# NickTravers/NeuralNetworkLibrary

Hardware: AMD Instinct MI355X
Metric: ResNet-34 224x224 training throughput (Learner.train1minibatch, fwd+loss+bwd+optimizer) (higher is better)
Workload: dtype f32; 1 GPU; DogsCats ResNet-34 classifier, 224x224, bs=64 per GPU, SGD momentum 0.9, fp32; global_batch=64, image_size=224, parallelism=dp1

## Files before the change

### include/nnl.h

```cpp
#ifndef NNL_H_
#define NNL_H_

#include <stddef.h>
#include <stdint.h>

#ifdef __cplusplus
extern "C" {
#endif

typedef enum {
  NNL_OK = 0,
  NNL_ERR_INVALID_ARG = -1,
  NNL_ERR_HIP = -2,
  NNL_ERR_UNSUPPORTED = -3,
  NNL_ERR_WORKSPACE = -4
} nnl_status_t;

int nnl_version(void);
const char* nnl_last_error(void);
int nnl_reload_env(void);

enum { NNL_PROF_CONV_FWD = 0, NNL_PROF_CONV_DGRAD = 1, NNL_PROF_CONV_WGRAD = 2, NNL_PROF_EMBDOT = 3,
       NNL_PROF_TABULAR = 4, NNL_PROF_RETINA_LOSS = 5, NNL_PROF_LSTM = 6, NNL_PROF_SOFTMAX_CE = 7,
       NNL_PROF_ELEMENTWISE = 8, NNL_PROF_GEMM = 9, NNL_PROF_OPTIM = 10, NNL_PROF_KINDS = 11 };
int nnl_prof_enable(int enable);
int nnl_prof_collect(int64_t* launches, double* total_ms, double* total_work);
int nnl_prof_collect2(int64_t* launches, double* total_ms, double* total_work, double* total_exec);
int nnl_dp_bump(int32_t* step, void* stream);
int nnl_dp_signal(int32_t* flag, const int32_t* step, void* stream);
int nnl_dp_wait(const int32_t* flag, int32_t value, int64_t timeout_us, int32_t* err, void* stream);
const char* nnl_source_stamp(void);

int nnl_embdotbias_fwd(const int64_t* x, const float* U, const float* M, const float* bu, const float* bi,
                       float* y, float* z, int64_t n, int64_t n_user, int64_t n_item, int64_t D,
                       int has_range, float lo, float hi, int32_t* err_flag, void* stream);
size_t nnl_embdotbias_bwd_workspace_bytes(int64_t n);
int nnl_embdotbias_bwd(const int64_t* x, const float* U, const float* M, const float* z, const float* dy,
                       float* dU, float* dM, float* dbu, float* dbi, int64_t n, int64_t n_user,
                       int64_t n_item, int64_t D, int has_range, float lo, float hi, void* workspace, size_t workspace_bytes, void* stream);

typedef struct {
  int32_t N, H, W, C;
  int32_t K, R, S;
  int32_t stride, pad;
  int32_t P, Q;
} nnl_conv_geom_t;

size_t nnl_conv2d_fwd_workspace_bytes(const nnl_conv_geom_t* g);
int64_t nnl_conv2d_tile_counters(void);
int nnl_conv2d_fwd(const float* x, const float* w, const float* bias, float* y, const nnl_conv_geom_t* g,
                   int relu, void* workspace, size_t workspace_bytes, int32_t* tile_counters, float* bn_partials,
                   const float* bn_pivot, int32_t* bn_rows, void* stream);
int nnl_conv2d_fwd_add_up2(const float* x, const float* w, const float* bias, const float* small, float* y,
                           const nnl_conv_geom_t* g, void* stream);
int nnl_upsample2_bwd(const float* dy, float* dsmall, int64_t N, int64_t h, int64_t w, int64_t C, void* stream);
int nnl_conv2d_weight_transpose(const float* w, float* wt, int K, int R, int S, int C, void* stream);
typedef struct {
  const float* w;
  float* wt;
  int32_t K, RS, C, first_tile;
} nnl_wt_desc_t;
int nnl_conv2d_weight_transpose_multi(const nnl_wt_desc_t* desc, const int32_t* tile_tensor, int64_t n_tiles,
                                      double total_elems, void* stream);
size_t nnl_conv2d_dgrad_workspace_bytes(const nnl_conv_geom_t* g);
int nnl_conv2d_dgrad(const float* dy, const float* wt, float* dx, const nnl_conv_geom_t* g, const float* addend,
                     void* workspace, size_t workspace_bytes, int32_t* tile_counters, void* stream);
typedef struct {
  const float* src;
  float* dst;
  int32_t rows, ch, flip, first_block;
  int32_t two_d, reserved;
} nnl_wino_desc_t;
int nnl_conv2d_wino_preferred(const nnl_conv_geom_t* g, int dgrad);
int nnl_wino_filter_multi(const nnl_wino_desc_t* desc, const int32_t* block_desc, int64_t n_blocks, void* stream);
int nnl_conv2d_fwd_pre(const float* x, const float* w, const float* bias, float* y, const nnl_conv_geom_t* g, int relu,
                       void* workspace, size_t workspace_bytes, int32_t* tile_counters, float* bn_partials, const float* bn_pivot,
                       int32_t* bn_rows, const float* u, void* stream);
int nnl_conv2d_dgrad_pre(const float* dy, const float* wt, float* dx, const nnl_conv_geom_t* g, const float* addend,
                         void* workspace, size_t workspace_bytes, int32_t* tile_counters, const float* u, void* stream);
size_t nnl_debug_conv_wino_workspace_bytes(int N, int H, int W, int C, int K);
int nnl_debug_conv_wino_fwd(const float* x, const float* filt, const float* bias, const float* add, float* y, void* ws,
                            size_t ws_bytes, int32_t* counters, long n_counters, float* bn_part, const float* bn_pivot, int N,
                            int H, int W, int C, int K, int relu, int flip, void* stream);
size_t nnl_debug_conv_wino2_workspace_bytes(int N, int H, int W, int C, int K);
int nnl_debug_conv_wino2_fwd(const float* x, const float* filt, const float* bias, const float* add, float* y, void* ws,
                            size_t ws_bytes, int32_t* counters, long n_counters, float* bn_part, const float* bn_pivot, int N,
                            int H, int W, int C, int K, int relu, int flip, void* stream);
int nnl_debug_conv_plan_times(int N, int H, int W, int C, int K, double* out);

int nnl_debug_route_record(int enable);
int nnl_debug_route_collect(char* out, size_t n);
size_t nnl_conv2d_wgrad_workspace_bytes(const nnl_conv_geom_t* g);
int nnl_conv2d_wgrad(const float* x, const float* dy, float* dw, const nnl_conv_geom_t* g, void* workspace,
                     size_t workspace_bytes, void* stream);
size_t nnl_colsum_workspace_bytes(int64_t rows, int64_t cols);
int nnl_sum_tensors(const float* const* src, int n, float* out, int64_t numel, void* stream);
int nnl_colsum(const float* a, float* out, int64_t rows, int64_t cols, void* workspace, size_t workspace_bytes,
               void* stream);
int nnl_relu_gate_colsum(const float* dy, const float* y, float* g, float* colsum, int64_t rows, int64_t cols, void* workspace,
                         size_t workspace_bytes, void* stream);
int nnl_act_gate_colsum(const float* dy, const float* y, float* g, float* colsum, int64_t rows, int64_t cols, int act,
                        void* workspace, size_t workspace_bytes, void* stream);

size_t nnl_bn_workspace_bytes(int64_t rows, int64_t C);
int nnl_bn_fwd(const float* x, const float* gamma, const float* beta, const float* residual, float* y,
               float* save_mean, float* save_invstd, float* running_mean, float* running_var, int64_t rows,
               int64_t C, float eps, float momentum, int training, int relu, int64_t* num_batches_tracked,
               uint32_t* relu_mask, const float* ext_partials, int64_t ext_rows, const float* ext_pivot, float* pivot_out,
               void* workspace, size_t workspace_bytes, void* stream);
int nnl_bn_bwd(const float* dy, const float* y, const uint32_t* relu_mask, const float* x, const float* gamma,
               const float* mean, const float* invstd, float* dx, float* dres, float* dgamma, float* dbeta, int64_t rows,
               int64_t C, int training, int relu, void* workspace, size_t workspace_bytes, void* stream);

int nnl_bn_relu_maxpool_supported(int64_t C);
int nnl_bn_relu_maxpool_fwd(const float* x, const float* gamma, const float* beta, float* y, uint8_t* idx, float* save_mean,
                            float* save_invstd, float* save_scale, float* save_shift, float* running_mean, float* running_var,
                            int64_t N, int64_t H, int64_t W, int64_t C, int64_t P, int64_t Q, int ks, int stride, int pad, float eps,
                            float momentum, int training, int64_t* num_batches_tracked, void* workspace, size_t workspace_bytes,
                            void* stream);
int nnl_bn_relu_maxpool_bwd(const float* dpool, const float* y, const uint8_t* idx, const float* x, const float* gamma,
                            const float* beta, const float* mean, const float* invstd, const float* scale, const float* shift,
                            float* dx, float* dgamma, float* dbeta,
                            int64_t N, int64_t H, int64_t W, int64_t C, int64_t P, int64_t Q, int ks, int stride, int pad,
                            int training, void* workspace, size_t workspace_bytes, void* stream);

int nnl_debug_bn_plan(int64_t rows, int64_t C, int64_t N, int64_t H, int64_t W, int64_t P, int64_t Q, int32_t* out10);

int nnl_bn_sync_stats(const float* x, float* stats, int64_t rows, int64_t C, void* workspace, size_t workspace_bytes,
                      void* stream);
int nnl_bn_sync_fwd(const float* x, const float* all_stats, int world, const float* gamma, const float* beta,
                    const float* residual, float* y, float* save_mean, float* save_invstd, float* running_mean,
                    float* running_var, int64_t rows, int64_t C, float eps, float momentum, int relu,
                    int64_t* num_batches_tracked, uint32_t* relu_mask, void* workspace, size_t workspace_bytes, void* stream);
int nnl_bn_sync_bwd_reduce(const float* dy, const float* y, const uint32_t* relu_mask, const float* x, const float* mean,
                           const float* invstd, float* sums, int64_t rows, int64_t C, int relu, void* workspace,
                           size_t workspace_bytes, void* stream);
int nnl_bn_sync_bwd(const float* dy, const float* y, const uint32_t* relu_mask, const float* x, const float* gamma,
                    const float* mean, const float* invstd, const float* local_sums, const float* global_sums,
                    const float* all_stats,
                    int world, float* dx, float* dres, float* dgamma, float* dbeta, int64_t rows, int64_t C, int relu,
                    void* workspace, size_t workspace_bytes, void* stream);

int nnl_maxpool2d_fwd(const float* x, float* y, uint8_t* idx, int64_t N, int64_t H, int64_t W, int64_t C, int64_t P,
                      int64_t Q, int ksize, int stride, int pad, void* stream);
int nnl_maxpool2d_bwd(const float* dy, const uint8_t* idx, float* dx, int64_t N, int64_t H, int64_t W, int64_t C,
                      int64_t P, int64_t Q, int ksize, int stride, int pad, void* stream);
int nnl_concat_pool_fwd(const float* x, float* out, int32_t* argmax, int64_t N, int64_t HW, int64_t C, void* stream);
int nnl_concat_pool_bwd(const float* dout, const int32_t* argmax, float* dx, int64_t N, int64_t HW, int64_t C, void* stream);

int nnl_bbox_decode(const float* anchors, const float* reg, const float* clas, int64_t bs, int64_t A, int64_t K,
                    const float* mean4, const float* std4, float thresh, float width, float height, float* cand_boxes,
                    int32_t* cand_classes, float* cand_scores, int32_t* cand_order, int32_t* cand_count, void* stream);
int nnl_bbox_decode_window(const float* anchors, const float* reg, const float* clas, int64_t bs, int64_t A, int64_t K,
                           const float* mean4, const float* std4, float thresh, float x_min, float y_min, float x_max, float y_max,
                           float* cand_boxes, int32_t* cand_classes, float* cand_scores, int32_t* cand_order, int32_t* cand_count,
                           void* stream);
size_t nnl_nms_workspace_bytes(int64_t bs, int64_t top_k);
int nnl_nms(const float* cand_boxes, const int32_t* cand_classes, const float* cand_scores, const int32_t* cand_order,
            const int32_t* cand_count, int64_t bs, int64_t cap, int64_t top_k, float max_overlap, float* kept_boxes,
            int32_t* kept_classes, float* kept_scores, int32_t* kept_count, void* workspace, size_t workspace_bytes,
            void* stream);

typedef struct {
  float col_jit, row_jit;
  float inv;
  float cols;
  int32_t flip;
} nnl_tta_undo_t;
int nnl_tta_bbox_merge(const float* boxes, const int32_t* classes, const float* scores, const int32_t* counts,
                       const nnl_tta_undo_t* undo, int64_t L, int64_t P, int64_t M, float* cand_boxes, int32_t* cand_classes,
                       float* cand_scores, int32_t* cand_order, int32_t* cand_count, int32_t* err_flag, void* stream);

int nnl_tab_renorm(const int64_t* xcat, float* const* tables, const int32_t* card, const int32_t* dim,
                   const int32_t* row_off, const int32_t* row_table, int32_t* flags, int64_t bs, int32_t ncat,
                   int32_t total_rows, float max_norm, int32_t* err_flag, void* stream);
int nnl_tab_gather_fwd(const int64_t* xcat, const float* const* tables, const int32_t* card, const int32_t* dim,
                       const int32_t* col_off, const int32_t* col_table, const float* row_mask, const float* cont,
                       const float* cont_mask, float* out, int64_t bs, int32_t ncat, int32_t cat_width,
                       int32_t n_cont, int32_t ld_out, void* stream);
size_t nnl_tab_scatter_bwd_workspace_bytes(int64_t bs, int32_t ncat);
int nnl_tab_scatter_bwd(const int64_t* xcat, const int32_t* card, const int32_t* dim, const int32_t* col_off,
                        const int32_t* col_table, const int64_t* grad_off, const float* row_mask,
                        const float* cont_mask, const float* dout, float* dtab_flat, int64_t dtab_elems,
                        float* dcont, int64_t bs, int32_t ncat, int32_t cat_width, int32_t n_cont, int32_t ld_out,
                        void* workspace, size_t workspace_bytes, void* stream);
int nnl_tab_scan_bwd(const int64_t* xcat, const int32_t* card, const int32_t* dim, const int32_t* col_off,
                     const int64_t* grad_off, const float* row_mask, const float* cont_mask, const float* dout,
                     float* dtab_flat, float* dcont, const int32_t* blk_col, const int32_t* blk_first, int32_t n_scan_blocks,
                     int32_t max_dim, int64_t bs, int32_t ncat, int32_t cat_width, int32_t n_cont, int32_t ld_out, void* stream);

int nnl_pad_cols(const float* src, float* dst, int64_t rows, int64_t C, int64_t Cp, void* stream);
int nnl_keep_masks(const float* u, float* a, int64_t na, float keep_a, float* b, int64_t nb, float keep_b, void* stream);

int nnl_linear_small_supported(int64_t N);
int nnl_linear_small_fwd(const float* x, const float* w, const float* bias, float* y, int64_t M, int64_t K, int64_t ldx, int64_t N,
                         void* stream);
size_t nnl_linear_small_bwd_workspace_bytes(int64_t M, int64_t K, int64_t N);
int nnl_linear_small_bwd(const float* dy, const float* x, const float* w, float* dx, float* dw, float* db, int64_t M, int64_t K,
                         int64_t ldx, int64_t N, void* workspace, size_t workspace_bytes, void* stream);

size_t nnl_retina_loss_workspace_bytes(int64_t bs, int64_t A);
int nnl_retina_loss_fwd(const float* anchors, const float* reg, const float* clas, const float* boxes,
                        const int64_t* cats, int32_t* state, float* npos, float* out, int64_t bs, int64_t A,
                        int64_t K, int64_t M, float beta, float alpha, float gamma, void* workspace,
                        size_t workspace_bytes, void* stream);
int nnl_retina_loss_bwd(const float* anchors, const float* reg, const float* clas, const float* boxes,
                        const int64_t* cats, const int32_t* state, const float* npos, const float* grad_out,
                        float* dreg, float* dclas, int64_t bs, int64_t A, int64_t K, int64_t M, float beta,
                        float alpha, float gamma, void* stream);

int64_t nnl_lstm_padded_hidden(int64_t H);
int64_t nnl_lstm_padded_gates(int64_t H);
size_t nnl_lstm_workspace_bytes(int64_t T, int64_t B, int64_t H);
int nnl_lstm_fwd(const float* gx, const float* w_hh_pad, const float* h0, const float* c0, float* y, float* cy,
                 float* gates, int64_t T, int64_t B, int64_t H, void* workspace, size_t workspace_bytes, int32_t* err_flag,
                 void* stream);
int nnl_lstm_bwd(const float* dy, const float* dhT, const float* dcT, const float* gates, const float* cy,
                 const float* c0, const float* w_hh_t_pad, float* dgates_pad, float* dh0, float* dc0, int64_t T, int64_t B,
                 int64_t H, void* workspace, size_t workspace_bytes, int32_t* err_flag, void* stream);
int nnl_debug_lstm_bptt2_plan(int64_t B, int64_t H, int32_t* out5);
int nnl_debug_lstm_plan(int64_t B, int64_t H, int32_t* out14);

size_t nnl_mse_workspace_bytes(int64_t n);
int nnl_mse_fwd(const float* pred, const float* target, float* loss, int64_t n, void* workspace, size_t workspace_bytes, void* stream);
int nnl_mse_bwd(const float* pred, const float* target, const float* grad_out, float* dpred, int64_t n, void* stream);
size_t nnl_bce_logits_workspace_bytes(int64_t n);
int nnl_bce_logits_fwd(const float* logits, const float* target, float* loss, int64_t n, void* workspace, size_t workspace_bytes, void* stream);
int nnl_bce_logits_bwd(const float* logits, const float* target, const float* grad_out, float* dlogits, int64_t n, void* stream);
size_t nnl_fbeta_workspace_bytes(int64_t N, int64_t C);
int nnl_fbeta(const float* pred, const float* target, float* out, int64_t N, int64_t C, float beta2, float threshold, int use_thresh, float eps,
              void* workspace, size_t workspace_bytes, void* stream);
int nnl_scaled_sigmoid_fwd(const float* x, float* y, float* sig, int64_t n, float lo, float hi, void* stream);
int nnl_scaled_sigmoid_bwd(const float* dy, const float* sig, float* dx, int64_t n, float lo, float hi, void* stream);

int nnl_embedding_rowmask_fwd(const int64_t* x, const float* W, const float* rowmask, float* out, int64_t n,
                              int64_t V, int64_t D, int32_t* err_flag, void* stream);
size_t nnl_embedding_rowmask_bwd_workspace_bytes(int64_t n);
int nnl_embedding_rowmask_bwd(const int64_t* x, const float* rowmask, const float* dout, float* dW, int64_t n,
                              int64_t V, int64_t D, int64_t padding_idx, void* workspace, size_t workspace_bytes, void* stream);
int nnl_softmax_ce_fwd(const float* logits, const int64_t* target, float* lse, float* loss_rows, float* loss_mean,
                       int64_t rows, int64_t V, int32_t* err_flag, void* stream);
int nnl_softmax_ce_bwd(const float* logits, const int64_t* target, const float* lse, const float* grad_out,
                       float* dlogits, int64_t rows, int64_t V, int64_t ld_dlogits, void* stream);
size_t nnl_seq_reg_workspace_bytes(int64_t T, int64_t R);
int nnl_seq_reg_fwd(const float* h, float* out3, int64_t T, int64_t R, float alpha, float beta, void* workspace,
                    size_t workspace_bytes, void* stream);
int nnl_seq_reg_bwd(const float* h, const float* grad_out, float* dh, int64_t T, int64_t R, float alpha, float beta, void* stream);
// ... 112 lines not shown
```

### neuralnetworklibrary_amd/_lib.py

```python
import ctypes as C
import os

import torch

_HERE = os.path.dirname(os.path.abspath(__file__))
LIB_PATH = os.environ.get('NNL_LIB_PATH') or os.path.join(_HERE, 'libnnl_hip.so')

if not os.path.exists(LIB_PATH):
    raise ImportError(
        f"{LIB_PATH} not found: build it with `python -c 'import __graft_entry__ as g; g.build()'` "
        "(or `make -C neuralnetworklibrary_amd/csrc`). There is no CPU fallback for the HIP hot path.")

lib = C.CDLL(LIB_PATH)

c_p = C.c_void_p
i32, i64, f32, f64 = C.c_int32, C.c_int64, C.c_float, C.c_double
sz = C.c_size_t


class ConvGeom(C.Structure):
    _fields_ = [('N', i32), ('H', i32), ('W', i32), ('C', i32), ('K', i32), ('R', i32), ('S', i32),
                ('stride', i32), ('pad', i32), ('P', i32), ('Q', i32)]


SIGNATURES = {
    'nnl_version': (C.c_int, []),
    'nnl_last_error': (C.c_char_p, []),
    'nnl_reload_env': (C.c_int, []),
    'nnl_prof_enable': (C.c_int, [C.c_int]),
    'nnl_prof_collect': (C.c_int, [C.POINTER(i64), C.POINTER(f64), C.POINTER(f64)]),
    'nnl_prof_collect2': (C.c_int, [C.POINTER(i64), C.POINTER(f64), C.POINTER(f64), C.POINTER(f64)]),
    'nnl_source_stamp': (C.c_char_p, []),
    'nnl_dp_bump': (C.c_int, [c_p, c_p]),
    'nnl_dp_signal': (C.c_int, [c_p, c_p, c_p]),
    'nnl_dp_wait': (C.c_int, [c_p, i32, i64, c_p, c_p]),
    'nnl_embdotbias_fwd': (C.c_int, [c_p, c_p, c_p, c_p, c_p, c_p, c_p, i64, i64, i64, i64, C.c_int, f32, f32,
                                     c_p, c_p]),
    'nnl_embdotbias_bwd_workspace_bytes': (sz, [i64]),
    'nnl_embdotbias_bwd': (C.c_int, [c_p, c_p, c_p, c_p, c_p, c_p, c_p, c_p, c_p, i64, i64, i64, i64, C.c_int,
                                     f32, f32, c_p, sz, c_p]),
    'nnl_conv2d_fwd_workspace_bytes': (sz, [C.POINTER(ConvGeom)]),
    'nnl_conv2d_dgrad_workspace_bytes': (sz, [C.POINTER(ConvGeom)]),
    'nnl_conv2d_tile_counters': (i64, []),
    'nnl_conv2d_wino_preferred': (C.c_int, [C.POINTER(ConvGeom), C.c_int]),
    'nnl_wino_filter_multi': (C.c_int, [c_p, c_p, i64, c_p]),
    'nnl_conv2d_fwd_pre': (C.c_int, [c_p, c_p, c_p, c_p, C.POINTER(ConvGeom), C.c_int, c_p, sz, c_p, c_p, c_p, C.POINTER(i32), c_p, c_p]),
    'nnl_conv2d_dgrad_pre': (C.c_int, [c_p, c_p, c_p, C.POINTER(ConvGeom), c_p, c_p, sz, c_p, c_p, c_p]),
    'nnl_debug_conv_wino_workspace_bytes': (sz, [C.c_int] * 5),
    'nnl_debug_conv_wino_fwd': (C.c_int, [c_p] * 6 + [sz, c_p, C.c_long, c_p, c_p] + [C.c_int] * 7 + [c_p]),
    'nnl_debug_conv_wino2_workspace_bytes': (sz, [C.c_int] * 5),
    'nnl_debug_conv_wino2_fwd': (C.c_int, [c_p] * 6 + [sz, c_p, C.c_long, c_p, c_p] + [C.c_int] * 7 + [c_p]),
    'nnl_debug_conv_plan_times': (C.c_int, [C.c_int] * 5 + [C.POINTER(C.c_double)]),
    'nnl_debug_route_record': (C.c_int, [C.c_int]),
    'nnl_debug_route_collect': (C.c_int, [C.c_char_p, sz]),
    'nnl_conv2d_fwd': (C.c_int, [c_p, c_p, c_p, c_p, C.POINTER(ConvGeom), C.c_int, c_p, sz, c_p, c_p, c_p, C.POINTER(i32), c_p]),
    'nnl_conv2d_weight_transpose': (C.c_int, [c_p, c_p, C.c_int, C.c_int, C.c_int, C.c_int, c_p]),
    'nnl_conv2d_weight_transpose_multi': (C.c_int, [c_p, c_p, i64, f64, c_p]),
    'nnl_conv2d_dgrad': (C.c_int, [c_p, c_p, c_p, C.POINTER(ConvGeom), c_p, c_p, sz, c_p, c_p]),
    'nnl_conv2d_wgrad_workspace_bytes': (sz, [C.POINTER(ConvGeom)]),
    'nnl_conv2d_wgrad': (C.c_int, [c_p, c_p, c_p, C.POINTER(ConvGeom), c_p, sz, c_p]),
    'nnl_colsum_workspace_bytes': (sz, [i64, i64]),
    'nnl_colsum': (C.c_int, [c_p, c_p, i64, i64, c_p, sz, c_p]),
    'nnl_relu_gate_colsum': (C.c_int, [c_p, c_p, c_p, c_p, i64, i64, c_p, sz, c_p]),
    'nnl_conv2d_fwd_add_up2': (C.c_int, [c_p, c_p, c_p, c_p, c_p, C.POINTER(ConvGeom), c_p]),
    'nnl_upsample2_bwd': (C.c_int, [c_p, c_p, i64, i64, i64, i64, c_p]),
    'nnl_act_gate_colsum': (C.c_int, [c_p, c_p, c_p, c_p, i64, i64, C.c_int, c_p, sz, c_p]),
    'nnl_maxpool2d_fwd': (C.c_int, [c_p, c_p, c_p, i64, i64, i64, i64, i64, i64, C.c_int, C.c_int, C.c_int, c_p]),
    'nnl_maxpool2d_bwd': (C.c_int, [c_p, c_p, c_p, i64, i64, i64, i64, i64, i64, C.c_int, C.c_int, C.c_int, c_p]),
    'nnl_sum_tensors': (C.c_int, [c_p, C.c_int, c_p, i64, c_p]),
    'nnl_bn_relu_maxpool_supported': (C.c_int, [i64]),
    'nnl_bn_relu_maxpool_fwd': (C.c_int, [c_p, c_p, c_p, c_p, c_p, c_p, c_p, c_p, c_p, c_p, c_p, i64, i64, i64, i64, i64, i64,
                                          C.c_int, C.c_int, C.c_int, f32, f32, C.c_int, c_p, c_p, sz, c_p]),
    'nnl_bn_relu_maxpool_bwd': (C.c_int, [c_p, c_p, c_p, c_p, c_p, c_p, c_p, c_p, c_p, c_p, c_p, c_p, c_p, i64, i64, i64, i64, i64, i64,
                                          C.c_int, C.c_int, C.c_int, C.c_int, c_p, sz, c_p]),
    'nnl_concat_pool_fwd': (C.c_int, [c_p, c_p, c_p, i64, i64, i64, c_p]),
    'nnl_concat_pool_bwd': (C.c_int, [c_p, c_p, c_p, i64, i64, i64, c_p]),
    'nnl_bbox_decode': (C.c_int, [c_p, c_p, c_p, i64, i64, i64, c_p, c_p, f32, f32, f32, c_p, c_p, c_p, c_p, c_p, c_p]),
    'nnl_bbox_decode_window': (C.c_int, [c_p, c_p, c_p, i64, i64, i64, c_p, c_p, f32, f32, f32, f32, f32, c_p, c_p, c_p, c_p, c_p, c_p]),
    'nnl_nms_workspace_bytes': (sz, [i64, i64]),
    'nnl_nms': (C.c_int, [c_p, c_p, c_p, c_p, c_p, i64, i64, i64, f32, c_p, c_p, c_p, c_p, c_p, sz, c_p]),
    'nnl_tta_bbox_merge': (C.c_int, [c_p, c_p, c_p, c_p, c_p, i64, i64, i64, c_p, c_p, c_p, c_p, c_p, c_p, c_p]),
    'nnl_tab_renorm': (C.c_int, [c_p, c_p, c_p, c_p, c_p, c_p, c_p, i64, i32, i32, f32, c_p, c_p]),
    'nnl_tab_gather_fwd': (C.c_int, [c_p, c_p, c_p, c_p, c_p, c_p, c_p, c_p, c_p, c_p, i64, i32, i32, i32, i32, c_p]),
    'nnl_tab_scatter_bwd_workspace_bytes': (sz, [i64, i32]),
    'nnl_tab_scatter_bwd': (C.c_int, [c_p, c_p, c_p, c_p, c_p, c_p, c_p, c_p, c_p, c_p, i64, c_p, i64, i32, i32, i32, i32, c_p, sz, c_p]),
    'nnl_tab_scan_bwd': (C.c_int, [c_p] * 12 + [i32, i32, i64, i32, i32, i32, i32, c_p]),
    'nnl_pad_cols': (C.c_int, [c_p, c_p, i64, i64, i64, c_p]),
    'nnl_keep_masks': (C.c_int, [c_p, c_p, i64, f32, c_p, i64, f32, c_p]),
    'nnl_linear_small_supported': (C.c_int, [i64]),
    'nnl_linear_small_fwd': (C.c_int, [c_p, c_p, c_p, c_p, i64, i64, i64, i64, c_p]),
    'nnl_linear_small_bwd_workspace_bytes': (sz, [i64, i64, i64]),
    'nnl_linear_small_bwd': (C.c_int, [c_p, c_p, c_p, c_p, c_p, c_p, i64, i64, i64, i64, c_p, sz, c_p]),
    'nnl_retina_loss_workspace_bytes': (sz, [i64, i64]),
    'nnl_retina_loss_fwd': (C.c_int, [c_p, c_p, c_p, c_p, c_p, c_p, c_p, c_p, i64, i64, i64, i64, f32, f32, f32, c_p, sz, c_p]),
    'nnl_retina_loss_bwd': (C.c_int, [c_p, c_p, c_p, c_p, c_p, c_p, c_p, c_p, c_p, c_p, i64, i64, i64, i64, f32, f32, f32, c_p]),
    'nnl_lstm_padded_hidden': (i64, [i64]),
    'nnl_lstm_padded_gates': (i64, [i64]),
    'nnl_lstm_workspace_bytes': (sz, [i64, i64, i64]),
    'nnl_lstm_fwd': (C.c_int, [c_p, c_p, c_p, c_p, c_p, c_p, c_p, i64, i64, i64, c_p, sz, c_p, c_p]),
    'nnl_lstm_bwd': (C.c_int, [c_p, c_p, c_p, c_p, c_p, c_p, c_p, c_p, c_p, c_p, i64, i64, i64, c_p, sz, c_p, c_p]),
    'nnl_debug_lstm_bptt2_plan': (C.c_int, [i64, i64, c_p]),
    'nnl_debug_lstm_plan': (C.c_int, [i64, i64, C.POINTER(i32)]),
    'nnl_embedding_rowmask_fwd': (C.c_int, [c_p, c_p, c_p, c_p, i64, i64, i64, c_p, c_p]),
    'nnl_embedding_rowmask_bwd_workspace_bytes': (sz, [i64]),
    'nnl_embedding_rowmask_bwd': (C.c_int, [c_p, c_p, c_p, c_p, i64, i64, i64, i64, c_p, sz, c_p]),
    'nnl_softmax_ce_fwd': (C.c_int, [c_p, c_p, c_p, c_p, c_p, i64, i64, c_p, c_p]),
    'nnl_softmax_ce_bwd': (C.c_int, [c_p, c_p, c_p, c_p, c_p, i64, i64, i64, c_p]),
    'nnl_mse_workspace_bytes': (sz, [i64]),
    'nnl_mse_fwd': (C.c_int, [c_p, c_p, c_p, i64, c_p, sz, c_p]),
    'nnl_mse_bwd': (C.c_int, [c_p, c_p, c_p, c_p, i64, c_p]),
    'nnl_bce_logits_workspace_bytes': (sz, [i64]),
    'nnl_bce_logits_fwd': (C.c_int, [c_p, c_p, c_p, i64, c_p, sz, c_p]),
    'nnl_bce_logits_bwd': (C.c_int, [c_p, c_p, c_p, c_p, i64, c_p]),
    'nnl_fbeta_workspace_bytes': (sz, [i64, i64]),
    'nnl_fbeta': (C.c_int, [c_p, c_p, c_p, i64, i64, C.c_float, C.c_float, C.c_int, C.c_float, c_p, sz, c_p]),
    'nnl_scaled_sigmoid_fwd': (C.c_int, [c_p, c_p, c_p, i64, C.c_float, C.c_float, c_p]),
    'nnl_scaled_sigmoid_bwd': (C.c_int, [c_p, c_p, c_p, i64, C.c_float, C.c_float, c_p]),
    'nnl_seq_reg_workspace_bytes': (sz, [i64, i64]),
    'nnl_seq_reg_fwd': (C.c_int, [c_p, c_p, i64, i64, C.c_float, C.c_float, c_p, sz, c_p]),
    'nnl_seq_reg_bwd': (C.c_int, [c_p, c_p, c_p, i64, i64, C.c_float, C.c_float, c_p]),
    'nnl_weight_drop': (C.c_int, [c_p, i64, c_p, c_p, i64, i64, i64, C.c_uint64, C.c_float, c_p]),
    'nnl_lstm_cell_b1': (C.c_int, [c_p, i64, c_p, i64, c_p, c_p, c_p, i64, c_p, i64, i64, c_p, c_p, c_p, c_p, i64, i64, c_p]),
    'nnl_lm_next_token_workspace_bytes': (sz, [i64, i64]),
    'nnl_lm_next_token': (C.c_int, [c_p, i64, c_p, i64, i64, i64, i64, c_p, i64, c_p, i64, c_p, c_p, c_p, c_p, sz, c_p]),
    'nnl_attn_pool_workspace_bytes': (sz, [i64, i64, i64, i64]),
    'nnl_attn_pool_fwd': (C.c_int, [c_p, c_p, c_p, c_p, c_p, i64, c_p, c_p, i64, i64, i64, i64, c_p, sz, c_p, i64, c_p]),
    'nnl_attn_pool_bwd': (C.c_int, [c_p, c_p, c_p, c_p, c_p, c_p, c_p, c_p, c_p, c_p, i64, i64, i64, i64, c_p, sz, c_p, i64, c_p]),
    'nnl_image_aug_workspace_bytes': (sz, [i64, i64, i64]),
    'nnl_image_aug': (C.c_int, [c_p, i64, c_p, i64, c_p, i64, i64, i64, C.POINTER(f32), C.c_int, c_p, c_p, sz, c_p]),
    'nnl_detect_aug': (C.c_int, [c_p, i64, c_p, i64, c_p, c_p, c_p, i64, c_p, i64, i64, i64, i64, i64, i64, f64, C.POINTER(f32),
                                 c_p, c_p, c_p, c_p]),
    'nnl_optim_chunk_elems': (i64, []),
    'nnl_optim_patch': (C.c_int, [c_p, c_p, c_p, i64, c_p]),
    'nnl_optim_step': (C.c_int, [c_p, c_p, c_p, i64, C.c_int, c_p, C.c_int, c_p, c_p]),
    'nnl_bn_workspace_bytes': (sz, [i64, i64]),
    'nnl_bn_fwd': (C.c_int, [c_p, c_p, c_p, c_p, c_p, c_p, c_p, c_p, c_p, i64, i64, f32, f32, C.c_int, C.c_int, c_p, c_p, c_p, i64,
                             c_p, c_p, c_p, sz, c_p]),
    'nnl_debug_bn_plan': (C.c_int, [i64] * 7 + [C.POINTER(i32)]),
    'nnl_bn_sync_stats': (C.c_int, [c_p, c_p, i64, i64, c_p, sz, c_p]),
    'nnl_bn_sync_fwd': (C.c_int, [c_p, c_p, C.c_int, c_p, c_p, c_p, c_p, c_p, c_p, c_p, c_p, i64, i64, f32, f32, C.c_int, c_p,
                                  c_p, c_p, sz, c_p]),
    'nnl_bn_sync_bwd_reduce': (C.c_int, [c_p, c_p, c_p, c_p, c_p, c_p, c_p, i64, i64, C.c_int, c_p, sz, c_p]),
    'nnl_bn_sync_bwd': (C.c_int, [c_p, c_p, c_p, c_p, c_p, c_p, c_p, c_p, c_p, c_p, C.c_int, c_p, c_p, c_p, c_p, i64, i64,
                                  C.c_int, c_p, sz, c_p]),
    'nnl_bn_bwd': (C.c_int, [c_p, c_p, c_p, c_p, c_p, c_p, c_p, c_p, c_p, c_p, c_p, i64, i64, C.c_int, C.c_int, c_p, sz, c_p]),
    'nnl_seg_event_gaps': (C.c_int, [c_p, c_p, c_p, i64, f64, c_p, c_p, c_p, c_p, c_p]),
    'nnl_seg_rolling': (C.c_int, [c_p, c_p, c_p, c_p, i64, i64, i64, i64, C.c_int, C.c_int, c_p, c_p]),
    'nnl_assoc_contingency': (C.c_int, [c_p, c_p, i64, i64, c_p, c_p, c_p, i64, c_p, c_p]),
    'nnl_assoc_table_stats': (C.c_int, [c_p, c_p, i64, c_p, c_p, c_p, i64, c_p, c_p]),
    'nnl_assoc_cat_cont_workspace_bytes': (sz, [c_p, i64, c_p, i64]),
    'nnl_assoc_cat_cont': (C.c_int, [c_p, c_p, i64, c_p, c_p, i64, i64, c_p, c_p, i64, c_p, sz, c_p, c_p]),
    'nnl_assoc_cont_cont_workspace_bytes': (sz, [i64, i64]),
    'nnl_assoc_cont_cont': (C.c_int, [c_p, c_p, i64, i64, c_p, c_p, i64, C.c_int, c_p, sz, c_p, c_p]),
    'nnl_det_coco_match': (C.c_int, [c_p] * 7 + [i64, i64, i64, c_p, i64, c_p, i64, c_p, sz, c_p, c_p, c_p, c_p, c_p]),
    'nnl_det_coco_accumulate': (C.c_int, [c_p] * 8 + [i64, i64, i64, i64, i64, c_p, i64, c_p, i64, c_p, c_p, c_p, c_p]),
    'nnl_det_map_match': (C.c_int, [c_p, c_p, c_p, c_p, i64, i64, i64, c_p, i64, c_p, c_p]),
    'nnl_det_map_integrate_workspace_bytes': (sz, [i64, i64]),
    'nnl_det_map_integrate': (C.c_int, [c_p, c_p, c_p, c_p, c_p, i64, i64, i64, c_p, sz, c_p, c_p]),
}

for _name, (_res, _args) in SIGNATURES.items():
    try:
        _fn = getattr(lib, _name)
    except AttributeError as e:
        raise ImportError(f"libnnl_hip.so does not export {_name}; rebuild it") from e
    _fn.restype = _res
    _fn.argtypes = _args

PROF_KINDS = ['conv_fwd', 'conv_dgrad', 'conv_wgrad', 'embdot', 'tabular', 'retina_loss', 'lstm',
              'softmax_ce', 'elementwise', 'gemm', 'optim']


class NnlError(RuntimeError):
    pass


def check(status):
    if status != 0:
        raise NnlError(f"nnl error {status}: {lib.nnl_last_error().decode()}")


def ptr(t):
    return None if t is None else C.c_void_p(t.data_ptr())


def stream():
    return C.c_void_p(torch.cuda.current_stream().cuda_stream)


def require_cuda(*tensors):
    for t in tensors:
        if t is not None and not t.is_cuda:
            raise NnlError("nnl HIP op called with a non-CUDA tensor: the MI355X path has no CPU fallback")


def prof_enable(flag=True):
    check(lib.nnl_prof_enable(1 if flag else 0))


def prof_collect():
    n = len(PROF_KINDS)
    a, b, c, d = (i64 * n)(), (f64 * n)(), (f64 * n)(), (f64 * n)()
    check(lib.nnl_prof_collect2(a, b, c, d))
    return {k: {'launches': int(a[i]), 'ms': float(b[i]), 'work': float(c[i]), 'exec': float(d[i])} for i, k in enumerate(PROF_KINDS)}


def source_stamp_of_tree():
    import glob
    import hashlib
    csrc = os.path.join(os.path.dirname(os.path.abspath(__file__)), 'csrc')
    names = sorted(os.path.basename(p) for p in glob.glob(os.path.join(csrc, '*.hip')) + glob.glob(os.path.join(csrc, '*.h')))
    hsh = hashlib.sha256()
    for p in [os.path.join(csrc, n) for n in names] + [os.path.join(csrc, 'Makefile'), os.path.join(csrc, '..', '..', 'include', 'nnl.h')]:
# ... 8 lines not shown
```

### neuralnetworklibrary_amd/csrc/conv2d.hip

```cpp
#include "igemm_kernels.h"
#include "igemm_taps.h"
#include "wino.h"
#include "igemm_wgrad.h"
#include "igemm_wgrad2d.h"

#ifdef NNL_TAPS_TIMING
static void* g_wgrad_dbg = nullptr;
extern "C" void* nnl_debug_wgrad_stamps(void) { return g_wgrad_dbg; }
#endif

namespace {

int check_geom(const nnl_conv_geom_t* g, const char* who) {
  if (!g) return nnl_set_error(NNL_ERR_INVALID_ARG, "%s: null geometry", who);
  if (g->N <= 0 || g->H <= 0 || g->W <= 0 || g->C <= 0 || g->K <= 0 || g->R <= 0 || g->S <= 0 || g->stride <= 0 ||
      g->pad < 0)
    return nnl_set_error(NNL_ERR_INVALID_ARG, "%s: non-positive dimension", who);
  if (g->H + 2L * g->pad < g->R || g->W + 2L * g->pad < g->S)
    return nnl_set_error(NNL_ERR_INVALID_ARG, "%s: the %d x %d filter is larger than the padded input (%d x %d, pad %d)", who, g->R, g->S,
                         g->H, g->W, g->pad);
  const int P = (g->H + 2 * g->pad - g->R) / g->stride + 1, Q = (g->W + 2 * g->pad - g->S) / g->stride + 1;
  if (P != g->P || Q != g->Q || P <= 0 || Q <= 0)
    return nnl_set_error(NNL_ERR_INVALID_ARG, "%s: P,Q=(%d,%d) do not match the geometry (%d,%d)", who, g->P, g->Q, P, Q);
  if (g->C % 4 != 0)
    return nnl_set_error(NNL_ERR_UNSUPPORTED, "%s: C=%d must be a multiple of 4 (pad the channels; ops.py does)", who, g->C);
  if ((long)g->N * g->H * g->W * g->C >= (1L << 31) || (long)g->N * g->P * g->Q * g->K >= (1L << 31) ||
      (long)g->N * g->P * g->Q >= (1L << 30))
    return nnl_set_error(NNL_ERR_UNSUPPORTED, "%s: tensor too large for 32-bit row indexing", who);
  return NNL_OK;
}

template <int BM, int BN, int WGM, int WGN, int MODE>
int launch_rowk(IgemmRowkParams p, hipStream_t s) {
  p.grid_m = (int)nnl_cdiv(p.M, BM);
  p.grid_n = (int)nnl_cdiv(p.Nc, BN);
  NNL_ROUTE("rowk<%d,%d>:%s", BM, BN, MODE == IGEMM_MODE_FWD ? "fwd" : "dgrad");
  hipLaunchKernelGGL((igemm_rowk_kernel<BM, BN, 16, WGM, WGN, MODE>), dim3(p.grid_m * p.grid_n), dim3(256), 0, s, p);
  NNL_CHECK_LAUNCH();
  return NNL_OK;
}

template <int MODE>
int dispatch_rowk(const IgemmRowkParams& p, hipStream_t s) {
  const long b128 = nnl_cdiv(p.M, 128);
  if (p.Nc > 64) {
    if (b128 * nnl_cdiv(p.Nc, 128) >= 400) return launch_rowk<128, 128, 2, 2, MODE>(p, s);
    if (nnl_cdiv(p.M, 64) * nnl_cdiv(p.Nc, 128) >= 400) return launch_rowk<64, 128, 2, 2, MODE>(p, s);
    return launch_rowk<64, 64, 2, 2, MODE>(p, s);
  }
  if (b128 >= 400) return launch_rowk<128, 64, 2, 2, MODE>(p, s);
  return launch_rowk<64, 64, 2, 2, MODE>(p, s);
}


static bool taps_dma(int bk) {
  const int m = NNL_ENV_INT("NNL_IGEMM_DMA", 0);
  return bk == 16 ? (m & 1) != 0 : (m & 2) != 0;
}

template <int BM, int BN, int BK = 16>
int launch_taps(IgemmTapsParams p, hipStream_t s) {
  p.grid_m = (int)nnl_cdiv(p.M, BM);
  p.grid_n = (int)nnl_cdiv(p.Nc, BN);
  p.cls_tiles = p.grid_m * p.grid_n;
  const dim3 grid((unsigned)(p.grid_m * p.grid_n * (p.ncls > 1 ? p.ncls : 1)), p.ksplit > 1 ? p.ksplit : 1);
  NNL_ROUTE("taps<%d,%d,%d>%s%s%s", BM, BN, BK, (BM == 64 && BN == 64 && taps_dma(BK)) ? ":dma" : "", p.ncls > 1 ? ":ncls" : "",
            p.ksplit > 1 ? ":ksplit" : "");
  if constexpr (BM == 64 && BN == 64) {
    if (taps_dma(BK))
      hipLaunchKernelGGL((igemm_taps_kernel<64, 64, BK, 2, 2, false, 0, true>), grid, dim3(256), 0, s, p);
    else if constexpr (BK == 16)
      hipLaunchKernelGGL((igemm_taps_kernel<64, 64, 16, 2, 2, true, 0, false, 2>), grid, dim3(256), 0, s, p);
    else
      hipLaunchKernelGGL((igemm_taps_kernel<64, 64, BK, 2, 2, true>), grid, dim3(256), 0, s, p);
  } else {
    hipLaunchKernelGGL((igemm_taps_kernel<BM, BN, BK, 2, 2>), grid, dim3(256), 0, s, p);
  }
  NNL_CHECK_LAUNCH();
  return NNL_OK;
}

template <int BK>
int launch_taps_ktail(IgemmTapsParams p, hipStream_t s) {
  p.grid_m = (int)nnl_cdiv(p.M, 64);
  p.grid_n = (int)nnl_cdiv(p.Nc, 64);
  p.cls_tiles = p.grid_m * p.grid_n;
  NNL_ROUTE("taps_ktail<%d>", BK);
  hipLaunchKernelGGL((igemm_taps_kernel<64, 64, BK, 2, 2, true, 0, false, 1, true>), dim3((unsigned)(p.grid_m * p.grid_n), 1), dim3(256), 0, s, p);
  NNL_CHECK_LAUNCH();
  return NNL_OK;
}

struct BalPlan {
  int on, bk, main_ks, n_main_tiles, tail_slices, tail_row0;
  size_t main_floats, tail_floats;
  double t_us;
};

constexpr int kCUs = 256;
constexpr long kTileCounters = 65536;

BalPlan plan_balance(long M, int Nc, int C, int ntaps) {
  BalPlan best{};
  const int e_bal = NNL_ENV_INT("NNL_IGEMM_BALANCE", 1);
  if (e_bal == 0 || Nc % 4 != 0) return best;
  const long gm = nnl_cdiv(M, 64), gn = nnl_cdiv(Nc, 64), T = gm * gn;
  const int bk = ((T < 1200 || C >= 256 || C == 64) && C % 32 == 0) ? 32 : 16;
  const long I = (long)ntaps * (C / bk);
  const double c_it = bk == 32 ? 0.60 : 0.30;
  const double occ = bk == 32 ? 4 : 6;
  auto wave_iters = [&](long blocks, long iters) {
    if (blocks <= 0) return 0.0;
    const long cap = (long)occ * kCUs;
    const long full = blocks / cap, rem = blocks - full * cap;
    return (double)(full * (long)occ + nnl_cdiv(rem, kCUs)) * iters;
  };
  const double plain = wave_iters(T, I) * c_it;
  best.t_us = plain;
  double best_t = plain * (e_bal == 2 ? 1.25 : 0.99);
  const int plan_extra = 2;
  const double plan_bw = 16000 * 1.0e3;
  for (int ks = 1; ks <= 4; ks *= 2) {
    if (I / ks < 8) break;
    const long units = T * ks;
    long n_main = ((units / kCUs) * kCUs / ks / gn) * gn;
    if (n_main > T) n_main = T;
    const long tail = T - n_main;
    const long it_main = nnl_cdiv(I, ks);
    static const int kSlices[] = {1, 2, 3, 4, 6, 8, 9, 12, 16, 18, 24, 32, 36, 48};
    for (int S : kSlices) {
      if (tail == 0 && S > 1) break;
      if (S > 1 && I / S < 4) break;
      const long it_tail = nnl_cdiv(I, S);
      const long tail_blocks = tail * S;
      double t = (wave_iters(n_main * ks, it_main) + wave_iters(tail_blocks, it_tail + (S > 1 ? plan_extra : 0))) * c_it;
      const long row0 = (n_main / gn) * 64 < M ? (n_main / gn) * 64 : M;
      const double main_b = ks > 1 ? (2.0 * ks + 1) * row0 * Nc * 4 : 0;
      const double tail_b = S > 1 ? (2.0 * S + 1) * (M - row0) * Nc * 4 : 0;
      t += (main_b + tail_b) / plan_bw + (ks > 1 ? 1 : 0) + (S > 1 && tail ? 1 : 0);
      if (t < best_t) {
        best_t = t;
        best.t_us = t;
        best.on = 1; best.bk = bk; best.main_ks = ks; best.n_main_tiles = (int)n_main; best.tail_slices = tail ? S : 1;
        best.tail_row0 = (int)row0;
        best.main_floats = ks > 1 ? (size_t)ks * row0 * Nc : 0;
        best.tail_floats = (S > 1 && tail) ? (size_t)S * (M - row0) * Nc : 0;
      }
    }
  }
  if (best.on && best.main_ks == 1 && best.tail_slices == 1) best.on = 0;
  return best;
}
// ... 2 lines not shown
  const BalPlan pl = plan_balance(M, Nc, C, ntaps);
  return pl.on ? (pl.main_floats + pl.tail_floats) * sizeof(float) : 0;
}

__global__ __launch_bounds__(256) void slab_reduce_kernel(const float* __restrict__ part, long slab_stride4, int nslabs,
                                                           float* __restrict__ out, long n4, const float* __restrict__ bias,
                                                           const float* __restrict__ add, int Nc4, int relu) {
  const long i = (long)blockIdx.x * 256 + threadIdx.x;
  if (i >= n4) return;
  f32x4 acc = reinterpret_cast<const f32x4*>(part)[i];
  for (int sl = 1; sl < nslabs; ++sl) acc += reinterpret_cast<const f32x4*>(part)[(long)sl * slab_stride4 + i];
  if (bias) acc += reinterpret_cast<const f32x4*>(bias)[i % Nc4];
  if (add) acc += reinterpret_cast<const f32x4*>(add)[i];
  if (relu == 1) { acc[0] = fmaxf(acc[0], 0.f); acc[1] = fmaxf(acc[1], 0.f); acc[2] = fmaxf(acc[2], 0.f); acc[3] = fmaxf(acc[3], 0.f); }
  else if (relu == 2) { acc[0] = nnl_sigmoid(acc[0]); acc[1] = nnl_sigmoid(acc[1]); acc[2] = nnl_sigmoid(acc[2]); acc[3] = nnl_sigmoid(acc[3]); }
  reinterpret_cast<f32x4*>(out)[i] = acc;
}

int launch_balanced(IgemmTapsParams p, const BalPlan& pl, float* ws, int* counters, hipStream_t s) {
  p.grid_m = (int)nnl_cdiv(p.M, 64);
  p.grid_n = (int)nnl_cdiv(p.Nc, 64);
  const int T = p.grid_m * p.grid_n;
  p.bal = 1; p.main_ks = pl.main_ks; p.n_main_tiles = pl.n_main_tiles; p.tail_slices = pl.tail_slices; p.tail_row0 = pl.tail_row0;
  p.main_out = ws; p.main_slab_stride = (long)pl.tail_row0 * p.Nc;
  p.tail_out = ws + pl.main_floats; p.tail_slab_stride = (long)(p.M - pl.tail_row0) * p.Nc;
  p.tile_counters = counters;
  const unsigned grid = (unsigned)(pl.n_main_tiles * pl.main_ks + (T - pl.n_main_tiles) * pl.tail_slices);
  NNL_ROUTE("balanced<%d>%s%s%s%s:%s@main_ks=%d,tail_slices=%d", pl.bk == 32 ? 32 : 16, p.ktail ? ":ktail" : "",
            (!p.ktail && taps_dma(pl.bk == 32 ? 32 : 16)) ? ":dma" : "", pl.main_ks > 1 ? ":main_ks" : "", pl.tail_slices > 1 ? ":tail_slices" : "",
            p.tile_counters != nullptr ? "counters" : "reduce", pl.main_ks, pl.tail_slices);
  if (p.ktail && pl.bk == 32)
    hipLaunchKernelGGL((igemm_taps_kernel<64, 64, 32, 2, 2, true, 0, false, 1, true>), dim3(grid), dim3(256), 0, s, p);
  else if (p.ktail)
    hipLaunchKernelGGL((igemm_taps_kernel<64, 64, 16, 2, 2, true, 0, false, 1, true>), dim3(grid), dim3(256), 0, s, p);
  else if (pl.bk == 32 && taps_dma(32))
    hipLaunchKernelGGL((igemm_taps_kernel<64, 64, 32, 2, 2, false, 0, true>), dim3(grid), dim3(256), 0, s, p);
  else if (pl.bk != 32 && taps_dma(16))
    hipLaunchKernelGGL((igemm_taps_kernel<64, 64, 16, 2, 2, false, 0, true>), dim3(grid), dim3(256), 0, s, p);
  else if (pl.bk == 32)
    hipLaunchKernelGGL((igemm_taps_kernel<64, 64, 32, 2, 2, true>), dim3(grid), dim3(256), 0, s, p);
  else
    hipLaunchKernelGGL((igemm_taps_kernel<64, 64, 16, 2, 2, true, 0, false, 2>), dim3(grid), dim3(256), 0, s, p);
  NNL_CHECK_LAUNCH();
  if (p.tile_counters != nullptr) return NNL_OK;
  const int Nc4 = p.Nc / 4;
  if (pl.main_ks > 1 && pl.tail_row0 > 0) {
    const long n4 = (long)pl.tail_row0 * Nc4;
    NNL_ROUTE("slab_reduce:main");
    hipLaunchKernelGGL(slab_reduce_kernel, dim3((unsigned)nnl_cdiv(n4, 256)), dim3(256), 0, s, (const float*)p.main_out, n4, pl.main_ks,
                       p.y, n4, p.bias, p.add, Nc4, p.relu);
    NNL_CHECK_LAUNCH();
  }
  if (pl.tail_slices > 1 && p.M > pl.tail_row0) {
    const long n4 = (long)(p.M - pl.tail_row0) * Nc4;
    const long off = (long)pl.tail_row0 * p.Nc;
    NNL_ROUTE("slab_reduce:tail");
    hipLaunchKernelGGL(slab_reduce_kernel, dim3((unsigned)nnl_cdiv(n4, 256)), dim3(256), 0, s, (const float*)p.tail_out, n4,
                       pl.tail_slices, p.y + off, n4, p.bias, p.add ? p.add + off : nullptr, Nc4, p.relu);
    NNL_CHECK_LAUNCH();
  }
  return NNL_OK;
}

int dispatch_taps(const IgemmTapsParams& p_in, hipStream_t s, void* ws = nullptr, size_t ws_bytes = 0, int* counters = nullptr,
                  int* bn_rows = nullptr) {
  IgemmTapsParams p = p_in;
#ifdef NNL_TAPS_TIMING
  p.tile_counters = counters;
#endif
  if (bn_rows) *bn_rows = 0;
  float* const bn_part = p.bn_part;
  p.bn_part = nullptr;
  if (!p.ktail && p.ntaps == 1 && p.C <= 512 && p.Nc >= 8192 && p.M >= 1024 && p.ncls <= 1) {
    return launch_taps<128, 128>(p, s);
  }
  const bool dense = p.out_stride == 1 && p.OH == p.P && p.OW == p.Q && p.oh0 == 0 && p.ow0 == 0 && p.ksplit <= 1;
  const int rows64 = (int)nnl_cdiv(p.M, 64);
  if (ws != nullptr && dense) {
    const BalPlan pl = plan_balance(p.M, p.Nc, p.ktail ? (int)nnl_cdiv(p.C, 32) * 32 : p.C, p.ntaps);
    if (pl.on && ws_bytes >= (pl.main_floats + pl.tail_floats) * sizeof(float)) {
      int* const cnt = rows64 * nnl_cdiv(p.Nc, 64) <= kTileCounters ? counters : nullptr;
      if (bn_part && cnt != nullptr) {
        p.bn_part = bn_part;
        if (bn_rows) *bn_rows = rows64;
      }
      return launch_balanced(p, pl, (float*)ws, cnt, s);
    }
  }
  if (bn_part && dense) {
    p.bn_part = bn_part;
    if (bn_rows) *bn_rows = rows64;
  }
  if (p.ktail) return p.C >= 64 ? launch_taps_ktail<32>(p, s) : launch_taps_ktail<16>(p, s);
  const long blocks64 = rows64 * nnl_cdiv(p.Nc, 64) * (p.ncls > 1 ? p.ncls : 1);
  const bool bk32 = blocks64 < 1200 || p.C >= 256 || p.C == 64;
  if (bk32 && p.C % 32 == 0) return launch_taps<64, 64, 32>(p, s);
  return launch_taps<64, 64>(p, s);
}

bool affine_taps_ok(int S) { return S <= 32; }

bool dgrad_tap_table_ok(const nnl_conv_geom_t* g) {
  if (g->stride == 1 && affine_taps_ok(g->S)) return true;
  return (g->pad + g->stride - 1) / g->stride <= 127;
}

bool taps_ok(long a_elems, long b_elems, int C, int ntaps) {
  return C % 16 == 0 && ntaps <= IGEMM_MAX_TAPS && a_elems * 4 < (1L << 31) && b_elems * 4 < (1L << 32) - 64;
}

int taps_kind(long a_elems, long b_elems, int C, int ntaps) {
  if (taps_ok(a_elems, b_elems, C, ntaps)) return 1;
  if (ntaps == 1 && C % 4 == 0 && C >= 32 && a_elems * 4 < (1L << 31) && b_elems * 4 < (1L << 32) - 64 && NNL_ENV_INT("NNL_IGEMM_KTAIL", 1) != 0)
    return 2;
  return 0;
}

__global__ void weight_transpose_kernel(const float* __restrict__ w, float* __restrict__ wt, int K, int RS, int C) {
  __shared__ float tile[32][33];
  const int tap = blockIdx.z;
  const int k0 = blockIdx.y * 32, c0 = blockIdx.x * 32;
  const int tx = threadIdx.x & 31, ty = threadIdx.x >> 5;
  for (int i = ty; i < 32; i += 8) {
    const int k = k0 + i, c = c0 + tx;
    tile[i][tx] = (k < K && c < C) ? w[((long)k * RS + tap) * C + c] : 0.f;
  }
  __syncthreads();
  for (int i = ty; i < 32; i += 8) {
    const int c = c0 + i, k = k0 + tx;
    if (k < K && c < C) wt[((long)c * RS + tap) * K + k] = tile[tx][i];
  }
}

__global__ void weight_transpose_multi_kernel(const nnl_wt_desc_t* __restrict__ desc, const int* __restrict__ tile_tensor) {
  __shared__ float tile[32][33];
  const nnl_wt_desc_t d = desc[tile_tensor[blockIdx.x]];
  int t = (int)blockIdx.x - d.first_tile;
  const int ct = (d.C + 31) / 32, kt = (d.K + 31) / 32;
  const int c0 = (t % ct) * 32; t /= ct;
  const int k0 = (t % kt) * 32;
  const int tap = t / kt;
  const int tx = threadIdx.x & 31, ty = threadIdx.x >> 5;
  for (int i = ty; i < 32; i += 8) {
    const int k = k0 + i, c = c0 + tx;
    tile[i][tx] = (k < d.K && c < d.C) ? d.w[((long)k * d.RS + tap) * d.C + c] : 0.f;
  }
  __syncthreads();
  for (int i = ty; i < 32; i += 8) {
    const int c = c0 + i, k = k0 + tx;
    if (k < d.K && c < d.C) d.wt[((long)c * d.RS + tap) * d.K + k] = tile[tx][i];
  }
}

__global__ __launch_bounds__(256) void splitk_reduce_kernel(const float* __restrict__ part, float* __restrict__ out, long n4,
                                                             int splits) {
  __shared__ f32x4 red[8][32];
  const int col = threadIdx.x & 31, sl = threadIdx.x >> 5;
  const long i = (long)blockIdx.x * 32 + col;
  f32x4 acc = {0.f, 0.f, 0.f, 0.f};
  if (i < n4) {
    int s = sl;
    for (; s + 24 < splits; s += 32) {
      const f32x4 v0 = reinterpret_cast<const f32x4*>(part)[(long)s * n4 + i], v1 = reinterpret_cast<const f32x4*>(part)[(long)(s + 8) * n4 + i];
      const f32x4 v2 = reinterpret_cast<const f32x4*>(part)[(long)(s + 16) * n4 + i], v3 = reinterpret_cast<const f32x4*>(part)[(long)(s + 24) * n4 + i];
      acc += v0; acc += v1; acc += v2; acc += v3;
    }
    for (; s < splits; s += 8) acc += reinterpret_cast<const f32x4*>(part)[(long)s * n4 + i];
  }
  red[sl][col] = acc;
  __syncthreads();
  if (sl == 0 && i < n4) {
    f32x4 t = red[0][col];
#pragma unroll
    for (int l = 1; l < 8; ++l) t += red[l][col];
    reinterpret_cast<f32x4*>(out)[i] = t;
  }
}

__global__ __launch_bounds__(256) void colsum_partial_kernel(const float* __restrict__ a, float* __restrict__ part, long rows,
                                                              int cols, long rows_per_chunk) {
  __shared__ float red[4][64];
  const int c = blockIdx.x * 64 + (threadIdx.x & 63);
  const int rl = threadIdx.x >> 6;
  const long r0 = (long)blockIdx.y * rows_per_chunk;
  const long r1 = r0 + rows_per_chunk < rows ? r0 + rows_per_chunk : rows;
  float acc = 0.f;
  if (c < cols) {
    long r = r0 + rl;
    for (; r + 12 < r1; r += 16) {
      const float v0 = a[r * cols + c], v1 = a[(r + 4) * cols + c], v2 = a[(r + 8) * cols + c], v3 = a[(r + 12) * cols + c];
      acc += (v0 + v1) + (v2 + v3);
    }
    for (; r < r1; r += 4) acc += a[r * cols + c];
  }
  red[rl][threadIdx.x & 63] = acc;
  __syncthreads();
  if (rl == 0 && c < cols)
    part[(long)blockIdx.y * cols + c] = (red[0][threadIdx.x] + red[1][threadIdx.x]) + (red[2][threadIdx.x] + red[3][threadIdx.x]);
}

template <int ACT>
__device__ __forceinline__ float act_gate(float dy, float y) {
  if (ACT == 1) return y > 0.f ? dy : 0.f;
  return dy * ((1.f - y) * y);
}

template <int ACT>
__global__ __launch_bounds__(256) void act_gate_colsum_kernel(const float* __restrict__ dy, const float* __restrict__ y,
                                                               float* __restrict__ g, float* __restrict__ part, long rows, int cols,
                                                               long rows_per_chunk) {
  __shared__ float red[4][64];
  const int c = blockIdx.x * 64 + (threadIdx.x & 63);
  const int rl = threadIdx.x >> 6;
  const long r0 = (long)blockIdx.y * rows_per_chunk;
  const long r1 = r0 + rows_per_chunk < rows ? r0 + rows_per_chunk : rows;
  float acc = 0.f;
  if (c < cols) {
    long r = r0 + rl;
    for (; r + 12 < r1; r += 16) {
      float v[4];
#pragma unroll
      for (int u = 0; u < 4; ++u) {
        const long o = (r + 4 * u) * cols + c;
        v[u] = act_gate<ACT>(dy[o], y[o]);
      }
#pragma unroll
      for (int u = 0; u < 4; ++u) g[(r + 4 * u) * cols + c] = v[u];
      acc += (v[0] + v[1]) + (v[2] + v[3]);
    }
    for (; r < r1; r += 4) {
      const long o = r * cols + c;
      const float v = act_gate<ACT>(dy[o], y[o]);
      g[o] = v;
      acc += v;
    }
  }
  red[rl][threadIdx.x & 63] = acc;
  __syncthreads();
  if (rl == 0 && c < cols && part != nullptr)
    part[(long)blockIdx.y * cols + c] = (red[0][threadIdx.x] + red[1][threadIdx.x]) + (red[2][threadIdx.x] + red[3][threadIdx.x]);
}

__global__ __launch_bounds__(256) void colsum_final_kernel(const float* __restrict__ part, float* __restrict__ out, int cols,
                                                            int nchunk) {
  __shared__ float red[16][17];
  const int cl = threadIdx.x & 15, kl = threadIdx.x >> 4;
  const int c = blockIdx.x * 16 + cl;
  float acc = 0.f;
  if (c < cols)
    for (int k = kl; k < nchunk; k += 16) acc += part[(long)k * cols + c];
  red[kl][cl] = acc;
  __syncthreads();
  if (kl == 0 && c < cols) {
    float t = red[0][cl];
#pragma unroll
    for (int l = 1; l < 16; ++l) t += red[l][cl];
    out[c] = t;
  }
}

int colsum_chunks(long rows) {
  long n = nnl_cdiv(rows, 64);
  if (n > 256) n = 256;
  if (n < 1) n = 1;
  return (int)n;
}

struct WgradPlan { int bm, bn, grid_m, grid_n, splits, k_per_split, kg; };

WgradPlan plan_wgrad(int Mc, int Nc, long Kp, int square_bn_divides = 0) {
  struct Cand { int bm, bn; double cost; };
  static const Cand cands[4] = {{128, 128, 1.00}, {128, 64, 1.08}, {64, 128, 1.08}, {64, 64, 1.10}};
  const long max_splits = Kp / 256 > 0 ? Kp / 256 : 1;
  WgradPlan pl{};
  double best_t = 1e300;
  for (int ci = 0; ci < 4; ++ci) {
    const Cand& c = cands[ci];
    if (square_bn_divides != 0) {
      if (c.bm != c.bn || square_bn_divides % c.bn != 0 || (c.bm == 128 && Mc < 128)) continue;
    } else if ((c.bm == 128 && Mc < 128) || (c.bn == 128 && Nc < 128)) continue;
    const long tiles = nnl_cdiv(Mc, c.bm) * nnl_cdiv(Nc, c.bn);
    const double us_per_px = (double)c.bm * c.bn * 2.0 / 441e3 * c.cost;
    for (long sp = 1; sp <= max_splits && (sp == 1 || tiles * sp <= 256 * 5); ++sp) {
      const long k1 = nnl_cdiv(nnl_cdiv(Kp, sp), 32) * 32;
      const long rs = nnl_cdiv(Kp, k1);
      if (rs != sp) continue;
      const long per_cu = nnl_cdiv(tiles * rs, 256);
      const double starve = per_cu < 4 ? pow(4.0 / per_cu, 0.3) : 1.0;
      const double t = (double)per_cu * k1 * us_per_px * starve + (rs > 1 ? (rs + 1.0) * Mc * Nc * 4 / 4.5e6 + 3 : 0);
      if (t < best_t) {
        best_t = t;
        pl.bm = c.bm; pl.bn = c.bn; pl.grid_m = (int)nnl_cdiv(Mc, c.bm); pl.grid_n = (int)nnl_cdiv(Nc, c.bn);
        pl.splits = (int)rs; pl.k_per_split = (int)k1;
      }
    }
  }
  if (pl.bm == 0) {
    pl.bm = Mc >= 128 ? 128 : 64; pl.bn = (Nc >= 128 && pl.bm == 128) ? 128 : 64;
    if (square_bn_divides != 0 && square_bn_divides % pl.bn != 0) { pl.bm = 64; pl.bn = 64; }
    pl.grid_m = (int)nnl_cdiv(Mc, pl.bm); pl.grid_n = (int)nnl_cdiv(Nc, pl.bn);
    pl.splits = 1; pl.k_per_split = (int)(nnl_cdiv(Kp, 32) * 32);
  }
  pl.kg = 1;
  const bool kg_tile = (pl.bm == 128 && pl.bn == 128) || (pl.bm == 64 && pl.bn == 64);
  if (kg_tile && pl.splits >= 2) {
    int kg = (pl.bm == 128 && pl.splits >= 16) ? 4 : 1;
    if (square_bn_divides != 0 && pl.bm == 128) kg = 1;
    if (kg > 1) {
      const long sp = nnl_cdiv(pl.splits, kg);
      const long k1 = nnl_cdiv(nnl_cdiv(Kp, sp), 32L * kg) * 32L * kg;
      pl.kg = kg; pl.k_per_split = (int)k1; pl.splits = (int)nnl_cdiv(Kp, k1);
    }
  }
  return pl;
}

bool wgrad_v2_ok(long a_elems, long b_elems, long Kp) {
  return a_elems * 4 < (1L << 32) - 64 && b_elems * 4 < (1L << 32) - 64 && Kp < (1L << 23);
}

constexpr size_t wgrad_lds_bytes(int bm_plus_bn, int bk, int kg) { return (size_t)kg * 2 * bk * bm_plus_bn * sizeof(float); }

template <auto Kernel, class Params, class Note>
int launch_wave_groups(const Params& q, int kg, size_t lds, hipStream_t s, Note note) {
  if (lds > 64 * 1024) {
    static bool attr_set = false;
    if (!attr_set) {
      NNL_CHECK_HIP(hipFuncSetAttribute(reinterpret_cast<const void*>(Kernel), hipFuncAttributeMaxDynamicSharedMemorySize, (int)lds));
      attr_set = true;
    }
  }
  note();
  hipLaunchKernelGGL(Kernel, dim3(q.grid_m * q.grid_n * q.splits), dim3(256 * kg), lds, s, q);
  NNL_CHECK_LAUNCH();
  return NNL_OK;
}

template <int BM, int BN, int BK, bool PIPE, int KG, bool PAIR>
int launch_wgrad_tile(const IgemmWgradParams& q, hipStream_t s) {
  return launch_wave_groups<igemm_wgrad_kernel<BM, BN, BK, 2, 2, PIPE, KG, false, PAIR>>(q, KG, wgrad_lds_bytes(BM + BN, BK, KG), s, [&] {
    NNL_ROUTE("wgrad<%d,%d,%d,kg%d>%s%s@splits=%d", BM, BN, BK, KG, PAIR ? ":pair" : "", q.splits > 1 ? ":splitk" : "", q.splits);
  });
}

int launch_wgrad_v2(const IgemmKmajorParams& p, long a_elems, long b_elems, const WgradPlan& pl, hipStream_t s) {
  IgemmWgradParams q{};
  q.a = p.a; q.b = p.b; q.y = p.y;
  q.a_bytes = (unsigned)(a_elems * 4); q.b_bytes = (unsigned)(b_elems * 4);
  q.H = p.H; q.W = p.W; q.C = p.C; q.P = p.P; q.Q = p.Q; q.R = p.R; q.S = p.S; q.stride = p.stride; q.pad = p.pad;
  q.Mc = p.Mc; q.Nc = p.Nc; q.Kp = (int)p.Kp;
  q.splits = pl.splits; q.k_per_split = pl.k_per_split; q.grid_m = pl.grid_m; q.grid_n = pl.grid_n;
#ifdef NNL_TAPS_TIMING
  { static void* dbg = nullptr; if (!dbg) (void)hipMalloc(&dbg, 3276 * 5 * 8); q.dbg_t = (unsigned long long*)dbg; g_wgrad_dbg = dbg; }
#endif
  {
    const long T = 128, gm = pl.grid_m, gn = pl.grid_n;
    const long fp_m = (T < gm ? T : gm) * pl.bm + nnl_cdiv(T, gm) * pl.bn;
    const long fp_n = nnl_cdiv(T, gn) * pl.bm + (T < gn ? T : gn) * pl.bn;
    q.n_fast = fp_n < fp_m ? 1 : 0;
  }
  const bool t128 = pl.bm == 128 && pl.bn == 128, t64 = pl.bm == 64 && pl.bn == 64;
  if (!(pl.kg == 1 || (pl.kg == 4 && t128)) || (t64 && pl.k_per_split % 32 != 0))
    return nnl_set_error(NNL_ERR_UNSUPPORTED, "wgrad: no kernel for the plan <%d,%d> kg=%d k_per_split=%d", pl.bm, pl.bn, pl.kg, pl.k_per_split);
  const bool pair = p.R * p.S == 1 || p.C % pl.bn == 0;
  if (t128) {
    if (pl.kg == 4) return pair ? launch_wgrad_tile<128, 128, 16, true, 4, true>(q, s) : launch_wgrad_tile<128, 128, 16, true, 4, false>(q, s);
    return pair ? launch_wgrad_tile<128, 128, 16, true, 1, true>(q, s) : launch_wgrad_tile<128, 128, 16, true, 1, false>(q, s);
  }
  if (pl.bm == 128) return launch_wgrad_tile<128, 64, 16, false, 1, false>(q, s);
  if (pl.bn == 128) return launch_wgrad_tile<64, 128, 16, true, 1, false>(q, s);
  return pair ? launch_wgrad_tile<64, 64, 32, true, 1, true>(q, s) : launch_wgrad_tile<64, 64, 32, true, 1, false>(q, s);
}

__global__ __launch_bounds__(256) void wino_wgrad_finish_kernel(const float* __restrict__ part, float* __restrict__ dw, long n4,
                                                                 int C4, int splits, long slab4) {
  __shared__ f32x4 red[8][32][4];
  const int it = threadIdx.x & 31, sl = threadIdx.x >> 5;
  const long i = (long)blockIdx.x * 32 + it;
  f32x4 u0 = {0.f, 0.f, 0.f, 0.f}, u1 = u0, u2 = u0, u3 = u0;
  long c4 = 0, r = 0, k = 0;
  if (i < n4) {
    c4 = i % C4; const long kr = i / C4; r = kr % 3; k = kr / 3;
    const f32x4* src = reinterpret_cast<const f32x4*>(part) + (k * 12 + r) * C4 + c4;
    for (int s = sl; s < splits; s += 8) {
      const f32x4* q = src + s * slab4;
      u0 += q[0]; u1 += q[3L * C4]; u2 += q[6L * C4]; u3 += q[9L * C4];
    }
  }
  red[sl][it][0] = u0; red[sl][it][1] = u1; red[sl][it][2] = u2; red[sl][it][3] = u3;
  __syncthreads();
  if (sl == 0 && i < n4) {
#pragma unroll
    for (int l = 1; l < 8; ++l) { u0 += red[l][it][0]; u1 += red[l][it][1]; u2 += red[l][it][2]; u3 += red[l][it][3]; }
    f32x4* dst = reinterpret_cast<f32x4*>(dw) + (k * 9 + r * 3) * C4 + c4;
    const f32x4 h = 0.5f * (u1 + u2);
    dst[0] = u0 + h;
    dst[C4] = 0.5f * (u1 - u2);
    dst[2L * C4] = h + u3;
  }
}

bool wgrad_wino_ok(const nnl_conv_geom_t* g) {
  const int mode = NNL_ENV_INT("NNL_WGRAD_WINO", 1);
  if (mode == 0) return false;
  if (g->R != 3 || g->S != 3 || g->stride != 1 || g->pad != 1 || g->Q % 2 != 0 || g->C % 64 != 0 || g->K % 4 != 0) return false;
  const long pairs = (long)g->N * g->P * (g->Q / 2);
  if (pairs < 1024 || !wgrad_v2_ok(2 * pairs * g->K, (long)g->N * g->H * g->W * g->C, pairs)) return false;
  if (mode == 2) return true;
  if (g->C == 64) return pairs >= 65536;
  return pairs >= 2048;
}

WgradPlan plan_wgrad_wino(const nnl_conv_geom_t* g) {
  return plan_wgrad(g->K, 12 * g->C, (long)g->N * g->P * (g->Q / 2), 3 * g->C);
}

int launch_wgrad_wino(const float* dy, const float* x, float* slabs, const nnl_conv_geom_t* g, const WgradPlan& pl, hipStream_t s) {
  IgemmWgradParams q{};
  const long pairs = (long)g->N * g->P * (g->Q / 2);
  q.a = dy; q.b = x; q.y = slabs;
  q.a_bytes = (unsigned)(2 * pairs * g->K * 4); q.b_bytes = (unsigned)((long)g->N * g->H * g->W * g->C * 4);
  q.H = g->H; q.W = g->W; q.C = g->C; q.P = g->P; q.Q = g->Q / 2; q.R = 3; q.S = 3; q.stride = 1; q.pad = 1;
  q.Mc = g->K; q.Nc = 12 * g->C; q.Kp = (int)pairs;
  q.splits = pl.splits; q.k_per_split = pl.k_per_split; q.grid_m = pl.grid_m; q.grid_n = pl.grid_n;
  q.n_fast = 1;
  if (pl.kg != 1 || (pl.bm == 64 && pl.k_per_split % 32 != 0))
    return nnl_set_error(NNL_ERR_UNSUPPORTED, "wgrad_wino1d: no kernel for the plan <%d> kg=%d k_per_split=%d", pl.bm, pl.kg, pl.k_per_split);
  const auto note = [&] { NNL_ROUTE("wgrad_wino1d<%d,%d,kg1>@splits=%d", pl.bm, pl.bm == 128 ? 16 : 32, pl.splits); };
  if (pl.bm == 128) return launch_wave_groups<igemm_wgrad_kernel<128, 128, 16, 2, 2, true, 1, true>>(q, 1, wgrad_lds_bytes(256, 16, 1), s, note);
  return launch_wave_groups<igemm_wgrad_kernel<64, 64, 32, 2, 2, true, 1, true>>(q, 1, wgrad_lds_bytes(128, 32, 1), s, note);
}

__global__ __launch_bounds__(256) void wino2d_wgrad_finish_kernel(const float* __restrict__ part, float* __restrict__ dw, long n_items, int C4,
                                                                   int splits, long slab4) {
  __shared__ f32x4 du[16][16];
  const int it = threadIdx.x >> 4, pos = threadIdx.x & 15;
  const long i = (long)blockIdx.x * 16 + it;
  const long c4 = i % C4, k = i / C4;
  f32x4 u = {0.f, 0.f, 0.f, 0.f};
  if (i < n_items) {
    const f32x4* src = reinterpret_cast<const f32x4*>(part) + (k * 16 + pos) * C4 + c4;
    for (int s0 = 0; s0 < splits; s0 += 8) {
      f32x4 v[8];
#pragma unroll
      for (int e = 0; e < 8; ++e) if (s0 + e < splits) v[e] = src[(long)(s0 + e) * slab4];
#pragma unroll
      for (int e = 0; e < 8; ++e) if (s0 + e < splits) u += v[e];
    }
  }
  du[it][pos] = u;
  __syncthreads();
  if (pos < 9 && i < n_items) {
    const int r = pos / 3, sx = pos - r * 3;
    const float gr[4] = {r == 0 ? 1.f : 0.f, 0.5f, r == 1 ? -0.5f : 0.5f, r == 2 ? 1.f : 0.f};
    const float gs[4] = {sx == 0 ? 1.f : 0.f, 0.5f, sx == 1 ? -0.5f : 0.5f, sx == 2 ? 1.f : 0.f};
    f32x4 acc = {0.f, 0.f, 0.f, 0.f};
#pragma unroll
    for (int a = 0; a < 4; ++a) {
      f32x4 row = {0.f, 0.f, 0.f, 0.f};
#pragma unroll
      for (int b = 0; b < 4; ++b) row += gs[b] * du[it][a * 4 + b];
      acc += gr[a] * row;
    }
    reinterpret_cast<f32x4*>(dw)[(k * 9 + pos) * C4 + c4] = acc;
  }
}

bool wgrad_wino2d_ok(const nnl_conv_geom_t* g) {
  const int mode = NNL_ENV_INT("NNL_WGRAD_WINO2D", 1);
  if (mode == 0 || NNL_ENV_INT("NNL_WGRAD_WINO", 1) == 0) return false;
  if (g->R != 3 || g->S != 3 || g->stride != 1 || g->pad != 1 || g->C % 64 != 0 || g->K % 4 != 0 || g->H < 2 || g->W < 2) return false;
  const long quads = (long)g->N * ((g->H + 1) / 2) * ((g->W + 1) / 2);
  if (quads < 512 || !wgrad_v2_ok((long)g->N * g->H * g->W * g->K, (long)g->N * g->H * g->W * g->C, quads)) return false;
  if (mode == 2) return true;
  return quads >= 1024;
}

WgradPlan plan_wgrad_wino2d(const nnl_conv_geom_t* g) {
  const long quads = (long)g->N * ((g->H + 1) / 2) * ((g->W + 1) / 2);
  WgradPlan pl = plan_wgrad(g->K, 16 * g->C, quads, g->C);
  auto with_tile = [&](int bt, int splits_target) {
    WgradPlan q{};
    q.bm = q.bn = bt; q.grid_m = (int)nnl_cdiv(g->K, bt); q.grid_n = (int)nnl_cdiv(16L * g->C, bt); q.kg = 1;
    const long tiles = (long)q.grid_m * q.grid_n;
    long sp = splits_target > 0 ? splits_target : (256L * 4 + tiles - 1) / tiles;
    const long max_sp = quads / 256 > 0 ? quads / 256 : 1;
    if (sp > max_sp) sp = max_sp;
    if (sp < 1) sp = 1;
    const long k1 = nnl_cdiv(nnl_cdiv(quads, sp), 32) * 32;
    q.k_per_split = (int)k1; q.splits = (int)nnl_cdiv(quads, k1);
    return q;
  };
  const bool big = g->K >= 128 && g->C % 128 == 0;
  if (big && (double)quads * g->K * g->C >= 500e6) return pl.bm == 128 ? pl : with_tile(128, 0);
  WgradPlan p64 = pl.bm == 64 ? pl : with_tile(64, 0);
  if (p64.splits >= 4) {
    const long sp = nnl_cdiv(p64.splits, 4);
    const long k1 = nnl_cdiv(nnl_cdiv(quads, sp), 128L) * 128L;
    if (k1 / 4 >= 700) {
      p64.kg = 4; p64.k_per_split = (int)k1; p64.splits = (int)nnl_cdiv(quads, k1);
      return p64;
    }
    return pl;
  }
  if (big) return pl.bm == 128 ? pl : with_tile(128, 0);
  return p64;
}

int launch_wgrad_wino2d(const float* dy, const float* x, float* slabs, const nnl_conv_geom_t* g, const WgradPlan& pl, hipStream_t s) {
  IgemmWgrad2dParams q{};
  q.a = dy; q.b = x; q.y = slabs;
  q.a_bytes = (unsigned)((long)g->N * g->H * g->W * g->K * 4); q.b_bytes = (unsigned)((long)g->N * g->H * g->W * g->C * 4);
  q.H = g->H; q.W = g->W; q.C = g->C; q.H2 = (g->H + 1) / 2; q.W2 = (g->W + 1) / 2;
  q.Mc = g->K; q.Nc = 16 * g->C; q.Kp = (int)((long)g->N * q.H2 * q.W2);
  q.splits = pl.splits; q.k_per_split = pl.k_per_split; q.grid_m = pl.grid_m; q.grid_n = pl.grid_n;
  q.n_fast = 1;
  if (!(pl.kg == 1 || (pl.kg == 4 && pl.bm == 64)) || (pl.bm == 64 && pl.k_per_split % 32 != 0))
    return nnl_set_error(NNL_ERR_UNSUPPORTED, "wgrad_wino2d: no kernel for the plan <%d> kg=%d k_per_split=%d", pl.bm, pl.kg, pl.k_per_split);
  const auto note = [&] { NNL_ROUTE("wgrad_wino2d<%d,%d,kg%d>@splits=%d", pl.bm, pl.bm == 128 ? 16 : 32, pl.kg, pl.splits); };
  if (pl.bm == 128) return launch_wave_groups<igemm_wgrad2d_kernel<128, 16, 1>>(q, 1, wgrad_lds_bytes(256, 16, 1), s, note);
  if (pl.kg == 4) return launch_wave_groups<igemm_wgrad2d_kernel<64, 32, 4>>(q, 4, wgrad_lds_bytes(128, 32, 4), s, note);
  return launch_wave_groups<igemm_wgrad2d_kernel<64, 32, 1>>(q, 1, wgrad_lds_bytes(128, 32, 1), s, note);
}

int launch_wgrad_direct(IgemmKmajorParams p, const WgradPlan& pl, float* ws, float* dw, hipStream_t s) {
  p.grid_m = pl.grid_m; p.grid_n = pl.grid_n; p.splits = pl.splits; p.k_per_split = pl.k_per_split;
  p.y = pl.splits > 1 ? ws : dw;
  const long a_elems = p.Kp * p.Mc, b_elems = (long)p.N * p.H * p.W * p.C;
  if (wgrad_v2_ok(a_elems, b_elems, p.Kp)) {
    const int st = launch_wgrad_v2(p, a_elems, b_elems, pl, s);
    if (st) return st;
  } else {
    const dim3 grid(pl.grid_m * pl.grid_n * pl.splits), block(256);
    NNL_ROUTE("wgrad_kmajor<%d,%d>%s@splits=%d", pl.bm, pl.bn, pl.splits > 1 ? ":splitk" : "", pl.splits);
    if (pl.bm == 128 && pl.bn == 128)
      hipLaunchKernelGGL((igemm_kmajor_kernel<128, 128, 16, 2, 2>), grid, block, 0, s, p);
    else if (pl.bm == 128)
      hipLaunchKernelGGL((igemm_kmajor_kernel<128, 64, 16, 2, 2>), grid, block, 0, s, p);
    else if (pl.bn == 128)
      hipLaunchKernelGGL((igemm_kmajor_kernel<64, 128, 16, 2, 2>), grid, block, 0, s, p);
    else
      hipLaunchKernelGGL((igemm_kmajor_kernel<64, 64, 16, 2, 2>), grid, block, 0, s, p);
    NNL_CHECK_LAUNCH();
  }
  if (pl.splits > 1) {
    const long n4 = (long)p.Mc * p.Nc / 4;
    NNL_ROUTE("splitk_reduce");
    hipLaunchKernelGGL(splitk_reduce_kernel, dim3((unsigned)nnl_cdiv(n4, 32)), dim3(256), 0, s, (const float*)ws, dw, n4, pl.splits);
    NNL_CHECK_LAUNCH();
  }
  return NNL_OK;
}

IgemmTapsParams fwd_taps_params(const nnl_conv_geom_t* g, const float* x, const float* w, float* y, const float* bias, int relu) {
  IgemmTapsParams q{};
  q.a = x; q.b = w; q.y = y; q.bias = bias; q.add = nullptr;
  q.a_bytes = (unsigned)((long)g->N * g->H * g->W * g->C * 4); q.b_bytes = (unsigned)((long)g->K * g->R * g->S * g->C * 4);
  q.H = g->H; q.W = g->W; q.C = g->C; q.P = g->P; q.Q = g->Q;
  q.in_stride = g->stride; q.ih0 = -g->pad; q.iw0 = -g->pad;
  q.OH = g->P; q.OW = g->Q; q.out_stride = 1; q.oh0 = 0; q.ow0 = 0;
  q.M = g->N * g->P * g->Q; q.Nc = g->K; q.b_row_stride = g->R * g->S * g->C; q.relu = relu;
  q.ntaps = g->R * g->S;
  for (int r = 0; r < g->R; ++r)
    for (int ss = 0; ss < g->S; ++ss) {
      const int t = r * g->S + ss;
      q.tap_dh[t] = (signed char)r; q.tap_dw[t] = (signed char)ss;
      q.tap_aoff[t] = (r * g->W + ss) * g->C; q.tap_woff[t] = t * g->C;
    }
  q.tap_affine = affine_taps_ok(g->S); q.tap_R = g->R; q.tap_S = g->S; q.tap_dh0 = 0; q.tap_dw0 = 0; q.tap_dstep = 1;
  return q;
}

IgemmTapsParams gemm_taps_params(const float* a, const float* b, float* y, int M, int N, int K) {
  IgemmTapsParams q{};
  q.a = a; q.b = b; q.y = y;
  q.a_bytes = (unsigned)((long)M * K * 4); q.b_bytes = (unsigned)((long)N * K * 4);
  q.H = 1; q.W = 1; q.C = K; q.P = 1; q.Q = 1; q.in_stride = 1; q.ih0 = 0; q.iw0 = 0;
  q.OH = 1; q.OW = 1; q.out_stride = 1; q.oh0 = 0; q.ow0 = 0;
  q.M = M; q.Nc = N; q.b_row_stride = K; q.ntaps = 1;
  q.tap_dh[0] = 0; q.tap_dw[0] = 0; q.tap_aoff[0] = 0; q.tap_woff[0] = 0;
  q.tap_affine = 1; q.tap_R = 1; q.tap_S = 1; q.tap_dstep = 1;
  return q;
}

}

int nnl_internal_gemm_nt(const float* a, const float* b, float* y, const float* bias, const float* add, int M, int N,
                         int K, int relu, hipStream_t s) {
  if (M <= 0 || N <= 0 || K <= 0 || K % 4 != 0) return nnl_set_error(NNL_ERR_INVALID_ARG, "gemm_nt: bad sizes");
  IgemmRowkParams p{};
  p.a = a; p.b = b; p.y = y; p.bias = bias; p.add = add;
  p.N = M; p.H = 1; p.W = 1; p.C = K; p.P = 1; p.Q = 1; p.R = 1; p.S = 1; p.stride = 1; p.pad = 0;
  p.M = M; p.Nc = N; p.Kg = K; p.relu = relu;
  if (taps_ok((long)M * K, (long)N * K, K, 1)) {
    IgemmTapsParams q = gemm_taps_params(a, b, y, M, N, K);
    q.bias = bias; q.add = add; q.relu = relu;
    return dispatch_taps(q, s);
  }
  return dispatch_rowk<IGEMM_MODE_FWD>(p, s);
}

int nnl_internal_gemm_nt_splitk(const float* a, const float* b, float* y_slabs, int M, int N, int K, int splits, hipStream_t s) {
  if (M <= 0 || N <= 0 || K <= 0 || K % 32 != 0 || splits < 1 || !taps_ok((long)M * K, (long)N * K, K, 1))
    return nnl_set_error(NNL_ERR_INVALID_ARG, "gemm_nt_splitk: bad sizes M=%d N=%d K=%d", M, N, K);
  IgemmTapsParams q = gemm_taps_params(a, b, y_slabs, M, N, K);
  q.ksplit = splits; q.slab_stride = (long)M * N;
  return launch_taps<64, 64, 32>(q, s);
}

int nnl_internal_lstm_step(IgemmTapsParams q, int epi, hipStream_t s) {
  if ((epi != 1 && epi != 2) || q.M <= 0 || q.C % 32 != 0 || q.lstm.H <= 0 || q.lstm.counters == nullptr)
    return nnl_set_error(NNL_ERR_INVALID_ARG, "lstm_step: bad arguments");
  q.grid_m = (int)nnl_cdiv(q.M, 64);
  q.grid_n = epi == 1 ? (int)nnl_cdiv(q.lstm.H, 16) : (int)nnl_cdiv(q.lstm.H, 64);
  q.bal = 0;
  const dim3 grid(q.grid_m * q.grid_n, q.ksplit > 1 ? q.ksplit : 1), block(256);
  if (epi == 1)
    hipLaunchKernelGGL((igemm_taps_kernel<64, 64, 32, 2, 2, true, 1>), grid, block, 0, s, q);
  else
    hipLaunchKernelGGL((igemm_taps_kernel<64, 64, 32, 2, 2, true, 2>), grid, block, 0, s, q);
  NNL_CHECK_LAUNCH();
  return NNL_OK;
}

size_t nnl_internal_gemm_tn_workspace_bytes(int Mc, int Nc, long Kp) {
  const WgradPlan pl = plan_wgrad(Mc, Nc, Kp);
  return pl.splits > 1 ? (size_t)pl.splits * Mc * Nc * sizeof(float) : 0;
}

int nnl_internal_gemm_tn(const float* a, const float* b, float* y, int Mc, int Nc, long Kp, void* ws, size_t ws_bytes,
                         hipStream_t s) {
  if (Mc <= 0 || Nc <= 0 || Kp <= 0 || Mc % 4 != 0 || Nc % 4 != 0) return nnl_set_error(NNL_ERR_INVALID_ARG, "gemm_tn: bad sizes");
  IgemmKmajorParams p{};
  p.a = a; p.b = b;
  p.N = (int)Kp; p.H = 1; p.W = 1; p.C = Nc; p.P = 1; p.Q = 1; p.R = 1; p.S = 1; p.stride = 1; p.pad = 0;
  p.Mc = Mc; p.Nc = Nc; p.Kp = Kp;
  const size_t need = nnl_internal_gemm_tn_workspace_bytes(Mc, Nc, Kp);
  if (need > 0 && (ws == nullptr || ws_bytes < need)) return nnl_set_error(NNL_ERR_WORKSPACE, "gemm_tn: workspace too small");
  return launch_wgrad_direct(p, plan_wgrad(Mc, Nc, Kp), (float*)ws, y, s);
}

static int wino_mode(int N, int H, int W, int Cin, int Nc, int R, int S, int stride, int pad) {
  if (!nnl_wino_ok(N, H, W, Cin, Nc, R, S, stride, pad)) return 0;
  const int e = NNL_ENV_INT("NNL_CONV_WINO", 1);
  const bool two_ok = nnl_wino2_ok(N, H, W, Cin, Nc, R, S, stride, pad);
  if (e >= 3) return two_ok ? 2 : 1;
  if (e == 2) return 1;
  const double t_d = plan_balance((long)N * H * W, Nc, Cin, 9).t_us + 6.0;
  const double t_w = nnl_wino_plan_time_us(N, H, W, Cin, Nc) + 6.0 + 3.0 + 21.0 * Cin * Nc * 4.0 / 4.0e6;
  const bool two_on = two_ok && NNL_ENV_INT("NNL_CONV_WINO2", 1) != 0;
  if (!(t_w < 0.97 * t_d)) {
    if (two_on && nnl_wino2_plan_is_pos(N, H, W, Cin, Nc) && nnl_wino2_plan_time_us(N, H, W, Cin, Nc) < 0.9 * t_d) return 2;
    return 0;
  }
  if (two_on && nnl_wino2_plan_time_us(N, H, W, Cin, Nc) < 0.9 * t_w) return 2;
  return 1;
}
static size_t wino_mode_workspace(int mode, int N, int H, int W, int Cin, int Nc) {
  return mode == 2 ? nnl_wino2_workspace_bytes(N, H, W, Cin, Nc) : nnl_wino_workspace_bytes(N, H, W, Cin, Nc);
}
static int wino_mode_launch(int mode, const WinoProblem& q, void* ws, size_t ws_bytes, int* counters, long n_counters, hipStream_t s) {
  nnl_prof_exec_frac(mode >= 2 ? 1.0 / 2.25 : 1.0 / 1.5);
  return mode == 2 ? nnl_wino2_launch(q, ws, ws_bytes, counters, n_counters, s) : nnl_wino_launch(q, ws, ws_bytes, counters, n_counters, s);
}

extern "C" int nnl_debug_conv_plan_times(int N, int H, int W, int Cin, int Nc, double* out) {
  out[0] = plan_balance((long)N * H * W, Nc, Cin, 9).t_us;
  out[1] = nnl_wino_plan_time_us(N, H, W, Cin, Nc);
  out[2] = nnl_wino2_plan_time_us(N, H, W, Cin, Nc);
  out[3] = -1.0;
  return wino_mode(N, H, W, Cin, Nc, 3, 3, 1, 1);
// ... 130 lines not shown
  {
    const bool taps = taps_ok((long)g->N * g->P * g->Q * g->K, (long)g->C * g->R * g->S * g->K, g->K, g->R * g->S) && dgrad_tap_table_ok(g);
    const bool s2_full = g->stride == 2 && g->R == 3 && g->S == 3 && g->pad == 1;
    if (addend != nullptr && !(taps && (g->stride == 1 || s2_full)))
      return nnl_set_error(NNL_ERR_UNSUPPORTED, "conv2d_dgrad: the fused addend needs K %% 16 == 0 and stride 1 (or a 3x3 / pad 1 filter at stride 2)");
  }
  hipStream_t s = (hipStream_t)stream;
  IgemmRowkParams p{};
  p.a = dy; p.b = wt; p.y = dx; p.bias = nullptr;
  p.N = g->N; p.H = g->P; p.W = g->Q; p.C = g->K;
  p.P = g->H; p.Q = g->W;
  p.R = g->R; p.S = g->S; p.stride = g->stride; p.pad = g->pad;
  p.M = g->N * g->H * g->W; p.Nc = g->C; p.Kg = g->R * g->S * g->K; p.relu = 0;
  NnlProfScope prof(NNL_PROF_CONV_DGRAD, s, 2.0 * g->N * (double)g->P * g->Q * g->K * g->R * g->S * g->C);
  const long a_elems = (long)g->N * g->P * g->Q * g->K, b_elems = (long)g->C * g->R * g->S * g->K;
  const int wmode = workspace != nullptr ? wino_mode(g->N, g->P, g->Q, g->K, g->C, g->R, g->S, g->stride, g->pad) : 0;
  if (wmode && workspace_bytes >= wino_mode_workspace(wmode, g->N, g->P, g->Q, g->K, g->C)) {
    WinoProblem wq{};
    wq.in = dy; wq.filt = wt; wq.out = dx; wq.bias = nullptr; wq.add = addend;
    wq.N = g->N; wq.H = g->P; wq.W = g->Q; wq.Cin = g->K; wq.Nc = g->C; wq.relu = 0; wq.flip = 1;
    wq.u_pre = u;
    return wino_mode_launch(wmode, wq, workspace, workspace_bytes, tile_counters, kTileCounters, s);
  }
  const int tk = dgrad_tap_table_ok(g) ? taps_kind(a_elems, b_elems, g->K, g->R * g->S) : 0;
  if (tk && (g->stride == 1 || g->stride == 2)) {
    IgemmTapsParams q{};
    q.ktail = tk == 2;
    q.a = dy; q.b = wt; q.y = dx; q.bias = nullptr; q.add = addend;
    q.a_bytes = (unsigned)(a_elems * 4); q.b_bytes = (unsigned)(b_elems * 4);
    q.H = g->P; q.W = g->Q; q.C = g->K;
    q.in_stride = 1; q.ih0 = 0; q.iw0 = 0;
    q.OH = g->H; q.OW = g->W; q.Nc = g->C; q.b_row_stride = g->R * g->S * g->K; q.relu = 0;
    const int st2 = g->stride;
    struct Cls { int ph, pw, P, Q, nt; signed char dh[IGEMM_MAX_TAPS], dw[IGEMM_MAX_TAPS]; int aoff[IGEMM_MAX_TAPS], woff[IGEMM_MAX_TAPS]; };
    Cls cls[4];
    int ncls = 0;
    bool need_zero = false;
    for (int ph = 0; ph < st2; ++ph)
      for (int pw = 0; pw < st2; ++pw) {
        Cls c{};
        c.ph = ph; c.pw = pw;
        c.P = (g->H - ph + st2 - 1) / st2; c.Q = (g->W - pw + st2 - 1) / st2;
        for (int r = 0; r < g->R; ++r) {
          if ((ph + g->pad - r) % st2 != 0) continue;
          for (int ss = 0; ss < g->S; ++ss) {
            if ((pw + g->pad - ss) % st2 != 0) continue;
            const int dh = (ph + g->pad - r) / st2, dw = (pw + g->pad - ss) / st2;
            c.dh[c.nt] = (signed char)dh; c.dw[c.nt] = (signed char)dw;
            c.aoff[c.nt] = (dh * g->Q + dw) * g->K; c.woff[c.nt] = (r * g->S + ss) * g->K;
            ++c.nt;
          }
        }
        if (c.P <= 0 || c.Q <= 0) continue;
        if (c.nt == 0) { need_zero = true; continue; }
        cls[ncls++] = c;
      }
    if (need_zero) NNL_ROUTE("dgrad:need_zero");
    if (need_zero) NNL_CHECK_HIP(hipMemsetAsync(dx, 0, sizeof(float) * g->N * g->H * g->W * g->C, s));
    auto fill = [&](IgemmTapsParams& c, const Cls& k, int at) {
      for (int t = 0; t < k.nt; ++t) {
        c.tap_dh[at + t] = k.dh[t]; c.tap_dw[at + t] = k.dw[t]; c.tap_aoff[at + t] = k.aoff[t]; c.tap_woff[at + t] = k.woff[t];
      }
    };
    bool merged = ncls > 1;
    for (int i = 1; i < ncls && merged; ++i) merged = cls[i].P == cls[0].P && cls[i].Q == cls[0].Q;
    if (merged) {
      NNL_ROUTE("dgrad:merged@ncls=%d", ncls);
      for (int i = 1; i < ncls; ++i)
        for (int j = i; j > 0 && cls[j].nt > cls[j - 1].nt; --j) { const Cls t = cls[j]; cls[j] = cls[j - 1]; cls[j - 1] = t; }
      IgemmTapsParams c = q;
      c.P = cls[0].P; c.Q = cls[0].Q; c.M = g->N * c.P * c.Q;
      c.out_stride = st2; c.oh0 = cls[0].ph; c.ow0 = cls[0].pw;
      c.ncls = ncls;
      int at = 0;
      for (int i = 0; i < ncls; ++i) {
        c.cls_tap0[i] = at; c.cls_ntaps[i] = cls[i].nt; c.cls_oh0[i] = cls[i].ph; c.cls_ow0[i] = cls[i].pw;
        fill(c, cls[i], at);
        at += cls[i].nt;
      }
      c.ntaps = cls[0].nt;
      return dispatch_taps(c, s, nullptr, 0, tile_counters);
    }
    if (st2 > 1) NNL_ROUTE("dgrad:per_class@ncls=%d", ncls);
    for (int i = 0; i < ncls; ++i) {
      IgemmTapsParams c = q;
      c.P = cls[i].P; c.Q = cls[i].Q; c.M = g->N * c.P * c.Q;
      c.out_stride = st2; c.oh0 = cls[i].ph; c.ow0 = cls[i].pw;
      fill(c, cls[i], 0);
      c.ntaps = cls[i].nt;
      if (st2 == 1 && cls[i].nt == g->R * g->S && affine_taps_ok(g->S)) {
        c.tap_affine = 1; c.tap_R = g->R; c.tap_S = g->S; c.tap_dh0 = g->pad; c.tap_dw0 = g->pad; c.tap_dstep = -1;
      }
      int st = dispatch_taps(c, s, st2 == 1 ? workspace : nullptr, workspace_bytes, tile_counters);
      if (st) return st;
    }
    return NNL_OK;
  }
  return dispatch_rowk<IGEMM_MODE_DGRAD>(p, s);
}

extern "C" size_t nnl_conv2d_wgrad_workspace_bytes(const nnl_conv_geom_t* g) {
  if (!g || check_geom(g, "conv2d_wgrad_workspace_bytes")) return 0;
  if (wgrad_wino2d_ok(g))
    return (size_t)plan_wgrad_wino2d(g).splits * g->K * 16 * g->C * sizeof(float);
  if (wgrad_wino_ok(g))
    return (size_t)plan_wgrad_wino(g).splits * g->K * 12 * g->C * sizeof(float);
  const WgradPlan pl = plan_wgrad(g->K, g->R * g->S * g->C, (long)g->N * g->P * g->Q);
  return pl.splits > 1 ? (size_t)pl.splits * g->K * g->R * g->S * g->C * sizeof(float) : 0;
}

extern "C" int nnl_conv2d_wgrad(const float* x, const float* dy, float* dw, const nnl_conv_geom_t* g, void* workspace,
                                size_t workspace_bytes, void* stream) {
  int st = check_geom(g, "conv2d_wgrad");
  if (st) return st;
  NNL_CHECK_ARG(x && dy && dw, "conv2d_wgrad: null pointer");
  NNL_CHECK_ARG(g->K % 4 == 0, "conv2d_wgrad: K=%d must be a multiple of 4", g->K);
  hipStream_t s = (hipStream_t)stream;
  IgemmKmajorParams p{};
  p.a = dy; p.b = x;
  p.N = g->N; p.H = g->H; p.W = g->W; p.C = g->C; p.P = g->P; p.Q = g->Q;
  p.R = g->R; p.S = g->S; p.stride = g->stride; p.pad = g->pad;
  p.Mc = g->K; p.Nc = g->R * g->S * g->C; p.Kp = (long)g->N * g->P * g->Q;
  const size_t need = nnl_conv2d_wgrad_workspace_bytes(g);
  if (need > 0 && (workspace == nullptr || workspace_bytes < need))
    return nnl_set_error(NNL_ERR_WORKSPACE, "conv2d_wgrad: workspace %zu B < required %zu B", workspace_bytes, need);
  NnlProfScope prof(NNL_PROF_CONV_WGRAD, s, 2.0 * p.Kp * (double)p.Mc * p.Nc);
  if (wgrad_wino2d_ok(g)) {
    const WgradPlan wp = plan_wgrad_wino2d(g);
    nnl_prof_exec_frac(1.0 / 2.25);
    int st2 = launch_wgrad_wino2d(dy, x, (float*)workspace, g, wp, s);
    if (st2) return st2;
    const long n_items = (long)g->K * (g->C / 4);
    NNL_ROUTE("wgrad_wino2d_finish");
    hipLaunchKernelGGL(wino2d_wgrad_finish_kernel, dim3((unsigned)nnl_cdiv(n_items, 16L)), dim3(256), 0, s, (const float*)workspace, dw, n_items,
                       g->C / 4, wp.splits, (long)g->K * 16 * (g->C / 4));
    NNL_CHECK_LAUNCH();
    return NNL_OK;
  }
  if (wgrad_wino_ok(g)) {
    const WgradPlan wp = plan_wgrad_wino(g);
    nnl_prof_exec_frac(1.0 / 1.5);
    int st2 = launch_wgrad_wino(dy, x, (float*)workspace, g, wp, s);
    if (st2) return st2;
    const long n4 = (long)g->K * 3 * (g->C / 4);
    NNL_ROUTE("wgrad_wino1d_finish");
    hipLaunchKernelGGL(wino_wgrad_finish_kernel, dim3((unsigned)nnl_cdiv(n4, 32L)), dim3(256), 0, s, (const float*)workspace, dw, n4,
                       g->C / 4, wp.splits, (long)g->K * 12 * (g->C / 4));
    NNL_CHECK_LAUNCH();
    return NNL_OK;
  }
  return launch_wgrad_direct(p, plan_wgrad(p.Mc, p.Nc, p.Kp), (float*)workspace, dw, s);
}

extern "C" size_t nnl_colsum_workspace_bytes(int64_t rows, int64_t cols) {
  if (rows <= 0 || cols <= 0) return 0;
  return (size_t)colsum_chunks(rows) * cols * sizeof(float);
}

extern "C" int nnl_act_gate_colsum(const float* dy, const float* y, float* g, float* colsum, int64_t rows, int64_t cols, int act,
                                   void* workspace, size_t workspace_bytes, void* stream) {
  NNL_CHECK_ARG(dy && y && g && rows > 0 && cols > 0 && cols < (1L << 30), "act_gate_colsum: bad argument");
  NNL_CHECK_ARG(act == 1 || act == 2, "act_gate_colsum: act must be 1 (ReLU) or 2 (sigmoid)");
  if (colsum != nullptr && (workspace == nullptr || workspace_bytes < nnl_colsum_workspace_bytes(rows, cols)))
    return nnl_set_error(NNL_ERR_WORKSPACE, "act_gate_colsum: workspace too small");
  hipStream_t s = (hipStream_t)stream;
  NnlProfScope prof(NNL_PROF_ELEMENTWISE, s, 12.0 * rows * cols);
  const int nchunk = colsum_chunks(rows);
  const long rpc = nnl_cdiv(nnl_cdiv(rows, nchunk), 4) * 4;
  const dim3 grid((unsigned)nnl_cdiv(cols, 64), nchunk);
  float* part = colsum ? (float*)workspace : nullptr;
  if (act == 1)
    hipLaunchKernelGGL(act_gate_colsum_kernel<1>, grid, dim3(256), 0, s, dy, y, g, part, (long)rows, (int)cols, rpc);
  else
    hipLaunchKernelGGL(act_gate_colsum_kernel<2>, grid, dim3(256), 0, s, dy, y, g, part, (long)rows, (int)cols, rpc);
  NNL_CHECK_LAUNCH();
  if (colsum != nullptr) {
    hipLaunchKernelGGL(colsum_final_kernel, dim3((unsigned)nnl_cdiv(cols, 16)), dim3(256), 0, s, (const float*)workspace, colsum,
                       (int)cols, nchunk);
    NNL_CHECK_LAUNCH();
  }
  return NNL_OK;
}

extern "C" int nnl_relu_gate_colsum(const float* dy, const float* y, float* g, float* colsum, int64_t rows, int64_t cols,
                                    void* workspace, size_t workspace_bytes, void* stream) {
  return nnl_act_gate_colsum(dy, y, g, colsum, rows, cols, 1, workspace, workspace_bytes, stream);
}

namespace {
struct SumN { const float* src[8]; };
__global__ __launch_bounds__(256) void sum_tensors_kernel(SumN p, int n, float* __restrict__ out, long numel) {
  const long i = ((long)blockIdx.x * 256 + threadIdx.x) * 4;
  if (i + 3 < numel) {
    f32x4 v[8];
#pragma unroll
    for (int k = 0; k < 8; ++k) if (k < n) v[k] = *reinterpret_cast<const f32x4*>(p.src[k] + i);
    f32x4 acc = v[0];
#pragma unroll
    for (int k = 1; k < 8; ++k) if (k < n) acc += v[k];
    *reinterpret_cast<f32x4*>(out + i) = acc;
  } else {
    for (long j = i; j < numel; ++j) {
      float acc = p.src[0][j];
      for (int k = 1; k < n; ++k) acc += p.src[k][j];
      out[j] = acc;
    }
  }
}
}

extern "C" int nnl_sum_tensors(const float* const* src, int n, float* out, int64_t numel, void* stream) {
  NNL_CHECK_ARG(src && out && n >= 1 && n <= 8 && numel > 0, "sum_tensors: 1 to 8 tensors of numel > 0 elements");
  SumN p{};
  for (int k = 0; k < n; ++k) {
    NNL_CHECK_ARG(src[k] != nullptr && ((uintptr_t)src[k] & 15) == 0, "sum_tensors: null or unaligned source");
    p.src[k] = src[k];
  }
  NNL_CHECK_ARG(((uintptr_t)out & 15) == 0, "sum_tensors: unaligned destination");
  hipStream_t s = (hipStream_t)stream;
  NnlProfScope prof(NNL_PROF_ELEMENTWISE, s, 4.0 * (n + 1) * numel);
  hipLaunchKernelGGL(sum_tensors_kernel, dim3((unsigned)nnl_cdiv(nnl_cdiv(numel, 4L), 256L)), dim3(256), 0, s, p, n, out, (long)numel);
  NNL_CHECK_LAUNCH();
  return NNL_OK;
}

extern "C" int nnl_colsum(const float* a, float* out, int64_t rows, int64_t cols, void* workspace, size_t workspace_bytes,
                          void* stream) {
  NNL_CHECK_ARG(a && out && rows > 0 && cols > 0 && cols < (1L << 30), "colsum: bad argument");
  if (workspace == nullptr || workspace_bytes < nnl_colsum_workspace_bytes(rows, cols))
    return nnl_set_error(NNL_ERR_WORKSPACE, "colsum: workspace too small");
  hipStream_t s = (hipStream_t)stream;
  NnlProfScope prof(NNL_PROF_ELEMENTWISE, s, 4.0 * rows * cols);
  const int nchunk = colsum_chunks(rows);
  const long rpc = nnl_cdiv(nnl_cdiv(rows, nchunk), 4) * 4;
  hipLaunchKernelGGL(colsum_partial_kernel, dim3((unsigned)nnl_cdiv(cols, 64), nchunk), dim3(256), 0, s, a, (float*)workspace,
                     (long)rows, (int)cols, rpc);
  NNL_CHECK_LAUNCH();
  hipLaunchKernelGGL(colsum_final_kernel, dim3((unsigned)nnl_cdiv(cols, 16)), dim3(256), 0, s, (const float*)workspace, out, (int)cols,
                     nchunk);
  NNL_CHECK_LAUNCH();
  return NNL_OK;
}
```

### neuralnetworklibrary_amd/csrc/igemm_wgrad.h

```cpp
#pragma once
#include "igemm_taps.h"

struct IgemmWgradParams {
  unsigned long long* dbg_t;
  const float* a;
  const float* b;
  float* y;
  unsigned a_bytes, b_bytes;
  int H, W, C, P, Q;
  int R, S, stride, pad;
  int Mc, Nc, Kp;
  int splits, k_per_split, grid_m, grid_n;
  int n_fast;
};

template <int BM, int BN, int BK, int WGM, int WGN, bool PIPE = false, int KG = 1, bool WINO = false, bool PAIR = false>
__global__ __launch_bounds__(256 * KG, KG > 1 ? 1 : ((BM * BN >= 128 * 128) ? 3 : 4)) void igemm_wgrad_kernel(const IgemmWgradParams p) {
  static_assert(WGM * WGN == 4, "4 waves per group");
  static_assert(KG == 1 || (size_t)KG * 2 * BK * (BM + BN) >= (size_t)BM * BN, "the staging LDS must hold one accumulator tile for the group reduction");
  static_assert(!PAIR || (!WINO && BK * BM / 8 >= 256 && BK * BN / 8 >= 256), "PAIR: two chunks per thread on both operands");
  constexpr int NCH = PAIR ? 2 : 1;
  constexpr int CA = BM / (4 * NCH), CB = BN / (4 * NCH);
  constexpr int RA = 256 / CA, RB = 256 / CB;
  constexpr int PA = BK / RA, PB = BK / RB;
  static_assert(PA >= 1 && PB >= 1 && BK % RA == 0 && BK % RB == 0, "tile/thread mapping");
  constexpr int WTM = BM / WGM, WTN = BN / WGN;
  constexpr int TM = WTM / 32, TN = WTN / 32;

  extern __shared__ __attribute__((aligned(16))) float lds_dyn[];
  typedef float StageBuf[BK * (BM + BN)];
  const int kg = KG > 1 ? __builtin_amdgcn_readfirstlane((int)threadIdx.x >> 8) : 0;
  StageBuf* lds = reinterpret_cast<StageBuf*>(lds_dyn) + kg * 2;
  const int tid = threadIdx.x & 255, lane = tid & 63, wave = tid >> 6;
  const int wm = wave / WGN, wn = wave % WGN;
#ifdef NNL_TAPS_TIMING
  unsigned long long* const dbg_t = (p.dbg_t != nullptr && blockIdx.x < 3276 && threadIdx.x < 256) ? p.dbg_t + (long)blockIdx.x * 5 : nullptr;
  if (dbg_t && threadIdx.x == 0) {
    dbg_t[0] = wall_clock64();
    dbg_t[4] = ((unsigned long long)__builtin_amdgcn_s_getreg((31 << 11) | 20) << 32) | (unsigned)__builtin_amdgcn_s_getreg((31 << 11) | 4);
  }
#endif
  const int tiles = p.grid_m * p.grid_n;
  const int lb = nnl_xcd_remap((int)blockIdx.x, (int)gridDim.x);
  const int split = lb / tiles;
  const int t_id = lb - split * tiles;
  const int tile_n = p.n_fast ? t_id % p.grid_n : t_id / p.grid_m;
  const int tile_m = p.n_fast ? t_id / p.grid_n : t_id - tile_n * p.grid_m;
  const int m0 = tile_m * BM, n0 = tile_n * BN;
  int k_begin = split * p.k_per_split;
  int k_end = min(k_begin + p.k_per_split, p.Kp);
  int nk = (k_end - k_begin + BK - 1) / BK;
  if constexpr (KG > 1) {
    const int sub = ((p.k_per_split / KG + BK - 1) / BK) * BK;
    nk = sub / BK;
    k_begin = min(k_begin + kg * sub, k_end);
    k_end = min(k_begin + sub, k_end);
  }

  const __amdgpu_buffer_rsrc_t ra_src = __builtin_amdgcn_make_buffer_rsrc(const_cast<float*>(p.a), 0, (int)p.a_bytes, 0x00020000);
  const __amdgpu_buffer_rsrc_t rb_src = __builtin_amdgcn_make_buffer_rsrc(const_cast<float*>(p.b), 0, (int)p.b_bytes, 0x00020000);

  const int ca = tid % CA, ra_row = tid / CA;
  const int a_col = m0 + ca * 4;
  const bool a_cok = a_col < p.Mc;
  const int cb = tid % CB, rb_row = tid / CB;
  const int b_col = n0 + cb * 4;
  const bool b_cok = b_col < p.Nc;
  const int btap = (b_cok ? b_col : 0) / p.C;
  const int bc = (b_cok ? b_col : 0) - btap * p.C;
  const int br = WINO ? btap % 3 : btap / p.S, bs = WINO ? 0 : btap - br * p.S;
  const int PQ = p.P * p.Q;
  const int xi = WINO ? n0 / (3 * p.C) : 0;
  const int wca = xi, wcb = xi < 2 ? 2 : 1;
  const float bsgn = xi == 1 ? 1.f : -1.f;
  const float ac0 = xi == 3 ? 0.f : 1.f, ac1 = xi == 0 ? 0.f : (xi == 2 ? -1.f : 1.f);
  const int dh = br - p.pad, dw = WINO ? wca - 1 : bs - p.pad;
  const int qstep = WINO ? 2 : p.stride;

  f32x4 ra[PA], rb[PB];
  f32x4 ra2[WINO ? PA : 1], rb2[WINO ? PB : 1];
  f32x4 rah[PAIR ? PA : 1], rbh[PAIR ? PB : 1];
  const int adv_n = BK / PQ, adv_r = BK - adv_n * PQ, adv_p = adv_r / p.Q, adv_q = adv_r - adv_p * p.Q;
  const int step_px = qstep * p.C * 4;
  const int step_row = p.stride * p.W * p.C * 4;
  const int off_adv = adv_n * p.H * p.W * p.C * 4 + adv_p * step_row + adv_q * step_px;
  const int off_qwrap = step_row - p.Q * step_px;
  const int off_pwrap = p.H * p.W * p.C * 4 - p.P * step_row;
  const int pp_lo = dh < 0 ? (-dh + p.stride - 1) / p.stride : 0, qq_lo = dw < 0 ? (-dw + qstep - 1) / qstep : 0;
  const int pp_hi = min(p.P, (p.H - dh + p.stride - 1) / p.stride), qq_hi = min(p.Q, (p.W - dw + qstep - 1) / qstep);
  const unsigned pp_span = pp_hi > pp_lo ? (unsigned)(pp_hi - pp_lo) : 0u, qq_span = qq_hi > qq_lo ? (unsigned)(qq_hi - qq_lo) : 0u;
  const int dw2 = wcb - 1;
  const int q2_lo = dw2 < 0 ? 1 : 0, q2_hi = min(p.Q, (p.W - dw2 + 1) / 2);
  const unsigned q2_span = q2_hi > q2_lo ? (unsigned)(q2_hi - q2_lo) : 0u;
  const int delta_b = (wcb - wca) * p.C * 4;
  int a_k[PA]; unsigned a_off[PA];
  int b_k[PB], b_pp[PB], b_qq[PB], b_off[PB];
#pragma unroll
  for (int i = 0; i < PA; ++i) {
    a_k[i] = k_begin + ra_row + i * RA;
    a_off[i] = WINO ? (unsigned)(2 * a_k[i] * p.Mc + a_col) * 4u : (unsigned)(a_k[i] * p.Mc + a_col) * 4u;
  }
#pragma unroll
  for (int i = 0; i < PB; ++i) {
    const int k = k_begin + rb_row + i * RB;
    const int n = k / PQ, rem = k - n * PQ;
    b_k[i] = k; b_pp[i] = rem / p.Q; b_qq[i] = rem - b_pp[i] * p.Q;
    b_off[i] = (((n * p.H + b_pp[i] * p.stride + dh) * p.W + b_qq[i] * qstep + dw) * p.C + bc) * 4;
  }
  auto advance = [&]() {
#pragma unroll
    for (int i = 0; i < PA; ++i) { a_k[i] += BK; a_off[i] += (unsigned)((WINO ? 2 : 1) * BK * p.Mc) * 4u; }
#pragma unroll
    for (int i = 0; i < PB; ++i) {
      b_k[i] += BK;
      int qq = b_qq[i] + adv_q, pp = b_pp[i] + adv_p, off = b_off[i] + off_adv;
      const bool qw = qq >= p.Q;
      qq -= qw ? p.Q : 0; pp += qw ? 1 : 0; off += qw ? off_qwrap : 0;
      const bool pw = pp >= p.P;
      pp -= pw ? p.P : 0; off += pw ? off_pwrap : 0;
      b_qq[i] = qq; b_pp[i] = pp; b_off[i] = off;
    }
  };
  auto load_tile = [&]() {
    if constexpr (WINO) {
#pragma unroll
      for (int i = 0; i < PA; ++i) {
        const unsigned o = (a_cok && a_k[i] < k_end) ? a_off[i] : 0xFFFFFFFFu;
        ra[i] = buf_load4(ra_src, ac0 != 0.f ? o : 0xFFFFFFFFu, 0);
        ra2[i] = buf_load4(ra_src, ac1 != 0.f ? o : 0xFFFFFFFFu, (unsigned)p.Mc * 4u);
      }
#pragma unroll
      for (int i = 0; i < PB; ++i) {
        const bool okp = b_cok && b_k[i] < k_end && (unsigned)(b_pp[i] - pp_lo) < pp_span;
        rb[i] = buf_load4(rb_src, (okp && (unsigned)(b_qq[i] - qq_lo) < qq_span) ? (unsigned)b_off[i] : 0xFFFFFFFFu, 0);
        rb2[i] = buf_load4(rb_src, (okp && (unsigned)(b_qq[i] - q2_lo) < q2_span) ? (unsigned)(b_off[i] + delta_b) : 0xFFFFFFFFu, 0);
      }
      return;
    }
#pragma unroll
    for (int i = 0; i < PA; ++i) {
      const unsigned o = (a_cok && a_k[i] < k_end) ? a_off[i] : 0xFFFFFFFFu;
      ra[i] = buf_load4(ra_src, o, 0);
      if constexpr (PAIR) rah[i] = buf_load4(ra_src, o, (unsigned)(BM / 2 * 4));
    }
#pragma unroll
    for (int i = 0; i < PB; ++i) {
      const bool ok = b_cok && b_k[i] < k_end && (unsigned)(b_pp[i] - pp_lo) < pp_span && (unsigned)(b_qq[i] - qq_lo) < qq_span;
      const unsigned o = ok ? (unsigned)b_off[i] : 0xFFFFFFFFu;
      rb[i] = buf_load4(rb_src, o, 0);
      if constexpr (PAIR) rbh[i] = buf_load4(rb_src, o, (unsigned)(BN / 2 * 4));
    }
  };
  auto store_tile = [&](int buf) {
    float* As = lds[buf];
    float* Bs = As + BK * BM;
    if constexpr (WINO) {
#pragma unroll
      for (int i = 0; i < PA; ++i) {
        f32x4 v;
#pragma unroll
        for (int e = 0; e < 4; ++e) v[e] = ac0 * ra[i][e] + ac1 * ra2[i][e];
        *reinterpret_cast<f32x4*>(As + (ra_row + i * RA) * BM + ca * 4) = v;
      }
#pragma unroll
      for (int i = 0; i < PB; ++i) {
        f32x4 v;
#pragma unroll
        for (int e = 0; e < 4; ++e) v[e] = rb[i][e] + bsgn * rb2[i][e];
        *reinterpret_cast<f32x4*>(Bs + (rb_row + i * RB) * BN + cb * 4) = v;
      }
      return;
    }
#pragma unroll
    for (int i = 0; i < PA; ++i) {
      *reinterpret_cast<f32x4*>(As + (ra_row + i * RA) * BM + ca * 4) = ra[i];
      if constexpr (PAIR) *reinterpret_cast<f32x4*>(As + (ra_row + i * RA) * BM + BM / 2 + ca * 4) = rah[i];
    }
#pragma unroll
    for (int i = 0; i < PB; ++i) {
      *reinterpret_cast<f32x4*>(Bs + (rb_row + i * RB) * BN + cb * 4) = rb[i];
      if constexpr (PAIR) *reinterpret_cast<f32x4*>(Bs + (rb_row + i * RB) * BN + BN / 2 + cb * 4) = rbh[i];
    }
  };

  f32x16 acc[TM][TN];
#pragma unroll
  for (int i = 0; i < TM; ++i)
#pragma unroll
    for (int j = 0; j < TN; ++j)
#pragma unroll
      for (int e = 0; e < 16; ++e) acc[i][j][e] = 0.f;

  const int l31 = lane & 31, lh = lane >> 5;
  auto compute = [&](int buf) {
    const float* As = lds[buf] + lh * BM + wm * WTM + l31;
    const float* Bs = lds[buf] + BK * BM + lh * BN + wn * WTN + l31;
    if constexpr (PIPE) {
      float af[2][TM], bf[2][TN];
#pragma unroll
      for (int i = 0; i < TM; ++i) af[0][i] = As[i * 32];
#pragma unroll
      for (int j = 0; j < TN; ++j) bf[0][j] = Bs[j * 32];
#pragma unroll
      for (int kk = 0; kk < BK / 2; ++kk) {
        const int c = kk & 1, n = c ^ 1;
        if (kk + 1 < BK / 2) {
#pragma unroll
          for (int i = 0; i < TM; ++i) af[n][i] = As[(kk + 1) * 2 * BM + i * 32];
#pragma unroll
          for (int j = 0; j < TN; ++j) bf[n][j] = Bs[(kk + 1) * 2 * BN + j * 32];
          __builtin_amdgcn_sched_barrier(0);
        }
#pragma unroll
        for (int i = 0; i < TM; ++i)
#pragma unroll
          for (int j = 0; j < TN; ++j)
            acc[i][j] = __builtin_amdgcn_mfma_f32_32x32x2f32(af[c][i], bf[c][j], acc[i][j], 0, 0, 0);
      }
      return;
    }
#pragma unroll
    for (int kk = 0; kk < BK / 2; ++kk) {
      float af[TM], bf[TN];
#pragma unroll
      for (int i = 0; i < TM; ++i) af[i] = As[kk * 2 * BM + i * 32];
#pragma unroll
      for (int j = 0; j < TN; ++j) bf[j] = Bs[kk * 2 * BN + j * 32];
#pragma unroll
      for (int i = 0; i < TM; ++i)
#pragma unroll
        for (int j = 0; j < TN; ++j)
          acc[i][j] = __builtin_amdgcn_mfma_f32_32x32x2f32(af[i], bf[j], acc[i][j], 0, 0, 0);
    }
  };

  if (nk > 0) {
    load_tile();
    store_tile(0);
    __syncthreads();
    NNL_TSTAMP(1);
    int cur = 0;
    for (int kt = 0; kt < nk; ++kt) {
      if (kt + 1 < nk) advance();
      load_tile();
      __builtin_amdgcn_sched_barrier(0);
      compute(cur);
      __builtin_amdgcn_sched_barrier(0);
      store_tile(cur ^ 1);
      __syncthreads();
      cur ^= 1;
    }
  }

  NNL_TSTAMP(2);
  if constexpr (KG > 1) {
    float* scratch = lds_dyn;
    for (int g = 1; g < KG; ++g) {
      if (kg == g) {
#pragma unroll
        for (int i = 0; i < TM; ++i)
#pragma unroll
          for (int j = 0; j < TN; ++j)
#pragma unroll
            for (int e = 0; e < 16; ++e) scratch[((i * TN + j) * 16 + e) * 256 + tid] = acc[i][j][e];
      }
      __syncthreads();
      if (kg == 0) {
#pragma unroll
        for (int i = 0; i < TM; ++i)
#pragma unroll
          for (int j = 0; j < TN; ++j)
#pragma unroll
            for (int e = 0; e < 16; ++e) acc[i][j][e] += scratch[((i * TN + j) * 16 + e) * 256 + tid];
      }
      __syncthreads();
    }
    if (kg != 0) return;
  }
  float* out = p.y + (long)split * p.Mc * p.Nc;
  const int row_h = lh * 4;
#pragma unroll
  for (int j = 0; j < TN; ++j) {
    const int col = n0 + wn * WTN + j * 32 + l31;
#pragma unroll
    for (int i = 0; i < TM; ++i) {
#pragma unroll
      for (int e = 0; e < 16; ++e) {
        const int row = m0 + wm * WTM + i * 32 + (e & 3) + 8 * (e >> 2) + row_h;
        if (col < p.Nc && row < p.Mc) out[(long)row * p.Nc + col] = acc[i][j][e];
      }
    }
  }
#ifdef NNL_TAPS_TIMING
  asm volatile("s_waitcnt vmcnt(0)" ::: "memory");
  NNL_TSTAMP(3);
#endif
}
```

### neuralnetworklibrary_amd/csrc/igemm_wgrad2d.h

```cpp
#pragma once
#include "igemm_taps.h"

struct IgemmWgrad2dParams {
  const float* a;
  const float* b;
  float* y;
  unsigned a_bytes, b_bytes;
  int H, W, C, H2, W2;
  int Mc, Nc, Kp;
  int splits, k_per_split, grid_m, grid_n;
  int n_fast;
};

template <int BT, int BK, int KG>
__global__ __launch_bounds__(256 * KG, KG > 1 ? 1 : (BT >= 128 ? 2 : 3)) void igemm_wgrad2d_kernel(const IgemmWgrad2dParams p) {
  static_assert(KG == 1 || (size_t)KG * 2 * BK * (2 * BT) >= (size_t)BT * BT, "the staging LDS must hold one accumulator tile for the group reduction");
  constexpr int NCH = (BK * BT / 8 >= 256) ? 2 : 1;
  constexpr int CA = BT / (4 * NCH), RA = 256 / CA, PA = BK / RA, C2 = BT / 2;
  static_assert(PA >= 1 && BK % RA == 0, "tile/thread mapping");
  constexpr int WT = BT / 2, TM = WT / 32, TN = WT / 32;
  extern __shared__ __attribute__((aligned(16))) float lds_dyn[];
  typedef float StageBuf[BK * 2 * BT];
  const int kg = KG > 1 ? __builtin_amdgcn_readfirstlane((int)threadIdx.x >> 8) : 0;
  StageBuf* lds = reinterpret_cast<StageBuf*>(lds_dyn) + kg * 2;
  const int tid = threadIdx.x & 255, lane = tid & 63, wave = tid >> 6;
  const int wm = wave >> 1, wn = wave & 1;
  const int tiles = p.grid_m * p.grid_n;
  const int lb = nnl_xcd_remap((int)blockIdx.x, (int)gridDim.x);
  const int split = lb / tiles;
  const int t_id = lb - split * tiles;
  const int tile_n = p.n_fast ? t_id % p.grid_n : t_id / p.grid_m;
  const int tile_m = p.n_fast ? t_id / p.grid_n : t_id - tile_n * p.grid_m;
  const int m0 = tile_m * BT, n0 = tile_n * BT;
  int k_begin = split * p.k_per_split;
  int k_end = min(k_begin + p.k_per_split, p.Kp);
  int nk = (k_end - k_begin + BK - 1) / BK;
  if constexpr (KG > 1) {
    const int sub = ((p.k_per_split / KG + BK - 1) / BK) * BK;
    nk = sub / BK;
    k_begin = min(k_begin + kg * sub, k_end);
    k_end = min(k_begin + sub, k_end);
  }
  const __amdgpu_buffer_rsrc_t ra_src = __builtin_amdgcn_make_buffer_rsrc(const_cast<float*>(p.a), 0, (int)p.a_bytes, 0x00020000);
  const __amdgpu_buffer_rsrc_t rb_src = __builtin_amdgcn_make_buffer_rsrc(const_cast<float*>(p.b), 0, (int)p.b_bytes, 0x00020000);

  const int pos = n0 / p.C, xi = pos >> 2, nu = pos & 3;
  const float cp0 = xi < 3 ? 1.f : 0.f, cp1 = xi == 0 ? 0.f : (xi == 2 ? -1.f : 1.f);
  const float cq0 = nu < 3 ? 1.f : 0.f, cq1 = nu == 0 ? 0.f : (nu == 2 ? -1.f : 1.f);
  const float a00 = cp0 * cq0, a01 = cp0 * cq1, a10 = cp1 * cq0, a11 = cp1 * cq1;
  const int rb_ = xi < 2 ? 2 : 1, cb_ = nu < 2 ? 2 : 1;
  const float sr = xi == 1 ? 1.f : -1.f, sc = nu == 1 ? 1.f : -1.f;

  const int ca = tid % CA, row0 = tid / CA;
  const int a_col = m0 + ca * 4, b_col = n0 - pos * p.C + ca * 4;
  const bool a_cok = a_col < p.Mc;
  const int a_px = p.Mc * 4, a_row = p.W * p.Mc * 4, b_px = p.C * 4, b_row = p.W * p.C * 4;
  const int bd00 = xi * b_row + nu * b_px, bd01 = xi * b_row + cb_ * b_px, bd10 = rb_ * b_row + nu * b_px, bd11 = rb_ * b_row + cb_ * b_px;

  const int HW2 = p.H2 * p.W2;
  const int adv_n = BK / HW2, adv_r = BK - adv_n * HW2, adv_i = adv_r / p.W2, adv_j = adv_r - adv_i * p.W2;
  const int a_adv = adv_n * p.H * a_row + adv_i * 2 * a_row + adv_j * 2 * a_px, b_adv = adv_n * p.H * b_row + adv_i * 2 * b_row + adv_j * 2 * b_px;
  const int a_jwrap = 2 * a_row - p.W2 * 2 * a_px, b_jwrap = 2 * b_row - p.W2 * 2 * b_px;
  const int a_iwrap = p.H * a_row - p.H2 * 2 * a_row, b_iwrap = p.H * b_row - p.H2 * 2 * b_row;
  int r_k[PA], r_i[PA], r_j[PA], a_off[PA], b_off[PA];
#pragma unroll
  for (int s = 0; s < PA; ++s) {
    const int k = k_begin + row0 + s * RA;
    const int n = k / HW2, rem = k - n * HW2;
    const int qi = rem / p.W2, qj = rem - qi * p.W2;
    r_k[s] = k; r_i[s] = 2 * qi; r_j[s] = 2 * qj;
    a_off[s] = ((n * p.H + 2 * qi) * p.W + 2 * qj) * a_px + a_col * 4;
    b_off[s] = ((n * p.H + 2 * qi - 1) * p.W + 2 * qj - 1) * b_px + b_col * 4;
  }
  const int adv_i2 = 2 * adv_i, adv_j2 = 2 * adv_j, W22 = 2 * p.W2, H22 = 2 * p.H2;
  auto advance = [&]() {
#pragma unroll
    for (int s = 0; s < PA; ++s) {
      r_k[s] += BK;
      int j = r_j[s] + adv_j2, i = r_i[s] + adv_i2, ao = a_off[s] + a_adv, bo = b_off[s] + b_adv;
      const bool jw = j >= W22;
      j -= jw ? W22 : 0; i += jw ? 2 : 0; ao += jw ? a_jwrap : 0; bo += jw ? b_jwrap : 0;
      const bool iw = i >= H22;
      i -= iw ? H22 : 0; ao += iw ? a_iwrap : 0; bo += iw ? b_iwrap : 0;
      r_j[s] = j; r_i[s] = i; a_off[s] = ao; b_off[s] = bo;
    }
  };
  f32x4 ra[PA][NCH][4], rb[PA][NCH][4];
  auto load_tile = [&]() {
#pragma unroll
    for (int s = 0; s < PA; ++s) {
      const bool ok = r_k[s] < k_end;
      const int i2 = r_i[s], j2 = r_j[s];
      const bool okA = ok && a_cok, h1 = i2 < p.H - 1, w1 = j2 < p.W - 1;
      const unsigned ao = (unsigned)a_off[s];
      const unsigned a0 = (a00 != 0.f && okA) ? ao : 0xFFFFFFFFu, a1 = (a01 != 0.f && okA && w1) ? ao : 0xFFFFFFFFu;
      const unsigned a2 = (a10 != 0.f && okA && h1) ? ao : 0xFFFFFFFFu;
      const unsigned a3 = (a11 != 0.f && okA && h1 && w1) ? ao : 0xFFFFFFFFu;
      const bool ra_ok = (unsigned)(i2 - 1 + xi) < (unsigned)p.H, rb_ok = (unsigned)(i2 - 1 + rb_) < (unsigned)p.H;
      const bool ca_ok = (unsigned)(j2 - 1 + nu) < (unsigned)p.W, cb_ok = (unsigned)(j2 - 1 + cb_) < (unsigned)p.W;
      const unsigned b0 = (ok && ra_ok && ca_ok) ? (unsigned)(b_off[s] + bd00) : 0xFFFFFFFFu;
      const unsigned b1 = (ok && ra_ok && cb_ok) ? (unsigned)(b_off[s] + bd01) : 0xFFFFFFFFu;
      const unsigned b2 = (ok && rb_ok && ca_ok) ? (unsigned)(b_off[s] + bd10) : 0xFFFFFFFFu;
      const unsigned b3 = (ok && rb_ok && cb_ok) ? (unsigned)(b_off[s] + bd11) : 0xFFFFFFFFu;
#pragma unroll
      for (int h = 0; h < NCH; ++h) {
        const unsigned so = (unsigned)(h * C2 * 4);
        ra[s][h][0] = buf_load4(ra_src, a0, so); ra[s][h][1] = buf_load4(ra_src, a1, so + (unsigned)a_px);
        ra[s][h][2] = buf_load4(ra_src, a2, so + (unsigned)a_row); ra[s][h][3] = buf_load4(ra_src, a3, so + (unsigned)(a_row + a_px));
        rb[s][h][0] = buf_load4(rb_src, b0, so); rb[s][h][1] = buf_load4(rb_src, b1, so);
        rb[s][h][2] = buf_load4(rb_src, b2, so); rb[s][h][3] = buf_load4(rb_src, b3, so);
      }
    }
  };
  auto store_tile = [&](int buf) {
    float* As = lds[buf];
    float* Bs = As + BK * BT;
#pragma unroll
    for (int s = 0; s < PA; ++s) {
      f32x4 va[NCH], vb[NCH];
#pragma unroll
      for (int h = 0; h < NCH; ++h) va[h] = ra[s][h][0];
      if (a01 != 0.f) {
        asm volatile("" ::: "memory");
#pragma unroll
        for (int h = 0; h < NCH; ++h)
#pragma unroll
          for (int e = 0; e < 4; ++e) va[h][e] = __builtin_fmaf(a01, ra[s][h][1][e], va[h][e]);
      }
      if (a10 != 0.f) {
        asm volatile("" ::: "memory");
#pragma unroll
        for (int h = 0; h < NCH; ++h)
#pragma unroll
          for (int e = 0; e < 4; ++e) va[h][e] = __builtin_fmaf(a10, ra[s][h][2][e], va[h][e]);
      }
      if (a11 != 0.f) {
        asm volatile("" ::: "memory");
#pragma unroll
        for (int h = 0; h < NCH; ++h)
#pragma unroll
          for (int e = 0; e < 4; ++e) va[h][e] = __builtin_fmaf(a11, ra[s][h][3][e], va[h][e]);
      }
#pragma unroll
      for (int h = 0; h < NCH; ++h) {
#pragma unroll
        for (int e = 0; e < 4; ++e)
          vb[h][e] = __builtin_fmaf(sr, __builtin_fmaf(sc, rb[s][h][3][e], rb[s][h][2][e]), __builtin_fmaf(sc, rb[s][h][1][e], rb[s][h][0][e]));
        *reinterpret_cast<f32x4*>(As + (row0 + s * RA) * BT + h * C2 + ca * 4) = va[h];
        *reinterpret_cast<f32x4*>(Bs + (row0 + s * RA) * BT + h * C2 + ca * 4) = vb[h];
      }
    }
  };

  f32x16 acc[TM][TN];
#pragma unroll
  for (int i = 0; i < TM; ++i)
#pragma unroll
    for (int j = 0; j < TN; ++j)
#pragma unroll
      for (int e = 0; e < 16; ++e) acc[i][j][e] = 0.f;
  const int l31 = lane & 31, lh = lane >> 5;
  auto compute = [&](int buf) {
    const float* As = lds[buf] + lh * BT + wm * WT + l31;
    const float* Bs = lds[buf] + BK * BT + lh * BT + wn * WT + l31;
    float af[2][TM], bf[2][TN];
#pragma unroll
    for (int i = 0; i < TM; ++i) af[0][i] = As[i * 32];
#pragma unroll
    for (int j = 0; j < TN; ++j) bf[0][j] = Bs[j * 32];
#pragma unroll
    for (int kk = 0; kk < BK / 2; ++kk) {
      const int c = kk & 1, n = c ^ 1;
      if (kk + 1 < BK / 2) {
#pragma unroll
        for (int i = 0; i < TM; ++i) af[n][i] = As[(kk + 1) * 2 * BT + i * 32];
#pragma unroll
        for (int j = 0; j < TN; ++j) bf[n][j] = Bs[(kk + 1) * 2 * BT + j * 32];
        __builtin_amdgcn_sched_barrier(0);
      }
#pragma unroll
      for (int i = 0; i < TM; ++i)
#pragma unroll
        for (int j = 0; j < TN; ++j)
          acc[i][j] = __builtin_amdgcn_mfma_f32_32x32x2f32(af[c][i], bf[c][j], acc[i][j], 0, 0, 0);
    }
  };

  if (nk > 0) {
    load_tile();
    store_tile(0);
    __syncthreads();
    int cur = 0;
    for (int kt = 0; kt < nk; ++kt) {
      if (kt + 1 < nk) advance();
      load_tile();
      __builtin_amdgcn_sched_barrier(0);
      compute(cur);
      __builtin_amdgcn_sched_barrier(0);
      store_tile(cur ^ 1);
      __syncthreads();
      cur ^= 1;
    }
  }
  if constexpr (KG > 1) {
    float* scratch = lds_dyn;
    for (int g = 1; g < KG; ++g) {
      if (kg == g) {
#pragma unroll
        for (int i = 0; i < TM; ++i)
#pragma unroll
          for (int j = 0; j < TN; ++j)
#pragma unroll
            for (int e = 0; e < 16; ++e) scratch[((i * TN + j) * 16 + e) * 256 + tid] = acc[i][j][e];
      }
      __syncthreads();
      if (kg == 0) {
#pragma unroll
        for (int i = 0; i < TM; ++i)
#pragma unroll
          for (int j = 0; j < TN; ++j)
#pragma unroll
            for (int e = 0; e < 16; ++e) acc[i][j][e] += scratch[((i * TN + j) * 16 + e) * 256 + tid];
      }
      __syncthreads();
    }
    if (kg != 0) return;
  }
  float* out = p.y + (long)split * p.Mc * p.Nc;
  const int row_h = lh * 4;
#pragma unroll
  for (int j = 0; j < TN; ++j) {
    const int col = n0 + wn * WT + j * 32 + l31;
#pragma unroll
    for (int i = 0; i < TM; ++i) {
#pragma unroll
      for (int e = 0; e < 16; ++e) {
        const int row = m0 + wm * WT + i * 32 + (e & 3) + 8 * (e >> 2) + row_h;
        if (col < p.Nc && row < p.Mc) out[(long)row * p.Nc + col] = acc[i][j][e];
      }
    }
  }
}
```

### neuralnetworklibrary_amd/ops.py

```python
import collections
import contextlib
import ctypes
import os
import weakref

import numpy as np
import torch

from . import _lib
from ._lib import check, lib, ptr, require_cuda, stream

__all__ = ['mse_loss', 'bce_with_logits', 'fbeta', 'scaled_sigmoid', 'embdotbias', 'index_error_flag', 'raise_if_index_error', 'conv2d', 'to_nhwc', 'from_nhwc', 'linear', 'bn_act', 'concat_pool2d', 'TabularPlan', 'tab_embed_concat', 'embedding_renorm_drop', 'retina_loss', 'image_aug']

_ERR_FLAGS = {}


def _flags(device):
    key = (device.type, device.index)
    if key not in _ERR_FLAGS:
        _ERR_FLAGS[key] = torch.zeros(2, dtype=torch.int32, device=device)
    return _ERR_FLAGS[key]


def index_error_flag(device):
# ... 98 lines not shown
class _BCEWithLogits(torch.autograd.Function):

    @staticmethod
    def forward(ctx, input, target):
        require_cuda(input, target)
        x, t = _f32c(input).reshape(-1), _f32c(target).reshape(-1)
        n = x.numel()
        loss = torch.empty((), dtype=torch.float32, device=x.device)
        wsb = int(lib.nnl_bce_logits_workspace_bytes(n))
        ws = _workspace(wsb, x.device)
        check(lib.nnl_bce_logits_fwd(ptr(x), ptr(t), ptr(loss), n, ptr(ws), wsb, stream()))
        ctx.save_for_backward(x, t)
        ctx.shape = input.shape
        return loss

    @staticmethod
    def backward(ctx, dloss):
        x, t = ctx.saved_tensors
        g = _f32c(dloss).reshape(1)
        dx = torch.empty_like(x)
        check(lib.nnl_bce_logits_bwd(ptr(x), ptr(t), ptr(g), ptr(dx), x.numel(), stream()))
        return dx.view(ctx.shape), None


def bce_with_logits(input, target):
    return _BCEWithLogits.apply(input, target)


def fbeta(pred, target, beta, threshold=0.5, use_thresh=True, eps=1e-9):
    require_cuda(pred, target)
    p, t = _f32c(pred.detach()), _f32c(target.detach())
    if p.dim() != 2 or p.shape != t.shape or p.numel() == 0:
        raise ValueError('fbeta: pred and target must be non-empty [N, C] tensors of one shape (got %s, %s)' % (tuple(pred.shape), tuple(target.shape)))
    N, C = p.shape
    out = torch.empty((), dtype=torch.float32, device=p.device)
    wsb = int(lib.nnl_fbeta_workspace_bytes(N, C))
    ws = _workspace(wsb, p.device)
    check(lib.nnl_fbeta(ptr(p), ptr(t), ptr(out), N, C, float(beta) ** 2, float(threshold), int(bool(use_thresh)), float(eps), ptr(ws), wsb, stream()))
    return out


class _ScaledSigmoid(torch.autograd.Function):

    @staticmethod
    def forward(ctx, x, lo, hi):
        require_cuda(x)
        xc = _f32c(x)
        y, sg = torch.empty_like(xc), torch.empty_like(xc)
        check(lib.nnl_scaled_sigmoid_fwd(ptr(xc), ptr(y), ptr(sg), xc.numel(), float(lo), float(hi), stream()))
        ctx.save_for_backward(sg)
        ctx.rng = (float(lo), float(hi))
        return y

    @staticmethod
    def backward(ctx, dy):
        sg, = ctx.saved_tensors
        dyc = _f32c(dy)
        dx = torch.empty_like(sg)
        check(lib.nnl_scaled_sigmoid_bwd(ptr(dyc), ptr(sg), ptr(dx), sg.numel(), ctx.rng[0], ctx.rng[1], stream()))
        return dx, None, None


def scaled_sigmoid(x, lo, hi):
    return _ScaledSigmoid.apply(x, float(lo), float(hi))


def embdotbias(x, U, M, bu, bi, output_range=None):
    lo, hi = (None, None) if output_range is None else (float(output_range[0]), float(output_range[1]))
    return _EmbDotBias.apply(x, U, M, bu, bi, lo, hi)


def to_nhwc(x):
    return x.permute(0, 2, 3, 1).contiguous()


def from_nhwc(x):
    return x.permute(0, 3, 1, 2)


def _geom(N, H, W, C, K, R, S, stride, pad):
    P = (H + 2 * pad - R) // stride + 1
    Q = (W + 2 * pad - S) // stride + 1
    return _lib.ConvGeom(N, H, W, C, K, R, S, stride, pad, P, Q)


def _pad_c4(t_nhwc):
    C = t_nhwc.shape[-1]
    if C % 4 == 0:
        return t_nhwc
    if t_nhwc.is_cuda and t_nhwc.dtype == torch.float32 and t_nhwc.is_contiguous() and not (torch.is_grad_enabled() and t_nhwc.requires_grad):
        Cp = C + 4 - C % 4
        out = torch.empty(t_nhwc.shape[:-1] + (Cp,), dtype=torch.float32, device=t_nhwc.device)
        check(lib.nnl_pad_cols(ptr(t_nhwc), ptr(out), t_nhwc.numel() // C, C, Cp, stream()))
        return out
    return torch.nn.functional.pad(t_nhwc, (0, 4 - C % 4))


_OPEN = None


def _wino_u_numel(rows, ch, mode):
    return rows * 16 * ch if mode == 2 else rows * 12 * ch


class _FilterBatch:

    def __init__(self, key, dev, entry, desc_dtype, items, extra=()):
        self.key, self.entry, self.extra = key, entry, extra
        sizes = [int(np.prod(shape)) for _, shape, _, _ in items]
        self.flat = torch.empty(sum(sizes), dtype=torch.float32, device=dev)
        desc = np.zeros(len(items), dtype=desc_dtype)
        block_desc, self.views, off = [], {}, 0
        for i, ((k, shape, nb, row), n) in enumerate(zip(items, sizes)):
            v = self.views[k] = self.flat[off:off + n].view(shape)
            off += n
            desc[i] = row(v.data_ptr(), len(block_desc))
            block_desc += [i] * nb
        self.n_blocks = len(block_desc)
        self.desc = torch.from_numpy(desc.view(np.uint8).copy()).to(dev)
        self.block_desc = torch.tensor(block_desc, dtype=torch.int32, device=dev)

    def run(self):
        check(getattr(lib, self.entry)(ptr(self.desc), ptr(self.block_desc), self.n_blocks, *self.extra, stream()))


def _wino_batch(key, srcs):
    def item(k, t, flip, mode):
        rows, ch = t.shape[0], t.shape[3]
        nb = (rows * ch + 255) // 256 if mode == 2 else (rows * 3 * ch + 255) // 256
        return (k, mode), (_wino_u_numel(rows, ch, mode),), nb, lambda dst, first: (t.data_ptr(), dst, rows, ch, flip, first, 1 if mode == 2 else 0, 0)
    dtype = np.dtype([('src', '<u8'), ('dst', '<u8'), ('rows', '<i4'), ('ch', '<i4'), ('flip', '<i4'), ('first', '<i4'), ('two_d', '<i4'), ('reserved', '<i4')])
    return _FilterBatch(key, srcs[0][1].device, 'nnl_wino_filter_multi', dtype, [item(*s) for s in srcs])


def _wt_batch(key, weights):
    def item(w):
        K, C, R, S = w.shape
        return w.data_ptr(), (C, R, S, K), R * S * ((K + 31) // 32) * ((C + 31) // 32), lambda dst, first: (w.data_ptr(), dst, K, R * S, C, first)
    dtype = np.dtype([('w', '<u8'), ('wt', '<u8'), ('K', '<i4'), ('RS', '<i4'), ('C', '<i4'), ('first', '<i4')])
    return _FilterBatch(key, weights[0].device, 'nnl_conv2d_weight_transpose_multi', dtype, [item(w) for w in weights],
                        (float(sum(w.numel() for w in weights)),))


class _Filters:

    def __init__(self, model):
        self.mods = [m for m in model.modules() if getattr(m, 'nnl_hip_conv', False)]
        self.step = 0
        self.modes = {}
        self.batches = {}
        self.u = ({}, {})
        self.wt = {}
        self.wt_padded = {}

    def open(self):
        global _OPEN
        finish_backward()
        self.step += 1
        _OPEN = self

    def recorded(self, key_ptr, which):
        return self.modes[key_ptr][which][1] if key_ptr in self.modes else ()

    def _run(self, slot, key, build, *args):
        batch = self.batches.get(slot)
        if batch is None or batch.key != key:
            if torch.cuda.is_current_stream_capturing():
                return None
            batch = self.batches[slot] = build(key, *args)
        batch.run()
        return batch

    def _run_wino(self, which, srcs):
        if srcs and os.environ.get('NNL_WINO_PREPARE', '1') != '0':
            batch = self._run(('fwd', 'bwd')[which], tuple((k, t.data_ptr(), tuple(t.shape), mode) for k, t, _, mode in srcs), _wino_batch, srcs)
            if batch is not None:
                self.u[which].update(batch.views)

    def prepare_forward(self):
        self.open()
        srcs = []
        for m in self.mods:
            w = m.weight
            modes = self.recorded(w.data_ptr(), 0)
            if (modes and w.is_cuda and w.dim() == 4 and w.shape[2] == 3 and w.shape[3] == 3 and w.dtype == torch.float32
                    and w.is_contiguous(memory_format=torch.channels_last)):
                srcs += [(w.data_ptr(), w.permute(0, 2, 3, 1), 0, mode) for mode in sorted(modes)]
        self._run_wino(0, srcs)

    def prepare_backward(self):
        if _OPEN is not self:
            self.open()
        ws = [m.weight for m in self.mods
              if m.weight.is_cuda and m.weight.dim() == 4 and m.weight.shape[1] % 4 == 0
              and m.weight.shape[0] % 4 == 0 and m.weight.dtype == torch.float32
              and m.weight.is_contiguous(memory_format=torch.channels_last)]
        if len(ws) < 2 or sum(w.requires_grad for w in ws) * 2 < len(ws):
            return
        batch = self._run('wt', tuple((w.data_ptr(), tuple(w.shape)) for w in ws), _wt_batch, ws)
        if batch is not None:
            self.wt.update(batch.views)
            self._run_wino(1, [(w.data_ptr(), batch.views[w.data_ptr()], 1, mode) for w in ws if w.shape[2] == 3 and w.shape[3] == 3
                               for mode in sorted(self.recorded(w.data_ptr(), 1))])

    def wino(self, key_ptr, which, g):
        if _OPEN is not self or not key_ptr:
            return None
        mode = int(lib.nnl_conv2d_wino_preferred(g, which)) if (g.R == 3 and g.S == 3 and g.stride == 1) else 0
        if mode or key_ptr in self.modes:
            e = self.modes.setdefault(key_ptr, [[-1, set()], [-1, set()]])[which]
            if e[0] != self.step:
                e[0], e[1] = self.step, set()
            if mode:
                e[1].add(mode)
        u = self.u[which].get((key_ptr, mode)) if mode else None
        rows, ch = (g.C, g.K) if which else (g.K, g.C)
        return u if u is not None and u.numel() == _wino_u_numel(rows, ch, mode) else None


_CLOSED = _Filters(torch.nn.Module())


def _filters(model):
    if getattr(model, '_nnl_filters', None) is None:
        object.__setattr__(model, '_nnl_filters', _Filters(model))
    return model._nnl_filters


def prepare_forward(model):
    _filters(model).prepare_forward()


def prepare_backward(model):
    _filters(model).prepare_backward()


def finish_backward():
    global _OPEN
    if _OPEN is not None:
        for views in (*_OPEN.u, _OPEN.wt, _OPEN.wt_padded):
            views.clear()
        _OPEN = None


def prepared_batches(model):
    return tuple(_filters(model).batches.values())


def prepared_filter_counts():
    f = _OPEN or _CLOSED
    return len(f.u[0]), len(f.u[1]), len(f.wt)


@contextlib.contextmanager
def filter_window(model):
    def backward(loss):
        prepare_backward(model)
        loss.backward()
    prepare_forward(model)
    try:
        yield backward
    finally:
        finish_backward()


_PADDED_GRADS = {}


def register_padded_grad(base, ld):
    if len(_PADDED_GRADS) > 64:
        for k in [k for k, (r, _) in _PADDED_GRADS.items() if r() is None]:
            del _PADDED_GRADS[k]
    _PADDED_GRADS[id(base)] = (weakref.ref(base), int(ld))


def _padded_rows(dy, K):
    base = dy._base if dy._is_view() else None
    ent = _PADDED_GRADS.get(id(base)) if base is not None else None
    if ent is None or ent[0]() is not base or dy.dim() != 4 or dy.shape[2] != 1 or dy.shape[3] != 1:
        return None
    ld = ent[1]
    if dy.dtype != torch.float32 or dy.stride(1) != 1 or dy.stride(0) != ld or ld < K or ld % 16 != 0 or dy.storage_offset() % ld != 0:
        return None
    if dy.storage_offset() + dy.shape[0] * ld > base.numel():
        return None
    return torch.as_strided(base, (dy.shape[0], 1, 1, ld), (ld, ld, ld, 1), dy.storage_offset())


_TILE_COUNTERS = {}


def _tile_counters(device):
    t = _TILE_COUNTERS.get(device.index)
    if t is None:
        if torch.cuda.is_current_stream_capturing():
            return None
        t = _TILE_COUNTERS[device.index] = torch.zeros(int(lib.nnl_conv2d_tile_counters()), dtype=torch.int32, device=device)
    return t


class GradSlot:
    __slots__ = ('tensor', 'closed')

    def __init__(self):
        self.tensor = None
        self.closed = False



_FAN = {}


class _FanOut(torch.autograd.Function):
    @staticmethod
    def forward(ctx, p, n):
        ctx.n = n
        return tuple(p.detach().view(p.shape) for _ in range(n))

    @staticmethod
    def backward(ctx, *grads):
        have = [g for g in grads if g is not None]
        if not have:
            return None, None
        if len(have) == 1:
            return have[0], None
        g0 = have[0]
        dense = all(g.is_cuda and g.dtype == torch.float32 and g.shape == g0.shape and g.stride() == g0.stride() and g.data_ptr() % 16 == 0
                    and (g.is_contiguous() or (g.dim() == 4 and g.is_contiguous(memory_format=torch.channels_last))) for g in have)
        if not dense or len(have) > 8:
            out = have[0]
            for g in have[1:]:
                out = out + g
            return out, None
        out = torch.empty_like(g0)
        arr = (ctypes.c_void_p * len(have))(*[g.data_ptr() for g in have])
        check(lib.nnl_sum_tensors(arr, len(have), ptr(out), g0.numel(), stream()))
        return out, None


class shared_params:

    def __init__(self, modules, n):
        self.modules, self.n, self.keys = modules, int(n), []

    def __enter__(self):
        if self.n > 1 and torch.is_grad_enabled():
            for m in self.modules:
                for p in m.parameters():
                    if p.requires_grad and p.is_cuda and id(p) not in _FAN:
                        _FAN[id(p)] = list(_FanOut.apply(p, self.n))
                        self.keys.append(id(p))
        return self

    def __exit__(self, *exc):
        for k in self.keys:
            _FAN.pop(k, None)
        return False


def fan_param(p):
    if p is None or not _FAN:
        return p
    lst = _FAN.get(id(p))
    return lst.pop(0) if lst else p


_ConvState = collections.namedtuple('_ConvState', 'g relu has_bias c_in w_layout slot give_slot grad_dst uses')


def _conv_operands(x, weight, bias, stride, pad):
    xn = _pad_c4(to_nhwc(_f32c(x) if x.dim() != 4 else x.float()))
    wn = _pad_c4(to_nhwc(weight.float()))
    N, H, W, C = xn.shape
    K, R, S, _ = wn.shape
    g = _geom(N, H, W, C, K, R, S, stride, pad)
    y = torch.empty((N, g.P, g.Q, K), dtype=torch.float32, device=x.device)
    return xn, wn, (None if bias is None else _f32c(bias)), g, y


def _conv_state(x, weight, bias, g, relu, slot=None, give_slot=None):
    uses = getattr(weight, '_nnl_uses', None)
    if uses is not None:
        uses[0] += 1
    return _ConvState(g, relu, bias is not None, x.shape[1], (tuple(weight.shape), tuple(weight.stride())), slot, give_slot,
                      getattr(weight, '_nnl_grad_dst', None), uses)


def _with_k(g, K):
    return _geom(g.N, g.H, g.W, g.C, K, g.R, g.S, g.stride, g.pad)


def _conv_backward(st, xn, wn, y, dy, needs):
    if dy is None:
        return None, None, None
    g, K = st.g, st.g.K
    want_db = st.has_bias and needs[2]
    db = None
    pre = _padded_rows(dy, K) if (not st.relu and g.R == 1 and g.S == 1 and g.H == 1 and g.W == 1) else None
    if pre is not None and pre.shape[-1] != K:
        dy4 = pre
    else:
        dy4 = to_nhwc(dy.float())
        if st.relu:
            dy4, db = _conv_act_gate(y, dy4, g, st.relu, want_db)
        if K % 4 != 0:
            dy4 = _pad_c4(dy4)
    w4, g4 = wn, g
    if dy4.shape[-1] != K:
        w4, g4 = torch.nn.functional.pad(wn, (0, 0, 0, 0, 0, 0, 0, dy4.shape[-1] - K)), _with_k(g, dy4.shape[-1])
    dx = dw = None
    if needs[0]:
        dx = _conv_dgrad(st, dy4, w4, g4, K)
    elif st.slot is not None:
        st.slot.tensor, st.slot.closed = None, True
    if needs[1]:
        dw = _conv_wgrad(st, xn, dy4, g4, K)
    if db is None and want_db:
        db = _conv_bias_grad(dy4, g4, K)
    return dx, dw, db


def _conv_act_gate(y, dyn, g, relu, want_db):
    rows = g.N * g.P * g.Q
    gated = torch.empty_like(dyn)
    cb = int(lib.nnl_colsum_workspace_bytes(rows, g.K)) if want_db else 0
    cws = _workspace(cb, dyn.device, floor=True) if want_db else None
    db = torch.empty(g.K, dtype=torch.float32, device=dyn.device) if want_db else None
    check(lib.nnl_act_gate_colsum(ptr(dyn), ptr(y), ptr(gated), ptr(db), rows, g.K, int(relu), ptr(cws), cb, stream()))
    return gated, db


def _conv_dgrad_operands(dy4, w4, g4, K):
    ktail = g4.R == 1 and g4.S == 1 and g4.K % 4 == 0 and os.environ.get('NNL_IGEMM_KTAIL', '1') != '0'
    dyd, gd, padk, wkey = dy4, g4, 0, None
    f = _OPEN or _CLOSED
    if g4.K % 16 != 0 and g4.K >= 32 and not ktail:
        padk = 16 - g4.K % 16
        dyd, gd = torch.nn.functional.pad(dy4, (0, padk)), _with_k(g4, g4.K + padk)
        wkey = (w4.data_ptr(), tuple(w4.shape), padk)
        wt = f.wt_padded.get(wkey) if f.wt else None
    else:
        wt = f.wt.get(w4.data_ptr()) if g4.K == K else None
        if wt is not None and tuple(wt.shape) != (g4.C, g4.R, g4.S, g4.K):
            wt = None
    if wt is None:
        wd = torch.nn.functional.pad(w4, (0, 0, 0, 0, 0, 0, 0, padk)) if padk else w4
        wt = torch.empty((gd.C, gd.R, gd.S, gd.K), dtype=torch.float32, device=dy4.device)
        check(lib.nnl_conv2d_weight_transpose(ptr(wd), ptr(wt), gd.K, gd.R, gd.S, gd.C, stream()))
        if wkey is not None and f.wt:
            f.wt_padded[wkey] = wt
    return dyd, wt, gd


def _conv_dgrad(st, dy4, w4, g4, K):
    dyd, wt, g = _conv_dgrad_operands(dy4, w4, g4, K)
    dxn = torch.empty((g.N, g.H, g.W, g.C), dtype=torch.float32, device=dyd.device)
    wsb = int(lib.nnl_conv2d_dgrad_workspace_bytes(g))
    dws = _workspace(wsb, dyd.device)
    shortcut = None
    if st.slot is not None:
        shortcut, st.slot.tensor, st.slot.closed = st.slot.tensor, None, True
    fuse = shortcut is not None and g.K % 16 == 0 and g.R * g.S <= 49 and shortcut.numel() == dxn.numel() \
        and ((g.stride == 1 and (g.S <= 32 or g.pad <= 127)) or (g.stride == 2 and g.R == 3 and g.S == 3 and g.pad == 1))
    u = (_OPEN or _CLOSED).wino(w4.data_ptr() if g.K == K else 0, 1, g)
    check(lib.nnl_conv2d_dgrad_pre(ptr(dyd), ptr(wt), ptr(dxn), g, ptr(shortcut) if fuse else None, ptr(dws), wsb,
                                   ptr(_tile_counters(dyd.device) if wsb else None), ptr(u), stream()))
    if shortcut is not None and not fuse:
        dxn += shortcut.view_as(dxn)
    give = st.give_slot
    if give is not None and not give.closed and st.c_in == g.C:
        give.tensor = dxn
        return None
    return from_nhwc(dxn[..., :st.c_in] if st.c_in != g.C else dxn)


def _conv_wgrad(st, xn, dy4, g4, K):
    dst = st.grad_dst
    if dst is not None and st.uses is not None and st.uses[0] == 1 and dst.dim() == 4 and g4.K == K and st.c_in == g4.C \
            and dst.permute(0, 2, 3, 1).is_contiguous() and tuple(dst.shape) == (g4.K, g4.C, g4.R, g4.S):
        dwn = dst.permute(0, 2, 3, 1)
    else:
        dwn = torch.empty((g4.K, g4.R, g4.S, g4.C), dtype=torch.float32, device=dy4.device)
    wsb = int(lib.nnl_conv2d_wgrad_workspace_bytes(g4))
    ws = _workspace(wsb, dy4.device, floor=True)
    check(lib.nnl_conv2d_wgrad(ptr(xn), ptr(dy4), ptr(dwn), g4, ptr(ws), wsb, stream()))
    dw = from_nhwc(dwn[:K, :, :, :st.c_in])
    wshape, wstride = st.w_layout
    if (g4.R == 1 and g4.S == 1 and wshape == tuple(dw.shape) and wstride != tuple(dw.stride()) and dw.is_contiguous(memory_format=torch.channels_last)
            and wstride[1] == 1 and wstride[0] == dw.shape[1]):
        dw = dw.as_strided(wshape, wstride)
    return dw


def _conv_bias_grad(dy4, g4, K):
    rows = g4.N * g4.P * g4.Q
    db_full = torch.empty(g4.K, dtype=torch.float32, device=dy4.device)
    cb = int(lib.nnl_colsum_workspace_bytes(rows, g4.K))
    cws = _workspace(cb, dy4.device, floor=True)
    check(lib.nnl_colsum(ptr(dy4), ptr(db_full), rows, g4.K, ptr(cws), cb, stream()))
    return db_full[:K]


class _Conv2d(torch.autograd.Function):

    @staticmethod
    def forward(ctx, x, weight, bias, stride, pad, relu, slot=None, bn_pivot=None, give_slot=None):
        require_cuda(x, weight, bias)
        xn, wn, b, g, y = _conv_operands(x, weight, bias, stride, pad)
        N, K = g.N, g.K
        ctx.st = _conv_state(x, weight, bias, g, relu, slot, give_slot)
        wsb = int(lib.nnl_conv2d_fwd_workspace_bytes(g))
        ws = _workspace(wsb, x.device)
        part, rows = None, _lib.i32(0)
        if bn_pivot is not None:
            part = torch.empty(((N * g.P * g.Q + 63) // 64) * K * 2, dtype=torch.float32, device=x.device)
        u = (_OPEN or _CLOSED).wino(wn.data_ptr(), 0, g)
        check(lib.nnl_conv2d_fwd_pre(ptr(xn), ptr(wn), ptr(b), ptr(y), g, int(relu), ptr(ws), wsb, ptr(_tile_counters(x.device) if wsb else None),
                                     ptr(part), ptr(bn_pivot), ctypes.byref(rows) if part is not None else None, ptr(u), stream()))
        if part is None or rows.value == 0:
            part = torch.empty(0, dtype=torch.float32, device=x.device)
        else:
            part = part[:rows.value * K * 2]
        ctx.mark_non_differentiable(part)
        ctx.set_materialize_grads(False)
        ctx.save_for_backward(xn, wn, y if relu else None)
        return from_nhwc(y), part

    @staticmethod
    def backward(ctx, dy, _dpart=None):
        xn, wn, y = ctx.saved_tensors
        return _conv_backward(ctx.st, xn, wn, y, dy, ctx.needs_input_grad[:3]) + (None,) * 6


def _conv(x, weight, bias, *, stride=1, pad=0, relu=0, slot=None, bn_pivot=None, give_slot=None):
    return _Conv2d.apply(x, weight, bias, int(stride), int(pad), int(relu), slot, bn_pivot, give_slot)


def conv2d(x, weight, bias=None, stride=1, pad=0, relu=False, grad_slot=None, give_slot=None):
    return _conv(x, weight, bias, stride=stride, pad=pad, relu=relu, slot=grad_slot, give_slot=give_slot)[0]


class _ConvAddUp2(torch.autograd.Function):

    @staticmethod
    def forward(ctx, x, weight, bias, small, stride, pad):
        require_cuda(x, weight, bias, small)
        xn, wn, b, g, y = _conv_operands(x, weight, bias, stride, pad)
        sn = to_nhwc(small.float())
        ctx.small_shape = (g.N, g.P // 2, g.Q // 2, g.K)
        if tuple(sn.shape) != ctx.small_shape or g.P % 2 or g.Q % 2:
            raise _lib.NnlError('conv_add_upsampled: `small` %s is not [N, K, P/2, Q/2] of the %dx%d output' % (tuple(small.shape), g.P, g.Q))
        ctx.st = _conv_state(x, weight, bias, g, 0)
        check(lib.nnl_conv2d_fwd_add_up2(ptr(xn), ptr(wn), ptr(b), ptr(sn), ptr(y), g, stream()))
        ctx.save_for_backward(xn, wn)
        return from_nhwc(y)

    @staticmethod
    def backward(ctx, dy):
        dsmall = None
        if ctx.needs_input_grad[3]:
            dyn = to_nhwc(dy.float())
            N, h, w, K = ctx.small_shape
            ds = torch.empty(ctx.small_shape, dtype=torch.float32, device=dy.device)
            check(lib.nnl_upsample2_bwd(ptr(dyn), ptr(ds), N, h, w, K, stream()))
            dsmall = from_nhwc(ds)
        xn, wn = ctx.saved_tensors
        return _conv_backward(ctx.st, xn, wn, None, dy, ctx.needs_input_grad[:3]) + (dsmall, None, None)


def conv_add_upsampled(x, weight, bias, small, stride=1, pad=0):
    return _ConvAddUp2.apply(x, weight, bias, small, int(stride), int(pad))


def conv2d_with_bn_stats(x, weight, bias, stride, pad, bn_pivot, grad_slot=None, give_slot=None):
    return _conv(x, weight, bias, stride=stride, pad=pad, slot=grad_slot, bn_pivot=bn_pivot, give_slot=give_slot)


def _rows_in_place(x):
    return x.dtype == torch.float32 and x.dim() == 2 and x.stride(1) == 1 and x.stride(0) >= x.shape[1]


class _LinearSmall(torch.autograd.Function):

    @staticmethod
    def forward(ctx, x, weight, bias):
        require_cuda(x, weight, bias)
        x = x if _rows_in_place(x) else _f32c(x)
        w = _f32c(weight)
        b = None if bias is None else _f32c(bias)
        M, K = x.shape
        N = w.shape[0]
        y = torch.empty(M, N, dtype=torch.float32, device=x.device)
        check(lib.nnl_linear_small_fwd(ptr(x), ptr(w), ptr(b), ptr(y), M, K, x.stride(0) if M > 1 else K, N, stream()))
        ctx.save_for_backward(x, w)
        ctx.has_bias = bias is not None
        return y

    @staticmethod
    def backward(ctx, dy):
        x, w = ctx.saved_tensors
        M, K = x.shape
        N = w.shape[0]
        dy = _f32c(dy)
        dev = dy.device
        dx = torch.empty(M, K, dtype=torch.float32, device=dev) if ctx.needs_input_grad[0] else None
        dw = torch.empty(N, K, dtype=torch.float32, device=dev) if ctx.needs_input_grad[1] else None
        db = torch.empty(N, dtype=torch.float32, device=dev) if (ctx.has_bias and ctx.needs_input_grad[2]) else None
        wsb = int(lib.nnl_linear_small_bwd_workspace_bytes(M, K, N)) if (dw is not None or db is not None) else 0
        ws = _workspace(wsb, dev)
        check(lib.nnl_linear_small_bwd(ptr(dy), ptr(x), ptr(w), ptr(dx), ptr(dw), ptr(db), M, K, x.stride(0) if M > 1 else K, N, ptr(ws), wsb,
                                       stream()))
        return dx, dw, db


def linear(x, weight, bias=None, relu=False):
    lead = x.shape[:-1]
    x2 = x.reshape(-1, x.shape[-1])
    if not relu and weight.shape[0] <= 4 and x2.is_cuda and x2.shape[0] > 0:
        return _LinearSmall.apply(x2, weight, bias).reshape(*lead, weight.shape[0])
    y = _conv(x2[:, :, None, None], weight[:, :, None, None], bias, relu=relu)[0]
    return y.reshape(*lead, weight.shape[0])


def _rows_view(x):
    if x.dim() == 4:
        xn = to_nhwc(x.float())
        N, H, W, C = xn.shape
        return xn.view(-1, C), (lambda m: from_nhwc(m.view(N, H, W, C)))
    if x.dim() == 2:
        return _f32c(x), (lambda m: m)
    if x.dim() == 3:
        xn = x.float().permute(0, 2, 1).contiguous()
        N, L, C = xn.shape
        return xn.view(-1, C), (lambda m: m.view(N, L, C).permute(0, 2, 1))
    raise ValueError('bn_act: unsupported input rank %d' % x.dim())


def _relu_mask(rows, C, device):
    return torch.empty((rows * C + 31) // 32 + 2, dtype=torch.int32, device=device)


def _bn_grad_buffers(ctx, xm, gamma, has_res):
    dx = torch.empty_like(xm)
    dres = torch.empty_like(xm) if (has_res and ctx.needs_input_grad[1]) else None
# ... 1020 lines not shown
```

Baseline: 5567 images/s.

## Defer conv weight-gradient kernels and launch them as grouped multi-problem kernels

During backward, conv weight-gradient computations are queued instead of launched immediately. At the end of backward, or when a per-kernel-variant queue fills or a memory cap is hit, they are flushed as single grouped launches, one per kernel variant, with the split-K reduce and finish steps also batched into multi-item kernels. The aim is to cut per-layer launch overhead and small-grid underutilization for ResNet-34's many wgrad calls. In exchange, dy and x buffers stay alive until the flush, which raises peak memory. It also adds bookkeeping for weight use counts and copying gradients when the handed-out tensor differs.

```diff
diff --git a/include/nnl.h b/include/nnl.h
--- a/include/nnl.h
+++ b/include/nnl.h
@@ -93,6 +93,16 @@
 size_t nnl_conv2d_wgrad_workspace_bytes(const nnl_conv_geom_t* g);
 int nnl_conv2d_wgrad(const float* x, const float* dy, float* dw, const nnl_conv_geom_t* g, void* workspace,
                      size_t workspace_bytes, void* stream);
+typedef struct {
+  const float* x;
+  const float* dy;
+  float* dw;
+  nnl_conv_geom_t g;
+  void* workspace;
+  size_t workspace_bytes;
+} nnl_wgrad_item_t;
+int nnl_conv2d_wgrad_group_key(const nnl_conv_geom_t* g);
+int nnl_conv2d_wgrad_group(const nnl_wgrad_item_t* items, int n, void* stream);
 size_t nnl_colsum_workspace_bytes(int64_t rows, int64_t cols);
 int nnl_sum_tensors(const float* const* src, int n, float* out, int64_t numel, void* stream);
 int nnl_colsum(const float* a, float* out, int64_t rows, int64_t cols, void* workspace, size_t workspace_bytes,
diff --git a/neuralnetworklibrary_amd/_lib.py b/neuralnetworklibrary_amd/_lib.py
--- a/neuralnetworklibrary_amd/_lib.py
+++ b/neuralnetworklibrary_amd/_lib.py
@@ -21,6 +21,10 @@
 class ConvGeom(C.Structure):
     _fields_ = [('N', i32), ('H', i32), ('W', i32), ('C', i32), ('K', i32), ('R', i32), ('S', i32),
                 ('stride', i32), ('pad', i32), ('P', i32), ('Q', i32)]
+
+
+class WgradItem(C.Structure):
+    _fields_ = [('x', c_p), ('dy', c_p), ('dw', c_p), ('g', ConvGeom), ('workspace', c_p), ('workspace_bytes', sz)]
 
 
 SIGNATURES = {
@@ -59,6 +63,8 @@
     'nnl_conv2d_dgrad': (C.c_int, [c_p, c_p, c_p, C.POINTER(ConvGeom), c_p, c_p, sz, c_p, c_p]),
     'nnl_conv2d_wgrad_workspace_bytes': (sz, [C.POINTER(ConvGeom)]),
     'nnl_conv2d_wgrad': (C.c_int, [c_p, c_p, c_p, C.POINTER(ConvGeom), c_p, sz, c_p]),
+    'nnl_conv2d_wgrad_group_key': (C.c_int, [C.POINTER(ConvGeom)]),
+    'nnl_conv2d_wgrad_group': (C.c_int, [C.POINTER(WgradItem), C.c_int, c_p]),
     'nnl_colsum_workspace_bytes': (sz, [i64, i64]),
     'nnl_colsum': (C.c_int, [c_p, c_p, i64, i64, c_p, sz, c_p]),
     'nnl_relu_gate_colsum': (C.c_int, [c_p, c_p, c_p, c_p, i64, i64, c_p, sz, c_p]),
diff --git a/neuralnetworklibrary_amd/csrc/conv2d.hip b/neuralnetworklibrary_amd/csrc/conv2d.hip
--- a/neuralnetworklibrary_amd/csrc/conv2d.hip
+++ b/neuralnetworklibrary_amd/csrc/conv2d.hip
@@ -1,3 +1,5 @@
+#include <algorithm>
+#include <vector>
 #include "igemm_kernels.h"
 #include "igemm_taps.h"
 #include "wino.h"
@@ -306,11 +308,10 @@
   }
 }
 
-__global__ __launch_bounds__(256) void splitk_reduce_kernel(const float* __restrict__ part, float* __restrict__ out, long n4,
-                                                             int splits) {
+__device__ __forceinline__ void splitk_reduce_body(const float* __restrict__ part, float* __restrict__ out, long n4, int splits, long blk) {
   __shared__ f32x4 red[8][32];
   const int col = threadIdx.x & 31, sl = threadIdx.x >> 5;
-  const long i = (long)blockIdx.x * 32 + col;
+  const long i = blk * 32 + col;
   f32x4 acc = {0.f, 0.f, 0.f, 0.f};
   if (i < n4) {
     int s = sl;
@@ -329,6 +330,38 @@
     for (int l = 1; l < 8; ++l) t += red[l][col];
     reinterpret_cast<f32x4*>(out)[i] = t;
   }
+}
+
+__global__ __launch_bounds__(256) void splitk_reduce_kernel(const float* __restrict__ part, float* __restrict__ out, long n4,
+                                                             int splits) {
+  splitk_reduce_body(part, out, n4, splits, (long)blockIdx.x);
+}
+
+constexpr int NNL_REDUCE_GROUP_MAX = 32;
+struct ReduceItem {
+  const float* part;
+  float* dw;
+  long n;
+  long slab4;
+  int C4, splits;
+};
+struct ReduceGroup {
+  int n;
+  int start[NNL_REDUCE_GROUP_MAX + 1];
+  ReduceItem it[NNL_REDUCE_GROUP_MAX];
+};
+__device__ __forceinline__ int reduce_group_find(const ReduceGroup& g, int bid, long& local) {
+  int idx = 0;
+#pragma unroll
+  for (int i = 1; i < NNL_REDUCE_GROUP_MAX; ++i) idx += bid >= g.start[i] ? 1 : 0;
+  local = bid - g.start[idx];
+  return idx;
+}
+
+__global__ __launch_bounds__(256) void splitk_reduce_multi(const ReduceGroup g) {
+  long blk;
+  const ReduceItem& q = g.it[reduce_group_find(g, (int)blockIdx.x, blk)];
+  splitk_reduce_body(q.part, q.dw, q.n, q.splits, blk);
 }
 
 __global__ __launch_bounds__(256) void colsum_partial_kernel(const float* __restrict__ a, float* __restrict__ part, long rows,
@@ -497,7 +530,7 @@
   });
 }
 
-int launch_wgrad_v2(const IgemmKmajorParams& p, long a_elems, long b_elems, const WgradPlan& pl, hipStream_t s) {
+IgemmWgradParams wgrad_v2_params(const IgemmKmajorParams& p, long a_elems, long b_elems, const WgradPlan& pl) {
   IgemmWgradParams q{};
   q.a = p.a; q.b = p.b; q.y = p.y;
   q.a_bytes = (unsigned)(a_elems * 4); q.b_bytes = (unsigned)(b_elems * 4);
@@ -513,10 +546,24 @@
     const long fp_n = nnl_cdiv(T, gn) * pl.bm + (T < gn ? T : gn) * pl.bn;
     q.n_fast = fp_n < fp_m ? 1 : 0;
   }
+  return q;
+}
+
+int wgrad_v2_plan_check(const WgradPlan& pl) {
   const bool t128 = pl.bm == 128 && pl.bn == 128, t64 = pl.bm == 64 && pl.bn == 64;
   if (!(pl.kg == 1 || (pl.kg == 4 && t128)) || (t64 && pl.k_per_split % 32 != 0))
     return nnl_set_error(NNL_ERR_UNSUPPORTED, "wgrad: no kernel for the plan <%d,%d> kg=%d k_per_split=%d", pl.bm, pl.bn, pl.kg, pl.k_per_split);
-  const bool pair = p.R * p.S == 1 || p.C % pl.bn == 0;
+  return NNL_OK;
+}
+
+bool wgrad_v2_pair(const IgemmKmajorParams& p, const WgradPlan& pl) { return p.R * p.S == 1 || p.C % pl.bn == 0; }
+
+int launch_wgrad_v2(const IgemmKmajorParams& p, long a_elems, long b_elems, const WgradPlan& pl, hipStream_t s) {
+  const IgemmWgradParams q = wgrad_v2_params(p, a_elems, b_elems, pl);
+  const int st = wgrad_v2_plan_check(pl);
+  if (st) return st;
+  const bool t128 = pl.bm == 128 && pl.bn == 128;
+  const bool pair = wgrad_v2_pair(p, pl);
   if (t128) {
     if (pl.kg == 4) return pair ? launch_wgrad_tile<128, 128, 16, true, 4, true>(q, s) : launch_wgrad_tile<128, 128, 16, true, 4, false>(q, s);
     return pair ? launch_wgrad_tile<128, 128, 16, true, 1, true>(q, s) : launch_wgrad_tile<128, 128, 16, true, 1, false>(q, s);
@@ -526,11 +573,11 @@
   return pair ? launch_wgrad_tile<64, 64, 32, true, 1, true>(q, s) : launch_wgrad_tile<64, 64, 32, true, 1, false>(q, s);
 }
 
-__global__ __launch_bounds__(256) void wino_wgrad_finish_kernel(const float* __restrict__ part, float* __restrict__ dw, long n4,
-                                                                 int C4, int splits, long slab4) {
+__device__ __forceinline__ void wino_wgrad_finish_body(const float* __restrict__ part, float* __restrict__ dw, long n4, int C4, int splits,
+                                                       long slab4, long blk) {
   __shared__ f32x4 red[8][32][4];
   const int it = threadIdx.x & 31, sl = threadIdx.x >> 5;
-  const long i = (long)blockIdx.x * 32 + it;
+  const long i = blk * 32 + it;
   f32x4 u0 = {0.f, 0.f, 0.f, 0.f}, u1 = u0, u2 = u0, u3 = u0;
   long c4 = 0, r = 0, k = 0;
   if (i < n4) {
@@ -554,6 +601,17 @@
   }
 }
 
+__global__ __launch_bounds__(256) void wino_wgrad_finish_kernel(const float* __restrict__ part, float* __restrict__ dw, long n4,
+                                                                 int C4, int splits, long slab4) {
+  wino_wgrad_finish_body(part, dw, n4, C4, splits, slab4, (long)blockIdx.x);
+}
+
+__global__ __launch_bounds__(256) void wino_wgrad_finish_multi(const ReduceGroup g) {
+  long blk;
+  const ReduceItem& q = g.it[reduce_group_find(g, (int)blockIdx.x, blk)];
+  wino_wgrad_finish_body(q.part, q.dw, q.n, q.C4, q.splits, q.slab4, blk);
+}
+
 bool wgrad_wino_ok(const nnl_conv_geom_t* g) {
   const int mode = NNL_ENV_INT("NNL_WGRAD_WINO", 1);
   if (mode == 0) return false;
@@ -569,7 +627,7 @@
   return plan_wgrad(g->K, 12 * g->C, (long)g->N * g->P * (g->Q / 2), 3 * g->C);
 }
 
-int launch_wgrad_wino(const float* dy, const float* x, float* slabs, const nnl_conv_geom_t* g, const WgradPlan& pl, hipStream_t s) {
+IgemmWgradParams wgrad_wino_params(const float* dy, const float* x, float* slabs, const nnl_conv_geom_t* g, const WgradPlan& pl) {
   IgemmWgradParams q{};
   const long pairs = (long)g->N * g->P * (g->Q / 2);
   q.a = dy; q.b = x; q.y = slabs;
@@ -578,18 +636,29 @@
   q.Mc = g->K; q.Nc = 12 * g->C; q.Kp = (int)pairs;
   q.splits = pl.splits; q.k_per_split = pl.k_per_split; q.grid_m = pl.grid_m; q.grid_n = pl.grid_n;
   q.n_fast = 1;
+  return q;
+}
+
+int wgrad_wino_plan_check(const WgradPlan& pl) {
   if (pl.kg != 1 || (pl.bm == 64 && pl.k_per_split % 32 != 0))
     return nnl_set_error(NNL_ERR_UNSUPPORTED, "wgrad_wino1d: no kernel for the plan <%d> kg=%d k_per_split=%d", pl.bm, pl.kg, pl.k_per_split);
+  return NNL_OK;
+}
+
+int launch_wgrad_wino(const float* dy, const float* x, float* slabs, const nnl_conv_geom_t* g, const WgradPlan& pl, hipStream_t s) {
+  const IgemmWgradParams q = wgrad_wino_params(dy, x, slabs, g, pl);
+  const int st = wgrad_wino_plan_check(pl);
+  if (st) return st;
   const auto note = [&] { NNL_ROUTE("wgrad_wino1d<%d,%d,kg1>@splits=%d", pl.bm, pl.bm == 128 ? 16 : 32, pl.splits); };
   if (pl.bm == 128) return launch_wave_groups<igemm_wgrad_kernel<128, 128, 16, 2, 2, true, 1, true>>(q, 1, wgrad_lds_bytes(256, 16, 1), s, note);
   return launch_wave_groups<igemm_wgrad_kernel<64, 64, 32, 2, 2, true, 1, true>>(q, 1, wgrad_lds_bytes(128, 32, 1), s, note);
 }
 
-__global__ __launch_bounds__(256) void wino2d_wgrad_finish_kernel(const float* __restrict__ part, float* __restrict__ dw, long n_items, int C4,
-                                                                   int splits, long slab4) {
+__device__ __forceinline__ void wino2d_wgrad_finish_body(const float* __restrict__ part, float* __restrict__ dw, long n_items, int C4, int splits,
+                                                         long slab4, long blk) {
   __shared__ f32x4 du[16][16];
   const int it = threadIdx.x >> 4, pos = threadIdx.x & 15;
-  const long i = (long)blockIdx.x * 16 + it;
+  const long i = blk * 16 + it;
   const long c4 = i % C4, k = i / C4;
   f32x4 u = {0.f, 0.f, 0.f, 0.f};
   if (i < n_items) {
@@ -618,6 +687,17 @@
     }
     reinterpret_cast<f32x4*>(dw)[(k * 9 + pos) * C4 + c4] = acc;
   }
+}
+
+__global__ __launch_bounds__(256) void wino2d_wgrad_finish_kernel(const float* __restrict__ part, float* __restrict__ dw, long n_items, int C4,
+                                                                   int splits, long slab4) {
+  wino2d_wgrad_finish_body(part, dw, n_items, C4, splits, slab4, (long)blockIdx.x);
+}
+
+__global__ __launch_bounds__(256) void wino2d_wgrad_finish_multi(const ReduceGroup g) {
+  long blk;
+  const ReduceItem& q = g.it[reduce_group_find(g, (int)blockIdx.x, blk)];
+  wino2d_wgrad_finish_body(q.part, q.dw, q.n, q.C4, q.splits, q.slab4, blk);
 }
 
 bool wgrad_wino2d_ok(const nnl_conv_geom_t* g) {
@@ -661,7 +741,7 @@
   return p64;
 }
 
-int launch_wgrad_wino2d(const float* dy, const float* x, float* slabs, const nnl_conv_geom_t* g, const WgradPlan& pl, hipStream_t s) {
+IgemmWgrad2dParams wgrad_wino2d_params(const float* dy, const float* x, float* slabs, const nnl_conv_geom_t* g, const WgradPlan& pl) {
   IgemmWgrad2dParams q{};
   q.a = dy; q.b = x; q.y = slabs;
   q.a_bytes = (unsigned)((long)g->N * g->H * g->W * g->K * 4); q.b_bytes = (unsigned)((long)g->N * g->H * g->W * g->C * 4);
@@ -669,8 +749,19 @@
   q.Mc = g->K; q.Nc = 16 * g->C; q.Kp = (int)((long)g->N * q.H2 * q.W2);
   q.splits = pl.splits; q.k_per_split = pl.k_per_split; q.grid_m = pl.grid_m; q.grid_n = pl.grid_n;
   q.n_fast = 1;
+  return q;
+}
+
+int wgrad_wino2d_plan_check(const WgradPlan& pl) {
   if (!(pl.kg == 1 || (pl.kg == 4 && pl.bm == 64)) || (pl.bm == 64 && pl.k_per_split % 32 != 0))
     return nnl_set_error(NNL_ERR_UNSUPPORTED, "wgrad_wino2d: no kernel for the plan <%d> kg=%d k_per_split=%d", pl.bm, pl.kg, pl.k_per_split);
+  return NNL_OK;
+}
+
+int launch_wgrad_wino2d(const float* dy, const float* x, float* slabs, const nnl_conv_geom_t* g, const WgradPlan& pl, hipStream_t s) {
+  const IgemmWgrad2dParams q = wgrad_wino2d_params(dy, x, slabs, g, pl);
+  const int st = wgrad_wino2d_plan_check(pl);
+  if (st) return st;
   const auto note = [&] { NNL_ROUTE("wgrad_wino2d<%d,%d,kg%d>@splits=%d", pl.bm, pl.bm == 128 ? 16 : 32, pl.kg, pl.splits); };
   if (pl.bm == 128) return launch_wave_groups<igemm_wgrad2d_kernel<128, 16, 1>>(q, 1, wgrad_lds_bytes(256, 16, 1), s, note);
   if (pl.kg == 4) return launch_wave_groups<igemm_wgrad2d_kernel<64, 32, 4>>(q, 4, wgrad_lds_bytes(128, 32, 4), s, note);
@@ -1107,6 +1198,227 @@
   return launch_wgrad_direct(p, plan_wgrad(p.Mc, p.Nc, p.Kp), (float*)workspace, dw, s);
 }
 
+namespace {
+
+static_assert(sizeof(WgradGroup<IgemmWgradParams>) <= 4096 && sizeof(WgradGroup<IgemmWgrad2dParams>) <= 4096 && sizeof(ReduceGroup) <= 4096,
+              "a group travels as a kernel argument");
+
+enum WgradKid {
+  KID_D128_KG4_PAIR, KID_D128_KG4, KID_D128_PAIR, KID_D128, KID_D128x64, KID_D64x128, KID_D64_PAIR, KID_D64,
+  KID_W1_128, KID_W1_64, KID_W2_128, KID_W2_64_KG4, KID_W2_64, KID_COUNT
+};
+const char* const wgrad_kid_name[KID_COUNT] = {
+  "wgrad<128,128,16,kg4>:pair", "wgrad<128,128,16,kg4>", "wgrad<128,128,16,kg1>:pair", "wgrad<128,128,16,kg1>", "wgrad<128,64,16,kg1>",
+  "wgrad<64,128,16,kg1>", "wgrad<64,64,32,kg1>:pair", "wgrad<64,64,32,kg1>",
+  "wgrad_wino1d<128,16,kg1>", "wgrad_wino1d<64,32,kg1>", "wgrad_wino2d<128,16,kg1>", "wgrad_wino2d<64,32,kg4>", "wgrad_wino2d<64,32,kg1>"};
+const char* const wgrad_reduce_name[4] = {"", "splitk_reduce", "wgrad_wino1d_finish", "wgrad_wino2d_finish"};
+
+struct WgradJob {
+  int kid;
+  int blocks;
+  IgemmWgradParams q1;
+  IgemmWgrad2dParams q2;
+  int reduce;
+  ReduceItem r;
+  int rblocks;
+};
+
+template <auto Kernel, class Params>
+int launch_group_kernel(const WgradGroup<Params>& grp, int kg, size_t lds, hipStream_t s) {
+  if (lds > 64 * 1024) {
+    static bool attr_set = false;
+    if (!attr_set) {
+      NNL_CHECK_HIP(hipFuncSetAttribute(reinterpret_cast<const void*>(Kernel), hipFuncAttributeMaxDynamicSharedMemorySize, (int)lds));
+      attr_set = true;
+    }
+  }
+  hipLaunchKernelGGL(Kernel, dim3(grp.start[grp.n]), dim3(256 * kg), lds, s, grp);
+  NNL_CHECK_LAUNCH();
+  return NNL_OK;
+}
+
+template <int BM, int BN, int BK, bool PIPE, int KG, bool WINO, bool PAIR>
+int launch_group_1d(const WgradGroup<IgemmWgradParams>& grp, hipStream_t s) {
+  return launch_group_kernel<igemm_wgrad_group_kernel<BM, BN, BK, 2, 2, PIPE, KG, WINO, PAIR>>(grp, KG, wgrad_lds_bytes(BM + BN, BK, KG), s);
+}
+template <int BT, int BK, int KG>
+int launch_group_2d(const WgradGroup<IgemmWgrad2dParams>& grp, hipStream_t s) {
+  return launch_group_kernel<igemm_wgrad2d_group_kernel<BT, BK, KG>>(grp, KG, wgrad_lds_bytes(2 * BT, BK, KG), s);
+}
+
+int launch_wgrad_group(int kid, const WgradGroup<IgemmWgradParams>& g1, const WgradGroup<IgemmWgrad2dParams>& g2, hipStream_t s) {
+  switch (kid) {
+    case KID_D128_KG4_PAIR: return launch_group_1d<128, 128, 16, true, 4, false, true>(g1, s);
+    case KID_D128_KG4:      return launch_group_1d<128, 128, 16, true, 4, false, false>(g1, s);
+    case KID_D128_PAIR:     return launch_group_1d<128, 128, 16, true, 1, false, true>(g1, s);
+    case KID_D128:          return launch_group_1d<128, 128, 16, true, 1, false, false>(g1, s);
+    case KID_D128x64:       return launch_group_1d<128, 64, 16, false, 1, false, false>(g1, s);
+    case KID_D64x128:       return launch_group_1d<64, 128, 16, true, 1, false, false>(g1, s);
+    case KID_D64_PAIR:      return launch_group_1d<64, 64, 32, true, 1, false, true>(g1, s);
+    case KID_D64:           return launch_group_1d<64, 64, 32, true, 1, false, false>(g1, s);
+    case KID_W1_128:        return launch_group_1d<128, 128, 16, true, 1, true, false>(g1, s);
+    case KID_W1_64:         return launch_group_1d<64, 64, 32, true, 1, true, false>(g1, s);
+    case KID_W2_128:        return launch_group_2d<128, 16, 1>(g2, s);
+    case KID_W2_64_KG4:     return launch_group_2d<64, 32, 4>(g2, s);
+    case KID_W2_64:         return launch_group_2d<64, 32, 1>(g2, s);
+  }
+  return nnl_set_error(NNL_ERR_UNSUPPORTED, "wgrad_group: no kernel %d", kid);
+}
+
+int launch_reduce_group(int kind, const ReduceGroup& g, hipStream_t s) {
+  const dim3 grid(g.start[g.n]), block(256);
+  if (kind == 1) hipLaunchKernelGGL(splitk_reduce_multi, grid, block, 0, s, g);
+  else if (kind == 2) hipLaunchKernelGGL(wino_wgrad_finish_multi, grid, block, 0, s, g);
+  else hipLaunchKernelGGL(wino2d_wgrad_finish_multi, grid, block, 0, s, g);
+  NNL_CHECK_LAUNCH();
+  return NNL_OK;
+}
+
+IgemmKmajorParams wgrad_direct_problem(const float* x, const float* dy, const nnl_conv_geom_t* g) {
+  IgemmKmajorParams p{};
+  p.a = dy; p.b = x;
+  p.N = g->N; p.H = g->H; p.W = g->W; p.C = g->C; p.P = g->P; p.Q = g->Q;
+  p.R = g->R; p.S = g->S; p.stride = g->stride; p.pad = g->pad;
+  p.Mc = g->K; p.Nc = g->R * g->S * g->C; p.Kp = (long)g->N * g->P * g->Q;
+  return p;
+}
+
+int plan_wgrad_job(const float* x, const float* dy, float* dw, const nnl_conv_geom_t* g, float* ws, WgradJob& j, char* note, size_t note_n) {
+  j = WgradJob{};
+  note[0] = 0;
+  WgradPlan pl;
+  if (wgrad_wino2d_ok(g)) {
+    pl = plan_wgrad_wino2d(g);
+    const int st = wgrad_wino2d_plan_check(pl);
+    if (st) return st;
+    j.q2 = wgrad_wino2d_params(dy, x, ws, g, pl);
+    j.kid = pl.bm == 128 ? KID_W2_128 : (pl.kg == 4 ? KID_W2_64_KG4 : KID_W2_64);
+    j.reduce = 3;
+    j.r.n = (long)g->K * (g->C / 4); j.r.slab4 = (long)g->K * 16 * (g->C / 4);
+    j.rblocks = (int)nnl_cdiv(j.r.n, 16L);
+    snprintf(note, note_n, "wgrad_wino2d<%d,%d,kg%d>@splits=%d", pl.bm, pl.bm == 128 ? 16 : 32, pl.kg, pl.splits);
+  } else if (wgrad_wino_ok(g)) {
+    pl = plan_wgrad_wino(g);
+    const int st = wgrad_wino_plan_check(pl);
+    if (st) return st;
+    j.q1 = wgrad_wino_params(dy, x, ws, g, pl);
+    j.kid = pl.bm == 128 ? KID_W1_128 : KID_W1_64;
+    j.reduce = 2;
+    j.r.n = (long)g->K * 3 * (g->C / 4); j.r.slab4 = (long)g->K * 12 * (g->C / 4);
+    j.rblocks = (int)nnl_cdiv(j.r.n, 32L);
+    snprintf(note, note_n, "wgrad_wino1d<%d,%d,kg1>@splits=%d", pl.bm, pl.bm == 128 ? 16 : 32, pl.splits);
+  } else {
+    IgemmKmajorParams p = wgrad_direct_problem(x, dy, g);
+    pl = plan_wgrad(p.Mc, p.Nc, p.Kp);
+    const long a_elems = p.Kp * p.Mc, b_elems = (long)p.N * p.H * p.W * p.C;
+    if (!wgrad_v2_ok(a_elems, b_elems, p.Kp)) { j.kid = -1; return NNL_OK; }
+    const int st = wgrad_v2_plan_check(pl);
+    if (st) return st;
+    p.y = pl.splits > 1 ? ws : dw;
+    j.q1 = wgrad_v2_params(p, a_elems, b_elems, pl);
+    const bool pair = wgrad_v2_pair(p, pl);
+    if (pl.bm == 128 && pl.bn == 128) j.kid = pl.kg == 4 ? (pair ? KID_D128_KG4_PAIR : KID_D128_KG4) : (pair ? KID_D128_PAIR : KID_D128);
+    else if (pl.bm == 128) j.kid = KID_D128x64;
+    else if (pl.bn == 128) j.kid = KID_D64x128;
+    else j.kid = pair ? KID_D64_PAIR : KID_D64;
+    const bool paired = j.kid == KID_D128_KG4_PAIR || j.kid == KID_D128_PAIR || j.kid == KID_D64_PAIR;
+    j.reduce = pl.splits > 1 ? 1 : 0;
+    j.r.n = (long)p.Mc * p.Nc / 4;
+    j.rblocks = (int)nnl_cdiv(j.r.n, 32L);
+    snprintf(note, note_n, "wgrad<%d,%d,%d,kg%d>%s%s@splits=%d", pl.bm, pl.bn, (pl.bm == 64 && pl.bn == 64) ? 32 : 16, pl.kg, paired ? ":pair" : "",
+             pl.splits > 1 ? ":splitk" : "", pl.splits);
+  }
+  j.blocks = pl.grid_m * pl.grid_n * pl.splits;
+  j.r.part = ws; j.r.dw = dw; j.r.C4 = g->C / 4; j.r.splits = pl.splits;
+  return NNL_OK;
+}
+
+}
+
+extern "C" int nnl_conv2d_wgrad_group_key(const nnl_conv_geom_t* g) {
+  if (!g || check_geom(g, "conv2d_wgrad_group_key") || g->K % 4 != 0) return -1;
+  WgradJob j;
+  char note[96];
+  if (plan_wgrad_job(nullptr, nullptr, nullptr, g, nullptr, j, note, sizeof(note)) != NNL_OK) return -1;
+  return j.kid;
+}
+
+extern "C" int nnl_conv2d_wgrad_group(const nnl_wgrad_item_t* items, int n, void* stream) {
+  NNL_CHECK_ARG(items != nullptr && n >= 1 && n <= 4096, "conv2d_wgrad_group: %d items", n);
+  hipStream_t s = (hipStream_t)stream;
+  std::vector<WgradJob> jobs((size_t)n);
+  double work = 0.0;
+  for (int i = 0; i < n; ++i) {
+    const nnl_wgrad_item_t& it = items[i];
+    int st = check_geom(&it.g, "conv2d_wgrad_group");
+    if (st) return st;
+    NNL_CHECK_ARG(it.x && it.dy && it.dw, "conv2d_wgrad_group: null pointer in item %d", i);
+    NNL_CHECK_ARG(it.g.K % 4 == 0, "conv2d_wgrad_group: item %d: K=%d must be a multiple of 4", i, it.g.K);
+    const size_t need = nnl_conv2d_wgrad_workspace_bytes(&it.g);
+    if (need > 0 && (it.workspace == nullptr || it.workspace_bytes < need))
+      return nnl_set_error(NNL_ERR_WORKSPACE, "conv2d_wgrad_group: item %d: workspace %zu B < required %zu B", i, it.workspace_bytes, need);
+    char note[96];
+    st = plan_wgrad_job(it.x, it.dy, it.dw, &it.g, (float*)it.workspace, jobs[i], note, sizeof(note));
+    if (st) return st;
+    if (jobs[i].kid >= 0) NNL_ROUTE("wgrad_group_item=%s", note);
+    work += 2.0 * it.g.N * it.g.P * it.g.Q * (double)it.g.K * it.g.R * it.g.S * it.g.C;
+  }
+  std::vector<int> order[KID_COUNT], red[4];
+  for (int i = 0; i < n; ++i) {
+    if (jobs[i].kid < 0) continue;
+    order[jobs[i].kid].push_back(i);
+    if (jobs[i].reduce) red[jobs[i].reduce].push_back(i);
+  }
+  for (int k = 0; k < KID_COUNT; ++k)
+    for (size_t c = 0; c < order[k].size(); c += NNL_WGRAD_GROUP_MAX)
+      NNL_ROUTE("wgrad_group<%s>@n=%d", wgrad_kid_name[k], (int)std::min<size_t>(NNL_WGRAD_GROUP_MAX, order[k].size() - c));
+  for (int k = 1; k < 4; ++k)
+    for (size_t c = 0; c < red[k].size(); c += NNL_REDUCE_GROUP_MAX)
+      NNL_ROUTE("wgrad_group<%s>@n=%d", wgrad_reduce_name[k], (int)std::min<size_t>(NNL_REDUCE_GROUP_MAX, red[k].size() - c));
+
+  for (int i = 0; i < n; ++i)
+    if (jobs[i].kid < 0) {
+      const nnl_wgrad_item_t& it = items[i];
+      const int st = nnl_conv2d_wgrad(it.x, it.dy, it.dw, &it.g, it.workspace, it.workspace_bytes, stream);
+      if (st) return st;
+    }
+  NnlProfScope prof(NNL_PROF_CONV_WGRAD, s, work);
+  for (int k = 0; k < KID_COUNT; ++k)
+    for (size_t c = 0; c < order[k].size(); c += NNL_WGRAD_GROUP_MAX) {
+      const int m = (int)std::min<size_t>(NNL_WGRAD_GROUP_MAX, order[k].size() - c);
+      WgradGroup<IgemmWgradParams> g1{};
+      WgradGroup<IgemmWgrad2dParams> g2{};
+      int total = 0;
+      for (int e = 0; e < m; ++e) {
+        const WgradJob& j = jobs[order[k][c + e]];
+        g1.start[e] = g2.start[e] = total;
+        if (k >= KID_W2_128) g2.p[e] = j.q2; else g1.p[e] = j.q1;
+        total += j.blocks;
+      }
+      for (int e = m; e <= NNL_WGRAD_GROUP_MAX; ++e) g1.start[e] = g2.start[e] = total;
+      g1.n = g2.n = m;
+      const int st = launch_wgrad_group(k, g1, g2, s);
+      if (st) return st;
+    }
+  for (int k = 1; k < 4; ++k)
+    for (size_t c = 0; c < red[k].size(); c += NNL_REDUCE_GROUP_MAX) {
+      const int m = (int)std::min<size_t>(NNL_REDUCE_GROUP_MAX, red[k].size() - c);
+      ReduceGroup rg{};
+      int total = 0;
+      for (int e = 0; e < m; ++e) {
+        const WgradJob& j = jobs[red[k][c + e]];
+        rg.start[e] = total;
+        rg.it[e] = j.r;
+        total += j.rblocks;
+      }
+      for (int e = m; e <= NNL_REDUCE_GROUP_MAX; ++e) rg.start[e] = total;
+      rg.n = m;
+      const int st = launch_reduce_group(k, rg, s);
+      if (st) return st;
+    }
+  return NNL_OK;
+}
+
 extern "C" size_t nnl_colsum_workspace_bytes(int64_t rows, int64_t cols) {
   if (rows <= 0 || cols <= 0) return 0;
   return (size_t)colsum_chunks(rows) * cols * sizeof(float);
diff --git a/neuralnetworklibrary_amd/csrc/igemm_wgrad.h b/neuralnetworklibrary_amd/csrc/igemm_wgrad.h
--- a/neuralnetworklibrary_amd/csrc/igemm_wgrad.h
+++ b/neuralnetworklibrary_amd/csrc/igemm_wgrad.h
@@ -14,8 +14,26 @@
   int n_fast;
 };
 
-template <int BM, int BN, int BK, int WGM, int WGN, bool PIPE = false, int KG = 1, bool WINO = false, bool PAIR = false>
-__global__ __launch_bounds__(256 * KG, KG > 1 ? 1 : ((BM * BN >= 128 * 128) ? 3 : 4)) void igemm_wgrad_kernel(const IgemmWgradParams p) {
+constexpr int NNL_WGRAD_GROUP_MAX = 16;
+template <class Params>
+struct WgradGroup {
+  int n;
+  int start[NNL_WGRAD_GROUP_MAX + 1];
+  Params p[NNL_WGRAD_GROUP_MAX];
+};
+
+template <class Params>
+__device__ __forceinline__ int wgrad_group_find(const WgradGroup<Params>& g, int bid, int& local, int& nblk) {
+  int idx = 0;
+#pragma unroll
+  for (int i = 1; i < NNL_WGRAD_GROUP_MAX; ++i) idx += bid >= g.start[i] ? 1 : 0;
+  local = bid - g.start[idx];
+  nblk = g.start[idx + 1] - g.start[idx];
+  return idx;
+}
+
+template <int BM, int BN, int BK, int WGM, int WGN, bool PIPE, int KG, bool WINO, bool PAIR>
+__device__ __forceinline__ void igemm_wgrad_body(const IgemmWgradParams& p, const int bid, const int nblk) {
   static_assert(WGM * WGN == 4, "4 waves per group");
   static_assert(KG == 1 || (size_t)KG * 2 * BK * (BM + BN) >= (size_t)BM * BN, "the staging LDS must hold one accumulator tile for the group reduction");
   static_assert(!PAIR || (!WINO && BK * BM / 8 >= 256 && BK * BN / 8 >= 256), "PAIR: two chunks per thread on both operands");
@@ -41,7 +59,7 @@
   }
 #endif
   const int tiles = p.grid_m * p.grid_n;
-  const int lb = nnl_xcd_remap((int)blockIdx.x, (int)gridDim.x);
+  const int lb = nnl_xcd_remap(bid, nblk);
   const int split = lb / tiles;
   const int t_id = lb - split * tiles;
   const int tile_n = p.n_fast ? t_id % p.grid_n : t_id / p.grid_m;
@@ -296,3 +314,17 @@
   NNL_TSTAMP(3);
 #endif
 }
+
+#define NNL_WGRAD_BOUNDS __launch_bounds__(256 * KG, KG > 1 ? 1 : ((BM * BN >= 128 * 128) ? 3 : 4))
+template <int BM, int BN, int BK, int WGM, int WGN, bool PIPE = false, int KG = 1, bool WINO = false, bool PAIR = false>
+__global__ NNL_WGRAD_BOUNDS void igemm_wgrad_kernel(const IgemmWgradParams p) {
+  igemm_wgrad_body<BM, BN, BK, WGM, WGN, PIPE, KG, WINO, PAIR>(p, (int)blockIdx.x, (int)gridDim.x);
+}
+
+template <int BM, int BN, int BK, int WGM, int WGN, bool PIPE = false, int KG = 1, bool WINO = false, bool PAIR = false>
+__global__ NNL_WGRAD_BOUNDS void igemm_wgrad_group_kernel(const WgradGroup<IgemmWgradParams> g) {
+  int local, nblk;
+  const int idx = wgrad_group_find(g, (int)blockIdx.x, local, nblk);
+  igemm_wgrad_body<BM, BN, BK, WGM, WGN, PIPE, KG, WINO, PAIR>(g.p[idx], local, nblk);
+}
+#undef NNL_WGRAD_BOUNDS
diff --git a/neuralnetworklibrary_amd/csrc/igemm_wgrad2d.h b/neuralnetworklibrary_amd/csrc/igemm_wgrad2d.h
--- a/neuralnetworklibrary_amd/csrc/igemm_wgrad2d.h
+++ b/neuralnetworklibrary_amd/csrc/igemm_wgrad2d.h
@@ -1,5 +1,6 @@
 #pragma once
 #include "igemm_taps.h"
+#include "igemm_wgrad.h"
 
 struct IgemmWgrad2dParams {
   const float* a;
@@ -13,7 +14,7 @@
 };
 
 template <int BT, int BK, int KG>
-__global__ __launch_bounds__(256 * KG, KG > 1 ? 1 : (BT >= 128 ? 2 : 3)) void igemm_wgrad2d_kernel(const IgemmWgrad2dParams p) {
+__device__ __forceinline__ void igemm_wgrad2d_body(const IgemmWgrad2dParams& p, const int bid, const int nblk) {
   static_assert(KG == 1 || (size_t)KG * 2 * BK * (2 * BT) >= (size_t)BT * BT, "the staging LDS must hold one accumulator tile for the group reduction");
   constexpr int NCH = (BK * BT / 8 >= 256) ? 2 : 1;
   constexpr int CA = BT / (4 * NCH), RA = 256 / CA, PA = BK / RA, C2 = BT / 2;
@@ -26,7 +27,7 @@
   const int tid = threadIdx.x & 255, lane = tid & 63, wave = tid >> 6;
   const int wm = wave >> 1, wn = wave & 1;
   const int tiles = p.grid_m * p.grid_n;
-  const int lb = nnl_xcd_remap((int)blockIdx.x, (int)gridDim.x);
+  const int lb = nnl_xcd_remap(bid, nblk);
   const int split = lb / tiles;
   const int t_id = lb - split * tiles;
   const int tile_n = p.n_fast ? t_id % p.grid_n : t_id / p.grid_m;
@@ -241,3 +242,17 @@
     }
   }
 }
+
+#define NNL_WGRAD2D_BOUNDS __launch_bounds__(256 * KG, KG > 1 ? 1 : (BT >= 128 ? 2 : 3))
+template <int BT, int BK, int KG>
+__global__ NNL_WGRAD2D_BOUNDS void igemm_wgrad2d_kernel(const IgemmWgrad2dParams p) {
+  igemm_wgrad2d_body<BT, BK, KG>(p, (int)blockIdx.x, (int)gridDim.x);
+}
+
+template <int BT, int BK, int KG>
+__global__ NNL_WGRAD2D_BOUNDS void igemm_wgrad2d_group_kernel(const WgradGroup<IgemmWgrad2dParams> g) {
+  int local, nblk;
+  const int idx = wgrad_group_find(g, (int)blockIdx.x, local, nblk);
+  igemm_wgrad2d_body<BT, BK, KG>(g.p[idx], local, nblk);
+}
+#undef NNL_WGRAD2D_BOUNDS
diff --git a/neuralnetworklibrary_amd/ops.py b/neuralnetworklibrary_amd/ops.py
--- a/neuralnetworklibrary_amd/ops.py
+++ b/neuralnetworklibrary_amd/ops.py
@@ -274,11 +274,16 @@
         self.u = ({}, {})
         self.wt = {}
         self.wt_padded = {}
+        self.uses = {}
+        self.defer = False
+        self.pending = {}
+        self.pending_dy = 0
 
     def open(self):
         global _OPEN
         finish_backward()
         self.step += 1
+        self.uses = {}
         _OPEN = self
 
     def recorded(self, key_ptr, which):
@@ -360,8 +365,9 @@
 def finish_backward():
     global _OPEN
     if _OPEN is not None:
-        for views in (*_OPEN.u, _OPEN.wt, _OPEN.wt_padded):
+        for views in (*_OPEN.u, _OPEN.wt, _OPEN.wt_padded, _OPEN.uses, _OPEN.pending):
             views.clear()
+        _OPEN.defer, _OPEN.pending_dy = False, 0
         _OPEN = None
 
 
@@ -378,7 +384,13 @@
 def filter_window(model):
     def backward(loss):
         prepare_backward(model)
-        loss.backward()
+        f = _OPEN
+        f.defer = os.environ.get('NNL_WGRAD_DEFER', '1') != '0'
+        try:
+            loss.backward()
+            _flush_wgrads(f)
+        finally:
+            f.defer = False
     prepare_forward(model)
     try:
         yield backward
@@ -487,7 +499,7 @@
     return lst.pop(0) if lst else p
 
 
-_ConvState = collections.namedtuple('_ConvState', 'g relu has_bias c_in w_layout slot give_slot grad_dst uses')
+_ConvState = collections.namedtuple('_ConvState', 'g relu has_bias c_in w_layout slot give_slot grad_dst uses wuses wref')
 
 
 def _conv_operands(x, weight, bias, stride, pad):
@@ -504,8 +516,12 @@
     uses = getattr(weight, '_nnl_uses', None)
     if uses is not None:
         uses[0] += 1
+    wuses = None
+    if _OPEN is not None:
+        wuses = _OPEN.uses.setdefault(weight.data_ptr(), [0])
+        wuses[0] += 1
     return _ConvState(g, relu, bias is not None, x.shape[1], (tuple(weight.shape), tuple(weight.stride())), slot, give_slot,
-                      getattr(weight, '_nnl_grad_dst', None), uses)
+                      getattr(weight, '_nnl_grad_dst', None), uses, wuses, weakref.ref(weight))
 
 
 def _with_k(g, K):
@@ -596,8 +612,67 @@
     return from_nhwc(dxn[..., :st.c_in] if st.c_in != g.C else dxn)
 
 
+WGRAD_DEFER_DY_CAP = 1 << 30
+_PendingWgrad = collections.namedtuple('_PendingWgrad', 'st xn dy4 dwn g4 K ws wsb out')
+
+
+def _may_defer_wgrad(st, g4, K):
+    f = _OPEN
+    if f is None or not f.defer or st.grad_dst is not None or st.uses is not None or torch.is_grad_enabled():
+        return False
+    if st.wuses is None or st.wuses[0] != 1 or f.uses.get(st.wref().data_ptr() if st.wref() is not None else 0) is not st.wuses:
+        return False
+    w = st.wref()
+    return w.is_leaf and w.grad is None and not w._backward_hooks
+
+
+def _wgrad_view(st, dwn, g4, K):
+    dw = from_nhwc(dwn[:K, :, :, :st.c_in])
+    wshape, wstride = st.w_layout
+    if (g4.R == 1 and g4.S == 1 and wshape == tuple(dw.shape) and wstride != tuple(dw.stride()) and dw.is_contiguous(memory_format=torch.channels_last)
+            and wstride[1] == 1 and wstride[0] == dw.shape[1]):
+        dw = dw.as_strided(wshape, wstride)
+    return dw
+
+
+def _flush_wgrads(f, key=None):
+    items = f.pending.pop(key, []) if key is not None else [it for k in list(f.pending) for it in f.pending.pop(k)]
+    if not items:
+        return
+    arr = (_lib.WgradItem * len(items))()
+    for a, it in zip(arr, items):
+        a.x, a.dy, a.dw, a.g = it.xn.data_ptr(), it.dy4.data_ptr(), it.dwn.data_ptr(), it.g4
+        a.workspace, a.workspace_bytes = it.ws.data_ptr(), it.wsb
+    check(lib.nnl_conv2d_wgrad_group(arr, len(items), stream()))
+    f.pending_dy -= sum(it.dy4.numel() * 4 for it in items)
+    for it in items:
+        if it.out is not None:
+            it.out.copy_(_wgrad_view(it.st, it.dwn, it.g4, it.K))
+        w, handed = it.st.wref(), it.dwn if it.out is None else it.out
+        if w is not None and w.grad is not None and w.grad.untyped_storage().data_ptr() != handed.untyped_storage().data_ptr():
+            w.grad.copy_(_wgrad_view(it.st, it.dwn, it.g4, it.K))
+
+
 def _conv_wgrad(st, xn, dy4, g4, K):
     dst = st.grad_dst
+    if _may_defer_wgrad(st, g4, K):
+        key = int(lib.nnl_conv2d_wgrad_group_key(g4))
+        if key >= 0:
+            f = _OPEN
+            dwn = torch.empty((g4.K, g4.R, g4.S, g4.C), dtype=torch.float32, device=dy4.device)
+            wsb = int(lib.nnl_conv2d_wgrad_workspace_bytes(g4))
+            ws = _workspace(wsb, dy4.device, floor=True)
+            lst = f.pending.setdefault(key, [])
+            out = None
+            if g4.K != K or st.c_in != g4.C:
+                out = torch.empty((K, st.c_in, g4.R, g4.S), dtype=torch.float32, device=dy4.device, memory_format=torch.channels_last)
+            lst.append(_PendingWgrad(st, xn, dy4, dwn, g4, K, ws, wsb, out))
+            f.pending_dy += dy4.numel() * 4
+            if f.pending_dy > WGRAD_DEFER_DY_CAP:
+                _flush_wgrads(f)
+            elif len(lst) >= 16:
+                _flush_wgrads(f, key)
+            return _wgrad_view(st, dwn, g4, K) if out is None else out
     if dst is not None and st.uses is not None and st.uses[0] == 1 and dst.dim() == 4 and g4.K == K and st.c_in == g4.C \
             and dst.permute(0, 2, 3, 1).is_contiguous() and tuple(dst.shape) == (g4.K, g4.C, g4.R, g4.S):
         dwn = dst.permute(0, 2, 3, 1)
@@ -606,12 +681,7 @@
     wsb = int(lib.nnl_conv2d_wgrad_workspace_bytes(g4))
     ws = _workspace(wsb, dy4.device, floor=True)
     check(lib.nnl_conv2d_wgrad(ptr(xn), ptr(dy4), ptr(dwn), g4, ptr(ws), wsb, stream()))
-    dw = from_nhwc(dwn[:K, :, :, :st.c_in])
-    wshape, wstride = st.w_layout
-    if (g4.R == 1 and g4.S == 1 and wshape == tuple(dw.shape) and wstride != tuple(dw.stride()) and dw.is_contiguous(memory_format=torch.channels_last)
-            and wstride[1] == 1 and wstride[0] == dw.shape[1]):
-        dw = dw.as_strided(wshape, wstride)
-    return dw
+    return _wgrad_view(st, dwn, g4, K)
 
 
 def _conv_bias_grad(dy4, g4, K):
```

Result: no change. 5531 images/s, median of 2 (-0.6%).
